# nv-tlabs/GEN3C

Measured on AMD Instinct MI355X. Metric: denoise-steps/sec (121x1280x704 latent, Cosmos-7B), higher is better.
Workload: dtype bf16

## Files before the change

### gen3c_amd/_lib.py

```python
from __future__ import annotations

import ctypes as C
from pathlib import Path

_LIB_PATH = Path(__file__).resolve().parent / "lib" / "libgen3c_hip.so"
_lib = None

vp, i64, i32, f32 = C.c_void_p, C.c_int64, C.c_int, C.c_float

G3_OK, G3_ERR_ARG, G3_ERR_LAUNCH, G3_ERR_RESOURCE = 0, 1, 2, 3

SIGNATURES = {
    "g3_last_error": [],
    "g3_abi_version": [],
    "g3_set_option": [C.c_char_p, i32],
    "g3_device_info": [i32, C.POINTER(i32), C.POINTER(i32), C.c_char_p, i32],
    "g3_event_create": [C.POINTER(vp)],
    "g3_event_record": [vp, vp],
    "g3_event_elapsed_ms": [vp, vp, C.POINTER(f32)],
    "g3_event_destroy": [vp],
    "g3_gemm_bf16_nt": [vp, i64, vp, i64, vp, i64, i32, i32, i32, i32, vp, i32, i64, vp, i64, vp],
    "g3_flash_attn_fwd_kvseg_bf16": [vp, i64, i64, i64, vp, i64, i64, i64, vp, i64, i64, i64, i32, i64, vp, i64, i64, i64, i32, i32, i32,
                                     i32, i32, f32, vp],
    "g3_gemm_kernel_name": [i32, i32, i32, i32],
    "g3_quant_mxfp8_bf16": [vp, i64, vp, i64, vp, i64, i32, i32, vp],
    "g3_gemm_mxfp8_nt": [vp, i64, vp, i64, vp, i64, vp, i64, vp, i64, i32, i32, i32, i32, vp, i32, i64, vp, i64, vp],
    "g3_gemm_mxfp8_kernel_name": [i32, i32, i32, i32],
    "g3_gemm_mxfp8_nt_mxout": [vp, i64, vp, i64, vp, i64, vp, i64, vp, i64, vp, i64, i32, i32, i32, i32, vp],
    "g3_gemm_mxfp8_mxout_kernel_name": [i32, i32, i32, i32],
    "g3_gemv_bf16": [vp, i64, vp, i64, vp, i64, vp, i64, i32, i32, i32, i32, vp],
    "g3_flash_attn_kernel_name": [i32, i32, i32, i32],
    "g3_flash_attn_fwd_bf16": [vp, i64, i64, i64, vp, i64, i64, i64, vp, i64, i64, i64, vp, i64, i64, i64, i32, i32, i32,
                               i32, i32, f32, vp],
    "g3_cross_attn_fwd_bf16": [vp, i64, i64, i64, vp, f32, vp, i64, i64, i64, vp, i64, i64, i64, vp, i64, i64, i64, i32, i32, i32, i32, i32,
                               i32, f32, vp],
    "g3_flash_attn_fwd_ex_bf16": [vp, i64, i64, i64, vp, i64, i64, i64, vp, i64, i64, i64, i32, i64, vp, vp, vp, i64, i64, i64, i32, i32, i32,
                                  i32, i32, f32, i32, vp],
    "g3_flash_attn_fwd_carry_bf16": [vp, i64, i64, i64, vp, i64, i64, i64, vp, i64, i64, i64, i32, i64, i32, i32, vp, vp, vp, vp, vp, i64, i64,
                                     i64, i32, i32, i32, i32, i32, f32, i32, vp],
    "g3_flash_attn_kernel_name_ex": [i32, i32, i32, i32, i32],
    "g3_attn_merge_partials_bf16": [vp, vp, i32, i64, i64, i64, vp, i64, i64, i64, i32, i32, i32, i32, vp],
    "g3_transpose_v_bf16": [vp, i64, vp, i64, i32, i32, i32, i32, vp],
    "g3_layernorm_modulate_bf16": [vp, i64, vp, vp, i64, i32, vp, i64, i32, i32, f32, vp],
    "g3_posemb_layernorm_modulate_bf16": [vp, i64, vp, vp, vp, vp, i32, i32, i32, i32, vp, vp, i64, i32, vp, i64, i32, f32, vp],
    "g3_layernorm_modulate_mxfp8": [vp, i64, vp, vp, i64, i32, vp, i64, vp, i64, i32, i32, f32, vp],
    "g3_posemb_layernorm_modulate_mxfp8": [vp, i64, vp, vp, vp, vp, i32, i32, i32, i32, vp, vp, i64, i32, vp, i64, vp, i64, i32, f32, vp],
    "g3_qk_rmsnorm_rope_bf16": [vp, i64, vp, vp, vp, vp, i64, i32, i32, i32, i32, f32, vp],
    "g3_qk_rmsnorm_rope_pair_bf16": [vp, i64, vp, i32, vp, i32, vp, vp, vp, i64, i32, i32, i32, f32, vp],
    "g3_gemm_qk_norm_rope_bf16": [vp, i64, vp, i64, vp, i64, i32, i32, i32, i32, i32, vp, vp, vp, vp, i32, f32, vp, i64, vp],
    "g3_add_inplace_bf16": [vp, vp, i64, vp],
    "g3_warp_project_f32": [vp, vp, vp, vp, vp, vp, vp, vp, vp, i32, i32, i32, i32, vp],
    "g3_warp_splat_f32": [vp, vp, vp, vp, vp, vp, i32, i32, i32, i32, vp],
    "g3_warp_resolve_f32": [vp, vp, vp, vp, i32, i32, i32, vp],
    "g3_warp_windows_workspace_bytes": [i32, i32, i32],
    "g3_warp_splat_resolve_f32": [vp, vp, vp, vp, vp, vp, vp, vp, vp, vp, i32, i32, i32, i32, vp],
    "g3_render_workspace_bytes": [i32, i32, i32, i32],
    "g3_render_workspace_init": [vp, i32, i32, i32, i32, vp],
    "g3_render_items_f32": [vp, vp, vp, vp, vp, vp, vp, vp, vp, vp, vp, vp, vp, i32, i32, i32, i32, i32, vp],
    "g3_mesh_occlusion_f32": [vp, vp, vp, vp, vp, vp, vp, vp, vp, vp, i32, i32, i32, i32, vp],
    "g3_unproject_points_f32": [vp, vp, vp, vp, i32, i32, i32, vp],
    "g3_dit_patchify_bf16": [vp, vp, vp, i32, vp, i32, i32, i32, i32, i32, i32, vp],
    "g3_dit_unpatchify_bf16": [vp, i64, vp, i32, i32, i32, i32, i32, i32, i32, vp],
    "g3_timestep_embedding_bf16": [vp, vp, vp, vp, i32, i32, vp],
    "g3_reliable_depth_mask_f32": [vp, vp, i32, i32, i32, i32, f32, f32, vp],
    "g3_align_depth_workspace_bytes": [i32, i32],
    "g3_align_depth_f32": [vp, vp, vp, vp, vp, i32, i32, f32, f32, vp, vp, C.c_size_t, i32, i32, vp],
    "g3_conv3d_cl_bf16": [vp, i64, vp, i64, vp, vp, i64, vp, i64] + [i32] * 17 + [vp],
    "g3_conv3d_cl_gnstats_bf16": [vp, i64, vp, i64, vp, vp, i64, vp, i64] + [i32] * 17 + [vp, i32, vp],
    "g3_groupnorm_stats_cl_bf16": [vp, i64, vp, i32, i32, i32, vp],
    "g3_groupnorm_apply_cl_bf16": [vp, i64, vp, vp, vp, vp, i64, i32, i32, i32, f32, i32, vp],
    "g3_groupnorm_swish_cl_bf16": [vp, i64, vp, vp, vp, vp, i64, i32, i32, i32, f32, i32, vp],
    "g3_haar3d_patch_bf16": [vp, vp, i32, i32, i32, vp],
    "g3_haar3d_unpatch_bf16": [vp, i64, vp, i32, i32, i32, vp],
    "g3_resample_cl_bf16": [vp, vp, i32, i32, i32, i32, i32, vp],
    "g3_softmax_rows_bf16": [vp, i64, i32, i32, f32, vp],
    "g3_transpose2d_bf16": [vp, i64, vp, i64, i32, i32, vp],
    "g3_temporal_attn_cl_bf16": [vp, vp, vp, vp, i32, i32, i32, f32, vp],
    "g3_spatial_attn_d512_bf16": [vp, vp, vp, i64, i64, vp, i32, i32, f32, vp],
    "g3_edm_prepare_input_bf16": [vp, vp, vp, vp, vp, vp, i64, i32, i32, f32, f32, f32, f32, vp],
    "g3_edm_cfg_euler_step_bf16": [vp, vp, vp, vp, vp, vp, i64, i32, i32, f32, f32, f32, f32, f32, f32, f32, vp],
}
_RESTYPES = {"g3_last_error": C.c_char_p, "g3_flash_attn_kernel_name": C.c_char_p, "g3_gemm_kernel_name": C.c_char_p, "g3_gemm_mxfp8_kernel_name": C.c_char_p, "g3_gemm_mxfp8_mxout_kernel_name": C.c_char_p, "g3_flash_attn_kernel_name_ex": C.c_char_p, "g3_align_depth_workspace_bytes": C.c_size_t,
             "g3_warp_windows_workspace_bytes": C.c_size_t, "g3_render_workspace_bytes": C.c_size_t}


class Gen3cHipError(RuntimeError):
    pass


def lib_path() -> Path:
    return _LIB_PATH


def load():
    global _lib
    if _lib is not None:
        return _lib
    import torch
    if not _LIB_PATH.exists():
        raise Gen3cHipError(
            f"{_LIB_PATH} is missing: build it with `python -m gen3c_amd.build` (or __graft_entry__.build()). "
            "gen3c_amd has no CPU/PyTorch fallback for its HIP kernels."
        )
    lib = C.CDLL(str(_LIB_PATH))
    for name, argtypes in SIGNATURES.items():
        fn = getattr(lib, name)
        fn.argtypes = argtypes
        fn.restype = _RESTYPES.get(name, C.c_int)
    _lib = lib
    return lib


def last_error() -> str:
    msg = load().g3_last_error()
    return msg.decode() if msg else "?"


def check(rc: int, what: str = ""):
    if rc != 0:
        msg = load().g3_last_error()
        raise Gen3cHipError(f"{what or 'gen3c_hip call'} failed (rc={rc}): {msg.decode() if msg else '?'}")
```

### gen3c_amd/csrc/attention.hip

```cpp
#include "common.hpp"
#include <stdlib.h>
#include <mutex>
#include <type_traits>

namespace {

constexpr int HD = 128;
constexpr int QB = 32;
constexpr int NWAVES = 8;
constexpr int BQ = QB * NWAVES;
constexpr int KVB = 64;
constexpr int NTHREADS = 64 * NWAVES;

struct AttnParams {
    const bf16_t* Q; int64_t q_row, q_batch, q_head;
    const bf16_t* K; int64_t k_row, k_batch, k_head;
    const bf16_t* Vt; int64_t vt_row, vt_batch, vt_head;
    bf16_t* O; int64_t o_row, o_batch, o_head;
    int Sq, Skv;
    float scale_log2;
    int vt_seg_len;
    int64_t vt_seg_stride;
    int grid_q, n_hb, n_heads, xcd_heads;
    float* O32;
    float* LSE;
    int kv_dense;
    const bf16_t* q_norm_w;
    float q_norm_eps;
    const float* carry_o;
    const float* carry_lse;
    int kv_skip_begin, kv_skip_len;
    uint32_t kv_skip_vt_bytes;
};

G3_DEVICE int k_off(int row, int chunk) { return row * HD + ((chunk ^ (row & 15)) << 3); }
G3_DEVICE int v_off(int row, int chunk) { return row * KVB + ((chunk ^ ((row >> 1) & 7)) << 3); }
G3_DEVICE int swap23(int i) { return (i & ~12) | ((i & 4) << 1) | ((i & 8) >> 1); }

template <int CTX>
__global__ __launch_bounds__(NTHREADS, 2) void flash_attn_fwd_kernel(AttnParams p) {
    extern __shared__ __attribute__((aligned(16))) char smem_raw[];
    bf16_t* sK = reinterpret_cast<bf16_t*>(smem_raw);
    bf16_t* sV = sK + 2 * KVB * HD;

    const int tid = threadIdx.x;
    const int lane = tid & 63;
    const int wave = tid >> 6;
    const int l31 = lane & 31;
    const int g = lane >> 5;
    const int head = blockIdx.y;
    const int batch = blockIdx.z;

    const bf16_t* Qb = p.Q + batch * p.q_batch + head * p.q_head;
    const bf16_t* Kb = p.K + batch * p.k_batch + head * p.k_head;
    const bf16_t* Vb = p.Vt + batch * p.vt_batch + head * p.vt_head;
    bf16_t* Ob = p.O + batch * p.o_batch + head * p.o_head;

    const int q_idx = blockIdx.x * BQ + wave * QB + l31;
    const bool q_ok = q_idx < p.Sq;
    bf16x8 qf[8];
    {
        const bf16_t* qrow = Qb + (int64_t)(q_ok ? q_idx : 0) * p.q_row + 8 * g;
#pragma unroll
        for (int ks = 0; ks < 8; ++ks) qf[ks] = q_ok ? load_bf16x8(qrow + 16 * ks) : zero_bf16x8();
    }

    bf16x8 rk[2], rv[2];
    auto stage_load = [&](int kv0) {
#pragma unroll
        for (int i = 0; i < 2; ++i) {
            const int idx = tid + NTHREADS * i;
            {
                const int row = idx >> 4, chunk = idx & 15;
                const bool ok = (kv0 + row) < p.Skv;
                rk[i] = ok ? load_bf16x8(Kb + (int64_t)(kv0 + row) * p.k_row + chunk * 8) : zero_bf16x8();
            }
            {
                const int row = idx >> 3, chunk = idx & 7;
                const bool ok = (kv0 + chunk * 8) < p.Skv;
                rv[i] = ok ? load_bf16x8(Vb + (int64_t)row * p.vt_row + kv0 + chunk * 8) : zero_bf16x8();
            }
        }
    };
    auto stage_write = [&](int buf) {
        bf16_t* dK = sK + buf * KVB * HD;
        bf16_t* dV = sV + buf * HD * KVB;
#pragma unroll
        for (int i = 0; i < 2; ++i) {
            const int idx = tid + NTHREADS * i;
            store_bf16x8(dK + k_off(idx >> 4, idx & 15), rk[i]);
            store_bf16x8(dV + v_off(idx >> 3, idx & 7), rv[i]);
        }
    };

    f32x16 accO[4];
#pragma unroll
    for (int d = 0; d < 4; ++d)
#pragma unroll
        for (int r = 0; r < 16; ++r) accO[d][r] = 0.f;
    float m_run = -1e30f;
    float l_run = 0.f;

    const int krow_perm = swap23(l31);
    const int nt = (p.Skv + KVB - 1) / KVB;
    stage_load(0);
    stage_write(0);
    __syncthreads();

    for (int t = 0; t < nt; ++t) {
        const int buf = t & 1;
        const int kv0 = t * KVB;
        if (t + 1 < nt) stage_load(kv0 + KVB);

        const bf16_t* cK = sK + buf * KVB * HD;
        const bf16_t* cV = sV + buf * HD * KVB;

        f32x16 accS[2];
#pragma unroll
        for (int mb = 0; mb < 2; ++mb) {
#pragma unroll
            for (int r = 0; r < 16; ++r) accS[mb][r] = 0.f;
#pragma unroll
            for (int ks = 0; ks < 8; ++ks) {
                const bf16x8 kf = load_bf16x8(cK + k_off(32 * mb + krow_perm, 2 * ks + g));
                accS[mb] = __builtin_amdgcn_mfma_f32_32x32x16_bf16(kf, qf[ks], accS[mb], 0, 0, 0);
            }
        }

        if (kv0 + KVB > p.Skv) {
#pragma unroll
            for (int mb = 0; mb < 2; ++mb)
#pragma unroll
                for (int r = 0; r < 16; ++r) {
                    const int kv = kv0 + 32 * mb + 16 * (r >> 3) + 8 * g + (r & 7);
                    if (kv >= p.Skv) accS[mb][r] = -INFINITY;
                }
        }

        float mx = accS[0][0];
#pragma unroll
        for (int r = 1; r < 16; ++r) mx = fmaxf(mx, accS[0][r]);
#pragma unroll
        for (int r = 0; r < 16; ++r) mx = fmaxf(mx, accS[1][r]);
        mx = fmaxf(mx, wave_xor_f32(mx, 32));
        const float m_new = fmaxf(m_run, mx * p.scale_log2);
        const float alpha = __builtin_amdgcn_exp2f(m_run - m_new);
        m_run = m_new;

        float psum = 0.f;
        bf16x8 pb[4];
#pragma unroll
        for (int mb = 0; mb < 2; ++mb)
#pragma unroll
            for (int r = 0; r < 16; ++r) {
                const float pv = __builtin_amdgcn_exp2f(__builtin_fmaf(accS[mb][r], p.scale_log2, -m_new));
                psum += pv;
                pb[2 * mb + (r >> 3)][r & 7] = f32_to_bf16(pv);
            }
        l_run = l_run * alpha + psum;
#pragma unroll
        for (int d = 0; d < 4; ++d)
#pragma unroll
            for (int r = 0; r < 16; ++r) accO[d][r] *= alpha;

#pragma unroll
        for (int s = 0; s < 4; ++s) {
#pragma unroll
            for (int d = 0; d < 4; ++d) {
                const bf16x8 vf = load_bf16x8(cV + v_off(32 * d + l31, 2 * s + g));
                accO[d] = __builtin_amdgcn_mfma_f32_32x32x16_bf16(vf, pb[s], accO[d], 0, 0, 0);
            }
        }

        if (t + 1 < nt) stage_write(buf ^ 1);
        __syncthreads();
    }

    const float l_tot = l_run + wave_xor_f32(l_run, 32);
    const float inv = 1.0f / l_tot;
    if (q_ok) {
        bf16_t* orow = Ob + (int64_t)q_idx * p.o_row;
#pragma unroll
        for (int d = 0; d < 4; ++d)
#pragma unroll
            for (int q4 = 0; q4 < 4; ++q4) {
                bf16x4 o;
#pragma unroll
                for (int e = 0; e < 4; ++e) o[e] = f32_to_bf16(accO[d][4 * q4 + e] * inv);
                *reinterpret_cast<bf16x4*>(orow + 32 * d + 8 * q4 + 4 * g) = o;
            }
    }
}


constexpr float RESCALE_THR = 8.0f;

G3_DEVICE float max3(float a, float b, float c) {
    float r;
    asm("v_max3_f32 %0, %1, %2, %3" : "=v"(r) : "v"(a), "v"(b), "v"(c));
    return r;
}
G3_DEVICE void swap_halves(float& a, float& b) {
    asm volatile("s_nop 1\n\tv_permlane32_swap_b32 %0, %1" : "+v"(a), "+v"(b));
}
G3_DEVICE float xor32_max(float x) {
    float a = x, b = x;
    swap_halves(a, b);
    return max3(a, b, b);
}
G3_DEVICE float xor32_sum(float x) {
    float a = x, b = x;
    swap_halves(a, b);
    return a + b;
}

template <int CTX>
__global__ __launch_bounds__(NTHREADS, 2) void flash_attn_fwd_v2_kernel(AttnParams p) {
    extern __shared__ __attribute__((aligned(16))) char smem_raw[];
    bf16_t* sK = reinterpret_cast<bf16_t*>(smem_raw);
    bf16_t* sV = sK + 2 * KVB * HD;

    const int tid = threadIdx.x;
    const int lane = tid & 63;
    const int wave = tid >> 6;
    const int l31 = lane & 31;
    const int g = lane >> 5;
    const int head = blockIdx.y;
    const int batch = blockIdx.z;

    const bf16_t* Qb = p.Q + batch * p.q_batch + head * p.q_head;
    const bf16_t* Kb = p.K + batch * p.k_batch + head * p.k_head;
    const bf16_t* Vb = p.Vt + batch * p.vt_batch + head * p.vt_head;
    bf16_t* Ob = p.O + batch * p.o_batch + head * p.o_head;

    const int q_idx = blockIdx.x * BQ + wave * QB + l31;
    const bool q_ok = q_idx < p.Sq;
    bf16x8 qf[8];
    {
        const bf16_t* qrow = Qb + (int64_t)(q_ok ? q_idx : 0) * p.q_row + 8 * g;
#pragma unroll
        for (int ks = 0; ks < 8; ++ks) qf[ks] = q_ok ? load_bf16x8(qrow + 16 * ks) : zero_bf16x8();
    }

    bf16x8 rk[2], rv[2];
    auto load_k = [&](int kv0) {
#pragma unroll
        for (int i = 0; i < 2; ++i) {
            const int idx = tid + NTHREADS * i;
            const int row = idx >> 4, chunk = idx & 15;
            rk[i] = (kv0 + row) < p.Skv ? load_bf16x8(Kb + (int64_t)(kv0 + row) * p.k_row + chunk * 8) : zero_bf16x8();
        }
    };
    auto load_v = [&](int kv0) {
#pragma unroll
        for (int i = 0; i < 2; ++i) {
            const int idx = tid + NTHREADS * i;
            const int row = idx >> 3, chunk = idx & 7;
            rv[i] = (kv0 + chunk * 8) < p.Skv ? load_bf16x8(Vb + (int64_t)row * p.vt_row + kv0 + chunk * 8) : zero_bf16x8();
        }
    };
    auto write_k = [&](int buf) {
        bf16_t* dK = sK + buf * KVB * HD;
#pragma unroll
        for (int i = 0; i < 2; ++i) {
            const int idx = tid + NTHREADS * i;
            store_bf16x8(dK + k_off(idx >> 4, idx & 15), rk[i]);
        }
    };
    auto write_v = [&](int buf) {
        bf16_t* dV = sV + buf * HD * KVB;
#pragma unroll
        for (int i = 0; i < 2; ++i) {
            const int idx = tid + NTHREADS * i;
            store_bf16x8(dV + v_off(idx >> 3, idx & 7), rv[i]);
        }
    };

    const int krow_perm = swap23(l31);
    int koff[8], voff[4];
#pragma unroll
    for (int ks = 0; ks < 8; ++ks) koff[ks] = k_off(krow_perm, 2 * ks + g);
#pragma unroll
    for (int s4 = 0; s4 < 4; ++s4) voff[s4] = v_off(l31, 2 * s4 + g);
    auto qk = [&](f32x16 (&S)[2], int kbuf) {
        const bf16_t* cK = sK + kbuf * KVB * HD;
#pragma unroll
        for (int mb = 0; mb < 2; ++mb) {
#pragma unroll
            for (int r = 0; r < 16; ++r) S[mb][r] = 0.f;
#pragma unroll
            for (int ks = 0; ks < 8; ++ks) {
                const bf16x8 kf = load_bf16x8(cK + 32 * mb * HD + koff[ks]);
                S[mb] = __builtin_amdgcn_mfma_f32_32x32x16_bf16(kf, qf[ks], S[mb], 0, 0, 0);
            }
        }
    };

    f32x16 accO[4];
#pragma unroll
    for (int d = 0; d < 4; ++d)
#pragma unroll
        for (int r = 0; r < 16; ++r) accO[d][r] = 0.f;
    float m_run = -1e30f;
    float l_run = 0.f;
    const float c = p.scale_log2;
    const int nt = (p.Skv + KVB - 1) / KVB;

    load_k(0);
    load_v(0);
    write_k(0);
    write_v(0);
    if (nt > 1) {
        load_k(KVB);
        write_k(1);
    }
    __syncthreads();
    f32x16 SA[2], SB[2];
    qk(SA, 0);

    auto tile = [&](f32x16 (&S_cur)[2], f32x16 (&S_next)[2], int t, auto has_next_c, auto par_c) {
        constexpr bool has_next = decltype(has_next_c)::value;
        constexpr int par = decltype(par_c)::value;
        const int kv0 = t * KVB;
        if (!has_next && kv0 + KVB > p.Skv) {
#pragma unroll
            for (int mb = 0; mb < 2; ++mb)
#pragma unroll
                for (int r = 0; r < 16; ++r) {
                    const int kv = kv0 + 32 * mb + 16 * (r >> 3) + 8 * g + (r & 7);
                    if (kv >= p.Skv) S_cur[mb][r] = -INFINITY;
                }
        }
        float mx = max3(S_cur[0][0], S_cur[0][1], S_cur[0][2]);
#pragma unroll
        for (int r = 3; r < 15; r += 2) mx = max3(mx, S_cur[0][r], S_cur[0][r + 1]);
// ... 253 lines not shown
            for (int r = 0; r < 16; ++r) SA[mb][r] = 0.f;
#pragma unroll
            for (int ks = 0; ks < 8; ++ks)
                SA[mb] = __builtin_amdgcn_mfma_f32_32x32x16_bf16(load_bf16x8(cK + 32 * mb * HD + koff[ks]), qf[ks], SA[mb], 0, 0, 0);
        }
    }
    G3_JITTER(wave + 1, blockIdx.x);
#ifndef G3_AB_OMIT_PROLOGUE_BARRIER
    __syncthreads();
#endif
    if (nt == 1 && KVB > Skv) mask_tail(SA, 0);
    float mx_cur = row_max(SA);
    f32x16 negm;
    if (FOLD) {
        m_run = mx_cur;
#pragma unroll
        for (int mb = 0; mb < 2; ++mb)
#pragma unroll
            for (int r = 0; r < 16; ++r) SA[mb][r] -= m_run;
#pragma unroll
        for (int r = 0; r < 16; ++r) negm[r] = -m_run;
        mx_cur = 0.f;
    }
#ifndef G3_AB_NO_ATTN_SETPRIO
    if (__builtin_amdgcn_readfirstlane(threadIdx.x) >= 256) __builtin_amdgcn_s_setprio(1);
#endif

    auto tile = [&](f32x16 (&S_cur)[2], f32x16 (&S_next)[2], int t, auto has_next_c, auto par_c) {
        constexpr bool has_next = decltype(has_next_c)::value;
        constexpr int par = decltype(par_c)::value;
        const int kv0 = t * KVB;
        G3_JITTER(wave + blockIdx.x, t);
        if (!has_next && kv0 + KVB > Skv) {
            mask_tail(S_cur, kv0);
            mx_cur = row_max(S_cur);
        }
        if (has_next) {
            if (t + 2 < nt) dma_k(kv0 + 2 * KVB, par);
            dma_v(kv0 + KVB, par ^ 1);
        }
        if (FOLD) {
            if (__any(mx_cur > RESCALE_THR)) {
                const float delta = fmaxf(mx_cur, 0.f);
                const float alpha = __builtin_amdgcn_exp2f(-delta);
                m_run += delta;
                l_run *= alpha;
#pragma unroll
                for (int d = 0; d < 4; ++d)
#pragma unroll
                    for (int r = 0; r < 16; ++r) accO[d][r] *= alpha;
#pragma unroll
                for (int mb = 0; mb < 2; ++mb)
#pragma unroll
                    for (int r = 0; r < 16; ++r) S_cur[mb][r] -= delta;
#pragma unroll
                for (int r = 0; r < 16; ++r) negm[r] = -m_run;
            }
        } else if (__any(mx_cur - m_run > RESCALE_THR)) {
            const float m_new = fmaxf(m_run, mx_cur);
            const float alpha = __builtin_amdgcn_exp2f(m_run - m_new);
            m_run = m_new;
            l_run *= alpha;
#pragma unroll
            for (int d = 0; d < 4; ++d)
#pragma unroll
                for (int r = 0; r < 16; ++r) accO[d][r] *= alpha;
        }
        const float neg_m = -m_run;
        float psum[4] = {0.f, 0.f, 0.f, 0.f};
        bf16x8 pb[4];
        auto softmax_slice = [&](int sl) {
            const int mb = sl >> 1, r0 = (sl & 1) * 8;
#pragma unroll
            for (int j = 0; j < 8; ++j) {
                const float sv = FOLD ? S_cur[mb][r0 + j] : __builtin_fmaf(S_cur[mb][r0 + j], c, neg_m);
                const float pv = (G3_AB_ATTN_ABLATE & 1) ? sv : __builtin_amdgcn_exp2f(sv);
                if (!(G3_AB_ATTN_ABLATE & 2)) psum[sl] += pv;
                pb[sl][j] = f32_to_bf16(pv);
            }
        };

        constexpr int RD = MW_RD;
        bf16x8 fr[RD];
        if (MW && has_next) {
            constexpr int KS = (par ^ 1) * KVB * HD * 2;
            constexpr int VS = par * HD * KVB * 2;
            auto k_addr = [&](auto ksc) -> uint32_t {
                constexpr int ks = decltype(ksc)::value;
                if constexpr (ks < MW_KREGS) return kaddr[ks];
                else return lds_addr_flip128(kaddr[ks - 4]);
            };
            if (!FOLD) {
#pragma unroll
                for (int mb = 0; mb < 2; ++mb)
#pragma unroll
                    for (int r = 0; r < 16; ++r) S_next[mb][r] = 0.f;
            }
            static_for<0, RD - 1>([&](auto ic) { constexpr int i = decltype(ic)::value; lds_read_frag<KS + 32 * (i >> 3) * HD * 2>(fr[i % RD], k_addr(std::integral_constant<int, (i & 7)>{})); });
            static_for<0, 16>([&](auto ic) {
                constexpr int i = decltype(ic)::value;
                constexpr int n = i + RD - 1;
                if constexpr (n < 16) lds_read_frag<KS + 32 * (n >> 3) * HD * 2>(fr[n % RD], k_addr(std::integral_constant<int, (n & 7)>{}));
                else lds_read_frag<VS + 32 * ((n - 16) & 3) * KVB * 2>(fr[n % RD], vaddr[(n - 16) >> 2]);
                lds_wait_frag<RD - 1>(fr[i % RD]);
                S_next[i >> 3] = __builtin_amdgcn_mfma_f32_32x32x16_bf16(fr[i % RD], qf[i & 7], (FOLD && (i & 7) == 0) ? negm : S_next[i >> 3], 0, 0, 0);
                if (i == 3) softmax_slice(0);
                if (i == 11) softmax_slice(1);
            });
#pragma unroll
            for (int i = 0; i < 16; ++i) {
                G3_SGB(SGB_MFMA, 1);
                G3_SGB(SGB_VALU, QA);
                G3_SGB(SGB_TRANS, 1);
            }
        } else if (has_next) {
            const bf16_t* cK = sK + (par ^ 1) * KVB * HD;
            bf16x8 kf[4];
#pragma unroll
            for (int i = 0; i < 3; ++i) kf[i] = load_bf16x8(cK + 32 * (i >> 3) * HD + koff[i & 7]);
            if (G3_AB_ATTN_ABLATE & 8) kf[3] = kf[0];
            if (!FOLD) {
#pragma unroll
                for (int mb = 0; mb < 2; ++mb)
#pragma unroll
                    for (int r = 0; r < 16; ++r) S_next[mb][r] = 0.f;
            }
#pragma unroll
            for (int i = 0; i < 16; ++i) {
                if (i + 3 < 16 && !(G3_AB_ATTN_ABLATE & 8)) kf[(i + 3) & 3] = load_bf16x8(cK + 32 * ((i + 3) >> 3) * HD + koff[(i + 3) & 7]);
                S_next[i >> 3] = __builtin_amdgcn_mfma_f32_32x32x16_bf16(kf[i & 3], qf[i & 7], (FOLD && (i & 7) == 0) ? negm : S_next[i >> 3], 0, 0, 0);
                if (i == 3) softmax_slice(0);
                if (i == 11) softmax_slice(1);
            }
            G3_SGB(SGB_DSR, 3);
#pragma unroll
            for (int i = 0; i < 16; ++i) {
                G3_SGB(SGB_MFMA, 1);
                if (i + 3 < 16) G3_SGB(SGB_DSR, 1);
                G3_SGB(SGB_VALU, QA);
                G3_SGB(SGB_TRANS, 1);
            }
        } else {
            softmax_slice(0);
            softmax_slice(1);
        }

        G3_JITTER(wave + blockIdx.x + 3, t);
        if (MW && has_next) {
            constexpr int VS = par * HD * KVB * 2;
            softmax_slice(2);
            float mx_next = 0.f;
            static_for<0, 16>([&](auto ic) {
                constexpr int i = decltype(ic)::value;
                constexpr int j = i + RD - 1;
                if constexpr (j < 16) lds_read_frag<VS + 32 * (j & 3) * KVB * 2>(fr[(16 + j) % RD], vaddr[j >> 2]);
                lds_wait_frag<(j < 16) ? RD - 1 : (15 - i)>(fr[(16 + i) % RD]);
                accO[i & 3] = __builtin_amdgcn_mfma_f32_32x32x16_bf16(fr[(16 + i) % RD], pb[i >> 2], accO[i & 3], 0, 0, 0);
                if (i == 3) softmax_slice(3);
                if (has_next && i == 7) mx_next = row_max(S_next);
            });
#pragma unroll
            for (int i = 0; i < 16; ++i) {
                G3_SGB(SGB_MFMA, 1);
                G3_SGB(SGB_VALU, QBV);
                G3_SGB(SGB_TRANS, 1);
            }
            l_run += (psum[0] + psum[1]) + (psum[2] + psum[3]);
            mx_cur = mx_next;
        } else {
            const bf16_t* cV = sV + par * HD * KVB;
            bf16x8 vf[4];
#pragma unroll
            for (int i = 0; i < 3; ++i) vf[i] = load_bf16x8(cV + 32 * (i & 3) * KVB + voff[i >> 2]);
            if (G3_AB_ATTN_ABLATE & 8) vf[3] = vf[0];
            softmax_slice(2);
            float mx_next = 0.f;
#pragma unroll
            for (int i = 0; i < 16; ++i) {
                if (i + 3 < 16 && !(G3_AB_ATTN_ABLATE & 8)) vf[(i + 3) & 3] = load_bf16x8(cV + 32 * ((i + 3) & 3) * KVB + voff[(i + 3) >> 2]);
                accO[i & 3] = __builtin_amdgcn_mfma_f32_32x32x16_bf16(vf[i & 3], pb[i >> 2], accO[i & 3], 0, 0, 0);
                if (i == 3) softmax_slice(3);
                if (has_next && i == 7) mx_next = row_max(S_next);
            }
            G3_SGB(SGB_DSR, 3);
#pragma unroll
            for (int i = 0; i < 16; ++i) {
                G3_SGB(SGB_MFMA, 1);
                if (i + 3 < 16) G3_SGB(SGB_DSR, 1);
                G3_SGB(SGB_VALU, QBV);
                G3_SGB(SGB_TRANS, 1);
            }
            l_run += (psum[0] + psum[1]) + (psum[2] + psum[3]);
            mx_cur = mx_next;
        }
        if (has_next) lds_dma_publish_barrier();
    };

    using True = std::integral_constant<bool, true>;
    using False = std::integral_constant<bool, false>;
    using P0 = std::integral_constant<int, 0>;
    using P1 = std::integral_constant<int, 1>;
    int t = 0;
    for (; t + 2 < nt; t += 2) {
        tile(SA, SB, t, True{}, P0{});
        tile(SB, SA, t + 1, True{}, P1{});
    }
    if (t + 1 < nt) {
        tile(SA, SB, t, True{}, P0{});
        tile(SB, SA, t + 1, False{}, P1{});
    } else {
        tile(SA, SB, t, False{}, P0{});
    }

    float l_tot = xor32_sum(l_run);
    float o_scale = 1.0f;
    if (p.kv_dense > 0 && p.kv_dense < p.Skv) {
        const float m_new = fmaxf(m_run, 0.f);
        o_scale = __builtin_amdgcn_exp2f(m_run - m_new);
        l_tot = l_tot * o_scale + (float)(p.Skv - p.kv_dense) * __builtin_amdgcn_exp2f(-m_new);
        m_run = m_new;
    }
    const float inv = o_scale / l_tot;
    if constexpr (CP) {
        const int q_ld = q_ok ? q_idx : p.Sq - 1;
        const int64_t li = ((int64_t)blockIdx.z * p.n_heads + blockIdx.y) * p.Sq + q_ld;
        const int64_t o_hb = (int64_t)blockIdx.z * p.o_batch + (int64_t)blockIdx.y * p.o_head;
        const float lse_k = m_run + __builtin_amdgcn_logf(l_tot);
        f32x4 oc[4][4];
        float lse_c = -INFINITY;
        if (p.carry_lse) {
            const float* crow = p.carry_o + o_hb + (int64_t)q_ld * p.o_row + 4 * g;
#pragma unroll
            for (int d = 0; d < 4; ++d)
#pragma unroll
                for (int q4 = 0; q4 < 4; ++q4) oc[d][q4] = *reinterpret_cast<const f32x4*>(crow + 32 * d + 8 * q4);
            lse_c = p.carry_lse[li];
        } else {
#pragma unroll
            for (int d = 0; d < 4; ++d)
#pragma unroll
                for (int q4 = 0; q4 < 4; ++q4) oc[d][q4] = f32x4{0.f, 0.f, 0.f, 0.f};
        }
        const float mm = fmaxf(lse_c, lse_k);
        const float wc = __builtin_amdgcn_exp2f(lse_c - mm), wk = __builtin_amdgcn_exp2f(lse_k - mm);
        const float rs = 1.0f / (wc + wk);
        const float fc = wc * rs, fk = (wk * rs) * inv;
        const bool use_c = fc > 0.f;
        if (q_ok) {
            const int64_t ro = o_hb + (int64_t)q_idx * p.o_row;
#pragma unroll
            for (int d = 0; d < 4; ++d)
#pragma unroll
                for (int q4 = 0; q4 < 4; ++q4) {
                    const int64_t off = ro + 32 * d + 8 * q4 + 4 * g;
                    f32x4 o;
#pragma unroll
                    for (int e = 0; e < 4; ++e) o[e] = (use_c ? fc * oc[d][q4][e] : 0.f) + fk * accO[d][4 * q4 + e];
                    if (p.O32) {
                        *reinterpret_cast<f32x4*>(p.O32 + off) = o;
                    } else {
                        bf16x4 ob;
#pragma unroll
                        for (int e = 0; e < 4; ++e) ob[e] = f32_to_bf16(o[e]);
                        *reinterpret_cast<bf16x4*>(p.O + off) = ob;
                    }
                }
            if (p.O32 && g == 0) p.LSE[li] = mm + __builtin_amdgcn_logf(wc + wk);
        }
        return;
    }
    if (p.O32) {
        if (q_ok) {
            float* orow = p.O32 + (int64_t)blockIdx.z * p.o_batch + (int64_t)blockIdx.y * p.o_head + (int64_t)q_idx * p.o_row;
#pragma unroll
            for (int d = 0; d < 4; ++d)
#pragma unroll
                for (int q4 = 0; q4 < 4; ++q4) {
                    f32x4 o;
#pragma unroll
                    for (int e = 0; e < 4; ++e) o[e] = accO[d][4 * q4 + e] * inv;
                    *reinterpret_cast<f32x4*>(orow + 32 * d + 8 * q4 + 4 * g) = o;
                }
            if (g == 0) p.LSE[((int64_t)blockIdx.z * p.n_heads + blockIdx.y) * p.Sq + q_idx] = m_run + __builtin_amdgcn_logf(l_tot);
        }
        return;
    }
    if (q_ok) {
        bf16_t* orow = Ob + (int64_t)q_idx * p.o_row;
#pragma unroll
        for (int d = 0; d < 4; ++d)
#pragma unroll
            for (int q4 = 0; q4 < 4; ++q4) {
                bf16x4 o;
#pragma unroll
                for (int e = 0; e < 4; ++e) o[e] = f32_to_bf16(accO[d][4 * q4 + e] * inv);
                *reinterpret_cast<bf16x4*>(orow + 32 * d + 8 * q4 + 4 * g) = o;
            }
    }
}



#include "attention_w4.hpp"
#define W4B_CP 0
#include "attention_w4b.hpp"
#undef W4B_CP
#define W4B_CP 1
#include "attention_w4b.hpp"
#undef W4B_CP

}

static int attn_resolve_variant(int Sq, int Skv, int B, int H, int requested = 0) {
    int variant = requested ? requested : g3_opt_attn_variant;
    if (variant == 0) {
        const long n_wg = (long)((Sq + 255) / 256) * H * B;
        const long rounds = (n_wg + 255) / 256;
        const bool even_fill = n_wg * 100 >= rounds * 256 * 93;
        variant = (Skv > 2048 && (Skv % KVB) == 0 && even_fill) ? 11 : 4;
    }
    if ((variant == 10 || variant == 11) && (Skv % KVB)) variant = 9;
    return variant;
}

extern "C" const char* g3_flash_attn_kernel_name_ex(int Sq, int Skv, int B, int H, int variant_req) {
    const bool long_ctx = Skv > 2048;
    switch (attn_resolve_variant(Sq, Skv, B, H, variant_req)) {
        case 1: return long_ctx ? "flash_attn_fwd_kernel<0>" : "flash_attn_fwd_kernel<1>";
        case 2: return long_ctx ? "flash_attn_fwd_v2_kernel<0>" : "flash_attn_fwd_v2_kernel<1>";
        case 3: return long_ctx ? "flash_attn_fwd_v3_kernel<0, 6, 8, false>" : "flash_attn_fwd_v3_kernel<1, 6, 8, false>";
        case 5: return long_ctx ? "flash_attn_fwd_v3_kernel<0, 6, 8, true>" : "flash_attn_fwd_v3_kernel<1, 6, 8, true>";
        case 6: return long_ctx ? "flash_attn_fwd_v3_kernel<0, 6, 8, true, true, 4, 4>" : "flash_attn_fwd_v3_kernel<1, 6, 8, false, true>";
        case 7: return long_ctx ? "flash_attn_fwd_v3_kernel<0, 6, 8, true, true, 4, 4>" : "flash_attn_fwd_v3_kernel<1, 6, 8, true, true, 4, 4>";
        case 8: return long_ctx ? "flash_attn_fwd_v3_kernel<0, 6, 8, false, true>" : "flash_attn_fwd_v3_kernel<1, 6, 8, false, true>";
        case 9: return long_ctx ? "flash_attn_fwd_w4_kernel<0>" : "flash_attn_fwd_w4_kernel<1>";
        case 10: return "flash_attn_fwd_w4b_kernel<false>";
        case 11: return "flash_attn_fwd_w4b_kernel<true>";
        default: return long_ctx ? "flash_attn_fwd_v3_kernel<0, 6, 8, true>" : "flash_attn_fwd_v3_kernel<1, 6, 8, false>";
    }
}

extern "C" const char* g3_flash_attn_kernel_name(int Sq, int Skv, int B, int H) { return g3_flash_attn_kernel_name_ex(Sq, Skv, B, H, 0); }

static int flash_attn_launch(const void* q, int64_t q_row, int64_t q_batch, int64_t q_head, const void* k, int64_t k_row, int64_t k_batch,
                             int64_t k_head, const void* vt, int64_t vt_row, int64_t vt_batch, int64_t vt_head, int vt_seg_len,
                             int64_t vt_seg_stride, void* o, int64_t o_row, int64_t o_batch, int64_t o_head, int Sq, int Skv, int B, int H,
                             int head_dim, float softmax_scale, void* stream, int variant_req = 0, float* o_partial = nullptr, float* lse = nullptr, int kv_dense = 0,
                             const void* q_norm_w = nullptr, float q_norm_eps = 0.f, bool cp_form = false, const float* carry_o = nullptr,
                             const float* carry_lse = nullptr, int kv_skip_begin = 0, int kv_skip_len = 0, uint32_t kv_skip_vt_bytes = 0) {
    if (!q || !k || !vt || (!o && !o_partial)) return g3_set_error(G3_ERR_ARG, "g3_flash_attn_fwd_bf16: null operand");
    if ((o_partial != nullptr) != (lse != nullptr)) return g3_set_error(G3_ERR_ARG, "g3_flash_attn_fwd_ex_bf16: o_partial and lse go together");
    if (o_partial && (((uintptr_t)o_partial & 15) || ((uintptr_t)lse & 3))) return g3_set_error(G3_ERR_ARG, "g3_flash_attn_fwd_ex_bf16: misaligned o_partial / lse");
    if (head_dim != HD) return g3_set_error(G3_ERR_ARG, "g3_flash_attn_fwd_bf16: head_dim %d unsupported (128 only)", head_dim);
    if (Sq <= 0 || Skv <= 0 || B <= 0 || H <= 0) return g3_set_error(G3_ERR_ARG, "g3_flash_attn_fwd_bf16: bad shape");
    if ((q_row & 7) || (k_row & 7) || (vt_row & 7) || (o_row & 3) || (q_batch & 7) || (k_batch & 7) || (vt_batch & 7) ||
        (q_head & 7) || (k_head & 7) || (vt_head & 7) || (o_batch & 3) || (o_head & 3))
        return g3_set_error(G3_ERR_ARG, "g3_flash_attn_fwd_bf16: strides must keep 16-byte (q,k,vt) / 8-byte (o) alignment");
    if ((((uintptr_t)q | (uintptr_t)k | (uintptr_t)vt) & 15) || ((uintptr_t)o & 7))
        return g3_set_error(G3_ERR_ARG, "g3_flash_attn_fwd_bf16: misaligned pointer");
    const int skv_phys = Skv + kv_skip_len;
    const int kv_span = vt_seg_len > 0 ? vt_seg_len : skv_phys;
    if (vt_seg_len < 0 || (vt_seg_len > 0 && ((vt_seg_len % KVB) || (skv_phys % vt_seg_len) || (vt_seg_stride & 7) || vt_seg_stride <= 0)))
        return g3_set_error(G3_ERR_ARG, "g3_flash_attn_fwd_kvseg_bf16: segments must be a multiple of 64 keys, tile S_kv exactly, 16-byte aligned stride");
    if (vt_row < ((kv_span + 7) & ~7)) return g3_set_error(G3_ERR_ARG, "g3_flash_attn_fwd_bf16: vt leading dim %lld < keys per row rounded to 8", (long long)vt_row);
    AttnParams p;
    p.Q = (const bf16_t*)q; p.q_row = q_row; p.q_batch = q_batch; p.q_head = q_head;
    p.K = (const bf16_t*)k; p.k_row = k_row; p.k_batch = k_batch; p.k_head = k_head;
    p.Vt = (const bf16_t*)vt; p.vt_row = vt_row; p.vt_batch = vt_batch; p.vt_head = vt_head;
    p.O = (bf16_t*)o; p.o_row = o_row; p.o_batch = o_batch; p.o_head = o_head;
    p.Sq = Sq; p.Skv = Skv;
    p.scale_log2 = softmax_scale * 1.4426950408889634f;
    p.vt_seg_len = vt_seg_len; p.vt_seg_stride = vt_seg_stride;
    p.grid_q = 0; p.n_hb = 0; p.n_heads = H; p.xcd_heads = 0;
    p.O32 = o_partial; p.LSE = lse;
    p.kv_dense = 0;
    if (kv_dense > 0) {
        const int kd = ((kv_dense + KVB - 1) / KVB) * KVB;
        if (kv_dense > Skv) return g3_set_error(G3_ERR_ARG, "g3_cross_attn_fwd_bf16: kv_dense %d > S_kv %d", kv_dense, Skv);
        if (kd < Skv) p.kv_dense = kd;
    }
    p.q_norm_w = (const bf16_t*)q_norm_w; p.q_norm_eps = q_norm_eps;
    p.carry_o = carry_o; p.carry_lse = carry_lse;
    p.kv_skip_begin = kv_skip_begin; p.kv_skip_len = kv_skip_len; p.kv_skip_vt_bytes = kv_skip_vt_bytes;
    if (q_norm_w && ((uintptr_t)q_norm_w & 15)) return g3_set_error(G3_ERR_ARG, "g3_cross_attn_fwd_bf16: misaligned q_norm_weight");
    const size_t smem = (size_t)2 * (KVB * HD + HD * KVB) * sizeof(bf16_t);
    static bool attr_set[64] = {};
    static std::mutex attr_mu;
    int variant = attn_resolve_variant(Sq, Skv, B, H, variant_req);
    if (cp_form && variant != 4 && variant != 11)
        return g3_set_error(G3_ERR_ARG, "g3_flash_attn_fwd_carry_bf16: the carry / key-skip form exists for the 8-wave (4) and one-wave-per-SIMD (11) kernels only "
                                        "(variant %d chosen; 11 needs S_kv %% 64 == 0)", variant);
    if (o_partial && variant == 9) variant = 4;
    if ((p.kv_dense || p.q_norm_w) && (variant < 3 || variant >= 9)) variant = 4;
    if (variant >= 3 && vt_row < ((kv_span + KVB - 1) / KVB) * KVB) variant = 2;
    if (variant >= 3) {
        const uint64_t k_max = (uint64_t)(skv_phys - 1 + 2 * KVB) * (uint64_t)k_row * 2u + 256u;
        const uint64_t n_seg = vt_seg_len > 0 ? (uint64_t)(skv_phys / vt_seg_len) : 1u;
        const uint64_t v_max = (uint64_t)(HD - 1) * (uint64_t)vt_row * 2u + (n_seg - 1) * (uint64_t)vt_seg_stride * 2u + ((uint64_t)kv_span + KVB) * 2u + 256u;
        if (k_max > 0xFFFFFFFFull || v_max > 0xFFFFFFFFull) {
            if (cp_form)
                return g3_set_error(G3_ERR_ARG, "g3_flash_attn_fwd_carry_bf16: K / V^T span (skipped keys included) exceeds the kernel's 32-bit byte offsets (k %llu, vt %llu bytes); "
                                                "the 64-bit-addressing kernel has no carry form", (unsigned long long)k_max, (unsigned long long)v_max);
            if (vt_seg_len > 0)
                return g3_set_error(G3_ERR_ARG, "g3_flash_attn_fwd_kvseg_bf16: K / V^T span exceeds the kernel's 32-bit byte offsets (k %llu, vt %llu bytes)",
                                    (unsigned long long)k_max, (unsigned long long)v_max);
            variant = 2;
        }
    }
    if (cp_form && variant < 3)
        return g3_set_error(G3_ERR_ARG, "g3_flash_attn_fwd_carry_bf16: V^T leading dimension %lld below ceil64 of the keys it spans forces the 64-bit-addressing kernel, which has "
                                        "no carry form", (long long)vt_row);
    if (vt_seg_len > 0 && variant < 3)
        return g3_set_error(G3_ERR_ARG, "g3_flash_attn_fwd_kvseg_bf16: segmented V^T is implemented by the default (v3) kernel only");
    if (o_partial && variant < 3)
        return g3_set_error(G3_ERR_ARG, "g3_flash_attn_fwd_ex_bf16: split-KV partial outputs are implemented by the v3 / w4b kernels only (variant %d chosen)", variant);
    if ((p.kv_dense || p.q_norm_w) && variant < 3)
        return g3_set_error(G3_ERR_ARG, "g3_cross_attn_fwd_bf16: the Q norm / zero-tail form is implemented by the v3 kernels only (variant %d chosen: V^T leading dimension below "
                                        "ceil64(S_kv), or operands beyond the kernel's 32-bit byte offsets)", variant);
    int dev_id = 0;
    if (hipGetDevice(&dev_id) != hipSuccess || dev_id < 0 || dev_id >= 64) return g3_set_error(G3_ERR_LAUNCH, "flash_attn: hipGetDevice failed");
    {
      std::lock_guard<std::mutex> attr_lock(attr_mu);
      if (!attr_set[dev_id]) {
        const void* fns[19] = {reinterpret_cast<const void*>(&flash_attn_fwd_w4b_carry_kernel<true>),
                               reinterpret_cast<const void*>(&flash_attn_fwd_v3_kernel<2, 6, 8, true>), reinterpret_cast<const void*>(&flash_attn_fwd_v3_kernel<3, 6, 8, false>),
                               reinterpret_cast<const void*>(&flash_attn_fwd_w4b_kernel<false>), reinterpret_cast<const void*>(&flash_attn_fwd_w4b_kernel<true>),
                               reinterpret_cast<const void*>(&flash_attn_fwd_kernel<0>), reinterpret_cast<const void*>(&flash_attn_fwd_kernel<1>),
                               reinterpret_cast<const void*>(&flash_attn_fwd_v2_kernel<0>), reinterpret_cast<const void*>(&flash_attn_fwd_v2_kernel<1>),
                               reinterpret_cast<const void*>(&flash_attn_fwd_v3_kernel<0, 6, 8, false>), reinterpret_cast<const void*>(&flash_attn_fwd_v3_kernel<1, 6, 8, false>),
                               reinterpret_cast<const void*>(&flash_attn_fwd_v3_kernel<0, 6, 8, true>), reinterpret_cast<const void*>(&flash_attn_fwd_v3_kernel<1, 6, 8, true>),
                               reinterpret_cast<const void*>(&flash_attn_fwd_v3_kernel<0, 6, 8, true, true, 4, 4>), reinterpret_cast<const void*>(&flash_attn_fwd_v3_kernel<1, 6, 8, true, true, 4, 4>),
                               reinterpret_cast<const void*>(&flash_attn_fwd_v3_kernel<0, 6, 8, false, true>), reinterpret_cast<const void*>(&flash_attn_fwd_v3_kernel<1, 6, 8, false, true>),
                               reinterpret_cast<const void*>(&flash_attn_fwd_w4_kernel<0>), reinterpret_cast<const void*>(&flash_attn_fwd_w4_kernel<1>)};
        for (int i = 0; i < 19; ++i) {
            hipError_t e = hipFuncSetAttribute(fns[i], hipFuncAttributeMaxDynamicSharedMemorySize, (int)smem);
            if (e != hipSuccess) return g3_set_error(G3_ERR_LAUNCH, "flash_attn: hipFuncSetAttribute: %s", hipGetErrorString(e));
        }
        attr_set[dev_id] = true;
      }
    }
    dim3 grid((Sq + BQ - 1) / BQ, H, B);
    const bool long_ctx = Skv > 2048;
    hipStream_t st = (hipStream_t)stream;
    if (variant == 10 || variant == 11) {
        dim3 grid4((Sq + W4_BQ - 1) / W4_BQ, H, B);
        p.grid_q = (int)grid4.x; p.n_hb = H * B; p.n_heads = H;
        p.xcd_heads = (g3_opt_attn_xcd_heads && (H * B) % 8 == 0) ? 1 : 0;
        if (p.xcd_heads) grid4 = dim3(grid4.x * H * B, 1, 1);
        if (cp_form) hipLaunchKernelGGL(flash_attn_fwd_w4b_carry_kernel<true>, grid4, dim3(W4_THREADS), smem, st, p);
        else if (variant == 11) hipLaunchKernelGGL(flash_attn_fwd_w4b_kernel<true>, grid4, dim3(W4_THREADS), smem, st, p);
        else hipLaunchKernelGGL(flash_attn_fwd_w4b_kernel<false>, grid4, dim3(W4_THREADS), smem, st, p);
        return g3_check_launch("g3_flash_attn_fwd_bf16");
    }
    if (variant == 9) {
        dim3 grid4((Sq + W4_BQ - 1) / W4_BQ, H, B);
        if (long_ctx) hipLaunchKernelGGL(flash_attn_fwd_w4_kernel<0>, grid4, dim3(W4_THREADS), smem, st, p);
        else hipLaunchKernelGGL(flash_attn_fwd_w4_kernel<1>, grid4, dim3(W4_THREADS), smem, st, p);
        return g3_check_launch("g3_flash_attn_fwd_bf16");
    }
#define G3_LAUNCH_ATTN(KERNEL0, KERNEL1) do { if (long_ctx) hipLaunchKernelGGL(KERNEL0, grid, dim3(NTHREADS), smem, st, p); else hipLaunchKernelGGL(KERNEL1, grid, dim3(NTHREADS), smem, st, p); } while (0)
    if (cp_form) G3_LAUNCH_ATTN((flash_attn_fwd_v3_kernel<2, 6, 8, true>), (flash_attn_fwd_v3_kernel<3, 6, 8, false>));
    else if (variant == 1) G3_LAUNCH_ATTN(flash_attn_fwd_kernel<0>, flash_attn_fwd_kernel<1>);
    else if (variant == 2) G3_LAUNCH_ATTN(flash_attn_fwd_v2_kernel<0>, flash_attn_fwd_v2_kernel<1>);
    else if (variant == 3) G3_LAUNCH_ATTN((flash_attn_fwd_v3_kernel<0, 6, 8, false>), (flash_attn_fwd_v3_kernel<1, 6, 8, false>));
    else if (variant == 5) G3_LAUNCH_ATTN((flash_attn_fwd_v3_kernel<0, 6, 8, true>), (flash_attn_fwd_v3_kernel<1, 6, 8, true>));
    else if (variant == 6) G3_LAUNCH_ATTN((flash_attn_fwd_v3_kernel<0, 6, 8, true, true, 4, 4>), (flash_attn_fwd_v3_kernel<1, 6, 8, false, true>));
    else if (variant == 7) G3_LAUNCH_ATTN((flash_attn_fwd_v3_kernel<0, 6, 8, true, true, 4, 4>), (flash_attn_fwd_v3_kernel<1, 6, 8, true, true, 4, 4>));
    else if (variant == 8) G3_LAUNCH_ATTN((flash_attn_fwd_v3_kernel<0, 6, 8, false, true>), (flash_attn_fwd_v3_kernel<1, 6, 8, false, true>));
    else G3_LAUNCH_ATTN((flash_attn_fwd_v3_kernel<0, 6, 8, true>), (flash_attn_fwd_v3_kernel<1, 6, 8, false>));
#undef G3_LAUNCH_ATTN
    return g3_check_launch("g3_flash_attn_fwd_bf16");
}

extern "C" int g3_flash_attn_fwd_bf16(const void* q, int64_t q_row, int64_t q_batch, int64_t q_head, const void* k,
                                      int64_t k_row, int64_t k_batch, int64_t k_head, const void* vt, int64_t vt_row,
                                      int64_t vt_batch, int64_t vt_head, void* o, int64_t o_row, int64_t o_batch,
                                      int64_t o_head, int Sq, int Skv, int B, int H, int head_dim, float softmax_scale,
                                      void* stream) {
    return flash_attn_launch(q, q_row, q_batch, q_head, k, k_row, k_batch, k_head, vt, vt_row, vt_batch, vt_head, 0, 0, o, o_row, o_batch, o_head,
                             Sq, Skv, B, H, head_dim, softmax_scale, stream);
}

extern "C" int g3_flash_attn_fwd_kvseg_bf16(const void* q, int64_t q_row, int64_t q_batch, int64_t q_head, const void* k, int64_t k_row,
                                            int64_t k_batch, int64_t k_head, const void* vt, int64_t vt_row, int64_t vt_batch,
                                            int64_t vt_head, int vt_seg_len, int64_t vt_seg_stride, void* o, int64_t o_row, int64_t o_batch,
                                            int64_t o_head, int Sq, int Skv, int B, int H, int head_dim, float softmax_scale, void* stream) {
    if (vt_seg_len <= 0) return g3_set_error(G3_ERR_ARG, "g3_flash_attn_fwd_kvseg_bf16: vt_seg_len must be positive");
    return flash_attn_launch(q, q_row, q_batch, q_head, k, k_row, k_batch, k_head, vt, vt_row, vt_batch, vt_head, vt_seg_len, vt_seg_stride, o, o_row,
                             o_batch, o_head, Sq, Skv, B, H, head_dim, softmax_scale, stream);
}

extern "C" int g3_cross_attn_fwd_bf16(const void* q, int64_t q_row, int64_t q_batch, int64_t q_head, const void* q_norm_weight, float q_norm_eps, const void* k,
                                      int64_t k_row, int64_t k_batch, int64_t k_head, const void* vt, int64_t vt_row, int64_t vt_batch, int64_t vt_head, void* o,
                                      int64_t o_row, int64_t o_batch, int64_t o_head, int Sq, int Skv, int kv_dense, int B, int H, int head_dim,
                                      float softmax_scale, void* stream) {
    if (kv_dense < 0) return g3_set_error(G3_ERR_ARG, "g3_cross_attn_fwd_bf16: kv_dense must be >= 0 (0 = every key through the loop)");
    return flash_attn_launch(q, q_row, q_batch, q_head, k, k_row, k_batch, k_head, vt, vt_row, vt_batch, vt_head, 0, 0, o, o_row, o_batch, o_head, Sq, Skv, B, H,
                             head_dim, softmax_scale, stream, 0, nullptr, nullptr, kv_dense, q_norm_weight, q_norm_eps);
}

extern "C" int g3_flash_attn_fwd_ex_bf16(const void* q, int64_t q_row, int64_t q_batch, int64_t q_head, const void* k, int64_t k_row,
                                         int64_t k_batch, int64_t k_head, const void* vt, int64_t vt_row, int64_t vt_batch, int64_t vt_head,
                                         int vt_seg_len, int64_t vt_seg_stride, void* o, float* o_partial, float* lse, int64_t o_row,
                                         int64_t o_batch, int64_t o_head, int Sq, int Skv, int B, int H, int head_dim, float softmax_scale,
                                         int variant, void* stream) {
    if (variant < 0 || variant > 11) return g3_set_error(G3_ERR_ARG, "g3_flash_attn_fwd_ex_bf16: variant %d out of range", variant);
    if (o && o_partial) return g3_set_error(G3_ERR_ARG, "g3_flash_attn_fwd_ex_bf16: pass either o (bf16 result) or o_partial + lse, not both");
    if (o_partial && ((o_row & 3) || (o_batch & 3) || (o_head & 3))) return g3_set_error(G3_ERR_ARG, "g3_flash_attn_fwd_ex_bf16: o_partial strides must be multiples of 4");
    return flash_attn_launch(q, q_row, q_batch, q_head, k, k_row, k_batch, k_head, vt, vt_row, vt_batch, vt_head, vt_seg_len, vt_seg_stride, o, o_row,
                             o_batch, o_head, Sq, Skv, B, H, head_dim, softmax_scale, stream, variant, o_partial, lse);
}

extern "C" int g3_flash_attn_fwd_carry_bf16(const void* q, int64_t q_row, int64_t q_batch, int64_t q_head, const void* k, int64_t k_row,
                                            int64_t k_batch, int64_t k_head, const void* vt, int64_t vt_row, int64_t vt_batch, int64_t vt_head,
                                            int vt_seg_len, int64_t vt_seg_stride, int kv_skip_begin, int kv_skip_len, const float* carry_o,
                                            const float* carry_lse, void* o, float* o_partial, float* lse, int64_t o_row, int64_t o_batch,
                                            int64_t o_head, int Sq, int Skv, int B, int H, int head_dim, float softmax_scale, int variant,
                                            void* stream) {
    const char* fn = "g3_flash_attn_fwd_carry_bf16";
    if (variant < 0 || variant > 11) return g3_set_error(G3_ERR_ARG, "%s: variant %d out of range", fn, variant);
    if (o && o_partial) return g3_set_error(G3_ERR_ARG, "%s: pass either o (bf16 result) or o_partial + lse, not both", fn);
    if (!q || !k || !vt || (!o && !o_partial)) return g3_set_error(G3_ERR_ARG, "%s: null operand", fn);
    if ((o_row & 3) || (o_batch & 3) || (o_head & 3)) return g3_set_error(G3_ERR_ARG, "%s: o / o_partial / carry_o strides must be multiples of 4", fn);
    if ((carry_o != nullptr) != (carry_lse != nullptr)) return g3_set_error(G3_ERR_ARG, "%s: carry_o and carry_lse go together", fn);
    if (carry_o && (((uintptr_t)carry_o & 15) || ((uintptr_t)carry_lse & 3))) return g3_set_error(G3_ERR_ARG, "%s: misaligned carry_o (16 B) / carry_lse (4 B)", fn);
    if (Skv <= 0) return g3_set_error(G3_ERR_ARG, "%s: bad shape", fn);
    if (kv_skip_begin < 0 || kv_skip_len < 0 || (kv_skip_begin % KVB) || (kv_skip_len % KVB) || kv_skip_begin > Skv)
        return g3_set_error(G3_ERR_ARG, "%s: kv_skip (begin %d, len %d) must be multiples of 64 with 0 <= begin <= S_kv %d", fn, kv_skip_begin, kv_skip_len, Skv);
    if (vt_seg_len > 0 && kv_skip_len > 0 && ((kv_skip_begin % vt_seg_len) || (kv_skip_len % vt_seg_len)))
        return g3_set_error(G3_ERR_ARG, "%s: kv_skip (begin %d, len %d) must cover whole V^T segments of %d keys", fn, kv_skip_begin, kv_skip_len, vt_seg_len);
    if ((int64_t)Skv + kv_skip_len > 0x7fffffff) return g3_set_error(G3_ERR_ARG, "%s: S_kv + kv_skip_len overflows", fn);
    const int64_t vt_jump = vt_seg_len > 0 ? (int64_t)(kv_skip_len / vt_seg_len) * vt_seg_stride : (int64_t)kv_skip_len;
    if (vt_seg_len > 0 && vt_seg_stride <= 0) return g3_set_error(G3_ERR_ARG, "%s: vt_seg_stride must be positive", fn);
    if (vt_seg_len == 0 && vt_row < ((int64_t)Skv + kv_skip_len + KVB - 1) / KVB * KVB)
        return g3_set_error(G3_ERR_ARG, "%s: V^T leading dim %lld below ceil64(S_kv + kv_skip_len) forces the 64-bit-addressing kernel, which has no carry form", fn,
                            (long long)vt_row);
    if (kv_skip_len > 0 && kv_skip_begin == 0) {
        k = (const bf16_t*)k + (int64_t)kv_skip_len * k_row;
        vt = (const bf16_t*)vt + vt_jump;
        kv_skip_len = 0;
    }
    if (kv_skip_begin == Skv) kv_skip_len = 0;
    if (kv_skip_len == 0) kv_skip_begin = 0;
    const int64_t vt_jump_bytes = (vt_seg_len > 0 ? (int64_t)(kv_skip_len / vt_seg_len) * vt_seg_stride : (int64_t)kv_skip_len) * 2;
    if (vt_jump_bytes > 0xFFFFFFFFll) return g3_set_error(G3_ERR_ARG, "%s: the skipped V^T range exceeds the kernel's 32-bit byte offsets", fn);
    return flash_attn_launch(q, q_row, q_batch, q_head, k, k_row, k_batch, k_head, vt, vt_row, vt_batch, vt_head, vt_seg_len, vt_seg_stride, o, o_row,
                             o_batch, o_head, Sq, Skv, B, H, head_dim, softmax_scale, stream, variant, o_partial, lse, 0, nullptr, 0.f, true, carry_o,
                             carry_lse, kv_skip_begin, kv_skip_len, (uint32_t)vt_jump_bytes);
}

namespace {
constexpr int MERGE_MAX_PARTS = 8;
struct MergeParams {
    const float* o[MERGE_MAX_PARTS];
    const float* lse[MERGE_MAX_PARTS];
    int n_parts;
    int64_t p_row, p_batch, p_head;
    bf16_t* out; int64_t o_row, o_batch, o_head;
    int Sq, B, H;
};
__global__ __launch_bounds__(256) void attn_merge_partials_kernel(MergeParams p) {
    const int64_t idx = (int64_t)blockIdx.x * 256 + threadIdx.x;
    const int c = (int)(idx & 15);
    int64_t r = idx >> 4;
    const int h = (int)(r % p.H); r /= p.H;
    const int b = (int)(r % p.B);
    const int64_t qi = r / p.B;
    if (qi >= p.Sq) return;
    const int64_t li = ((int64_t)b * p.H + h) * p.Sq + qi;
    float l[MERGE_MAX_PARTS], mx = -INFINITY;
#pragma unroll
    for (int i = 0; i < MERGE_MAX_PARTS; ++i)
        if (i < p.n_parts) { l[i] = p.lse[i][li]; mx = fmaxf(mx, l[i]); }
    float wsum = 0.f;
#pragma unroll
    for (int i = 0; i < MERGE_MAX_PARTS; ++i)
        if (i < p.n_parts) { l[i] = __builtin_amdgcn_exp2f(l[i] - mx); wsum += l[i]; }
    const float inv = 1.0f / wsum;
    float acc[8] = {0.f, 0.f, 0.f, 0.f, 0.f, 0.f, 0.f, 0.f};
    const int64_t poff = qi * p.p_row + (int64_t)b * p.p_batch + (int64_t)h * p.p_head + 8 * c;
#pragma unroll
    for (int i = 0; i < MERGE_MAX_PARTS; ++i)
        if (i < p.n_parts) {
            const f32x4 a = *reinterpret_cast<const f32x4*>(p.o[i] + poff);
            const f32x4 bb = *reinterpret_cast<const f32x4*>(p.o[i] + poff + 4);
            const float w = l[i] * inv;
#pragma unroll
            for (int e = 0; e < 4; ++e) { acc[e] += w * a[e]; acc[4 + e] += w * bb[e]; }
        }
    bf16x8 o;
#pragma unroll
    for (int e = 0; e < 8; ++e) o[e] = f32_to_bf16(acc[e]);
    store_bf16x8(p.out + qi * p.o_row + (int64_t)b * p.o_batch + (int64_t)h * p.o_head + 8 * c, o);
}
}

extern "C" int g3_attn_merge_partials_bf16(const float* const* o_parts, const float* const* lse_parts, int n_parts, int64_t p_row, int64_t p_batch,
                                           int64_t p_head, void* out, int64_t o_row, int64_t o_batch, int64_t o_head, int Sq, int B, int H,
                                           int head_dim, void* stream) {
    if (!o_parts || !lse_parts || !out) return g3_set_error(G3_ERR_ARG, "g3_attn_merge_partials_bf16: null operand");
    if (n_parts < 1 || n_parts > MERGE_MAX_PARTS) return g3_set_error(G3_ERR_ARG, "g3_attn_merge_partials_bf16: 1..%d parts", MERGE_MAX_PARTS);
    if (head_dim != HD || Sq <= 0 || B <= 0 || H <= 0) return g3_set_error(G3_ERR_ARG, "g3_attn_merge_partials_bf16: bad shape");
    if ((p_row & 3) || (p_batch & 3) || (p_head & 3) || (o_row & 7) || (o_batch & 7) || (o_head & 7) || ((uintptr_t)out & 15))
        return g3_set_error(G3_ERR_ARG, "g3_attn_merge_partials_bf16: strides / pointers must keep 16-byte alignment");
    MergeParams p;
    for (int i = 0; i < MERGE_MAX_PARTS; ++i) {
        p.o[i] = i < n_parts ? o_parts[i] : nullptr;
        p.lse[i] = i < n_parts ? lse_parts[i] : nullptr;
        if (i < n_parts && (!p.o[i] || !p.lse[i] || ((uintptr_t)p.o[i] & 15))) return g3_set_error(G3_ERR_ARG, "g3_attn_merge_partials_bf16: part %d null / misaligned", i);
    }
    p.n_parts = n_parts; p.p_row = p_row; p.p_batch = p_batch; p.p_head = p_head;
    p.out = (bf16_t*)out; p.o_row = o_row; p.o_batch = o_batch; p.o_head = o_head; p.Sq = Sq; p.B = B; p.H = H;
    const int64_t total = (int64_t)Sq * B * H * 16;
    hipLaunchKernelGGL(attn_merge_partials_kernel, dim3((unsigned)((total + 255) / 256)), dim3(256), 0, (hipStream_t)stream, p);
    return g3_check_launch("g3_attn_merge_partials_bf16");
}
```

### gen3c_amd/csrc/attention_w4b.hpp

```cpp

#ifndef G3_ATTENTION_W4B_HELPERS
#define G3_ATTENTION_W4B_HELPERS
#define W4B_RING_AGPRS "a192","a193","a194","a195","a196","a197","a198","a199","a200","a201","a202","a203","a204","a205","a206","a207","a208","a209","a210","a211","a212","a213","a214","a215","a216","a217","a218","a219","a220","a221","a222","a223","a224","a225","a226","a227","a228","a229","a230","a231","a232","a233","a234","a235","a236","a237","a238","a239","a240","a241","a242","a243","a244","a245","a246","a247","a248","a249","a250","a251","a252","a253","a254","a255"
#define W4B_OWNED W4_OWNED_AGPRS, W4B_RING_AGPRS
constexpr int W4B_RING0 = 192;
constexpr int W4B_D = 6;

#if G3_AB_ATTN_ABLATE & 32
#define W4B_READ ""
#else
#define W4B_READ "ds_read_b128 a[%c[ra]:%c[rb]], %[addr] offset:%c[off]\n\t"
#endif
#define W4B_QK(h) "v_mfma_f32_32x32x16_bf16 %[s" #h "], a[%c[fa]:%c[fb]], a[%c[q" #h "]:%c[e" #h "]], %[s" #h "]\n\t"
#define W4B_QK0(h) "v_mfma_f32_32x32x16_bf16 %[s" #h "], a[%c[fa]:%c[fb]], a[%c[q" #h "]:%c[e" #h "]], %[c" #h "]\n\t"
#define W4B_PV(h) "v_mfma_f32_32x32x16_bf16 a[%c[o" #h "]:%c[g" #h "]], a[%c[fa]:%c[fb]], %[pf" #h "], a[%c[o" #h "]:%c[g" #h "]]\n\t"
#if G3_AB_ATTN_ABLATE & 128
#define W4B_M0 ""
#define W4B_DMA ""
#else
#define W4B_M0 "s_mov_b32 m0, %[m0v]\n\t"
#define W4B_DMA "global_load_lds_dwordx4 %[voff], %[sbase]\n\t"
#endif
#if G3_AB_ATTN_ABLATE & 256
#define W4B_MAXP(k) ""
#define W4B_MAXP0(k) "v_mov_b32 %[mx], 0\n\tv_mov_b32 %[my], 0\n\t"
#else
#define W4B_MAXP(k) "v_max3_f32 %[mx], %[mx], %[ma" #k "], %[mb" #k "]\n\tv_max3_f32 %[my], %[my], %[mc" #k "], %[md" #k "]\n\t"
#define W4B_MAXP0(k) "v_max3_f32 %[mx], 0, %[ma" #k "], %[mb" #k "]\n\tv_max3_f32 %[my], 0, %[mc" #k "], %[md" #k "]\n\t"
#endif

template <int O0, int O1, int O2, int O3, int O4, int O5> G3_DEVICE void w4b_read_head(uint32_t ad0, uint32_t ad1, uint32_t ad2) {
    static_assert(W4B_D == 6, "w4b_read_head is laid out for a read-ahead of 6");
    if (!(G3_AB_ATTN_ABLATE & 32))
        asm volatile("ds_read_b128 a[192:195], %0 offset:%c3\n\tds_read_b128 a[196:199], %0 offset:%c4\n\tds_read_b128 a[200:203], %1 offset:%c5\n\t"
                     "ds_read_b128 a[204:207], %1 offset:%c6\n\tds_read_b128 a[208:211], %2 offset:%c7\n\tds_read_b128 a[212:215], %2 offset:%c8"
                     ::"v"(ad0), "v"(ad1), "v"(ad2), "n"(O0), "n"(O1), "n"(O2), "n"(O3), "n"(O4), "n"(O5) : W4B_OWNED);
}

#define W4B_XA "v_exp_f32 %[a2], %[x2]\n\tv_exp_f32 %[b2], %[y2]\n\tv_add_f32 %[pe], %[pe], %[a2]\n\t"
#define W4B_XB "v_add_f32 %[pe], %[pe], %[b2]\n\tv_cvt_pk_bf16_f32 %[k2], %[a2], %[b2]\n\t"
template <int I, int ROFF, bool READ, int WN, bool INIT, bool DMA, int EXTRA = 0>
G3_DEVICE void w4b_step_qk(uint32_t addr, f32x16& s0, f32x16& s1, const f32x16& c0, const f32x16& c1, float x1, float y1, uint32_t& k1, float& p1, float& r1,
                           uint32_t m0v, uint32_t voff, const char* sbase, float& a1, float& b1, float x2 = 0.f, float y2 = 0.f, uint32_t* k2 = nullptr,
                           float* pe = nullptr, float* a2 = nullptr, float* b2 = nullptr) {
    constexpr int ks = I >> 1;
    constexpr int q0 = W4_QBASE + 4 * ks, q1 = W4_QBASE + 4 * (8 + ks);
    constexpr int fa = W4B_RING0 + 4 * (I & 15), ra = W4B_RING0 + 4 * ((I + W4B_D) & 15);
#define W4B_A_OUT [a1] "+v"(a1), [b1] "+v"(b1), [k1] "=&v"(k1), [p1] "+v"(p1), [r1] "+v"(r1)
#define W4B_A_IN [addr] "v"(addr), [x1] "v"(x1), [y1] "v"(y1), [off] "n"(ROFF), [wn] "n"(WN), [q0] "n"(q0), [e0] "n"(q0 + 3), [q1] "n"(q1), [e1] "n"(q1 + 3), \
                 [fa] "n"(fa), [fb] "n"(fa + 3), [ra] "n"(ra), [rb] "n"(ra + 3)
    static_assert(READ, "region A always reads ahead");
    if constexpr (INIT && DMA)
        asm volatile(W4B_M0 W4B_READ W4_WAIT W4B_QK0(0) W4_UNIT(1) W4B_DMA W4B_QK0(1)
                     : W4B_A_OUT, [s0] "=&v"(s0), [s1] "=&v"(s1) : W4B_A_IN, [c0] "v"(c0), [c1] "v"(c1), [m0v] "s"(m0v), [voff] "v"(voff), [sbase] "s"(sbase)
                     : "memory");
    else if constexpr (!INIT && DMA)
        asm volatile(W4B_M0 W4B_READ W4_WAIT W4B_QK(0) W4_UNIT(1) W4B_DMA W4B_QK(1)
                     : W4B_A_OUT, [s0] "+v"(s0), [s1] "+v"(s1) : W4B_A_IN, [m0v] "s"(m0v), [voff] "v"(voff), [sbase] "s"(sbase) : "memory");
    else if constexpr (INIT && !DMA && EXTRA == 1)
        asm volatile(W4B_READ W4_WAIT W4B_QK0(0) W4_UNIT(1) W4B_QK0(1) W4B_XA
                     : W4B_A_OUT, [s0] "=&v"(s0), [s1] "=&v"(s1), [a2] "=&v"(*a2), [b2] "=&v"(*b2), [pe] "+v"(*pe)
                     : W4B_A_IN, [c0] "v"(c0), [c1] "v"(c1), [x2] "v"(x2), [y2] "v"(y2));
    else if constexpr (INIT && !DMA)
        asm volatile(W4B_READ W4_WAIT W4B_QK0(0) W4_UNIT(1) W4B_QK0(1)
                     : W4B_A_OUT, [s0] "=&v"(s0), [s1] "=&v"(s1) : W4B_A_IN, [c0] "v"(c0), [c1] "v"(c1));
    else if constexpr (EXTRA == 1)
        asm volatile(W4B_READ W4_WAIT W4B_QK(0) W4_UNIT(1) W4B_QK(1) W4B_XA
                     : W4B_A_OUT, [s0] "+v"(s0), [s1] "+v"(s1), [a2] "=&v"(*a2), [b2] "=&v"(*b2), [pe] "+v"(*pe) : W4B_A_IN, [x2] "v"(x2), [y2] "v"(y2));
    else if constexpr (EXTRA == 2)
        asm volatile(W4B_READ W4_WAIT W4B_QK(0) W4_UNIT(1) W4B_QK(1) W4B_XB
                     : W4B_A_OUT, [s0] "+v"(s0), [s1] "+v"(s1), [k2] "=&v"(*k2), [pe] "+v"(*pe) : W4B_A_IN, [a2] "v"(*a2), [b2] "v"(*b2));
    else
        asm volatile(W4B_READ W4_WAIT W4B_QK(0) W4_UNIT(1) W4B_QK(1) : W4B_A_OUT, [s0] "+v"(s0), [s1] "+v"(s1) : W4B_A_IN);
    static_assert(EXTRA == 0 || (!DMA && !(INIT && EXTRA == 2)), "w4b_step_qk: extra half units only on steps without an LDS-DMA piece");
#undef W4B_A_OUT
#undef W4B_A_IN
}

template <int I, int ROFF, bool READ, int WN, bool UNIT, int MX>
G3_DEVICE void w4b_step_pv(uint32_t addr, const u32x4& pf0, const u32x4& pf1, float x1, float y1, uint32_t& k1, float& p1, float& r1, float& mx, float& my,
                           float ma0, float mb0, float mc0, float md0, float ma1, float mb1, float mc1, float md1, float ma2, float mb2, float mc2, float md2,
                           float& a1, float& b1) {
    constexpr int D = I & 3;
    constexpr int o0 = 16 * D, o1 = 16 * (4 + D);
    constexpr int fa = W4B_RING0 + 4 * ((16 + I) & 15), ra = W4B_RING0 + 4 * ((16 + I + W4B_D) & 15);
#define W4B_B_IN [pf0] "v"(pf0), [pf1] "v"(pf1), [wn] "n"(WN), [o0] "n"(o0), [g0] "n"(o0 + 15), [o1] "n"(o1), [g1] "n"(o1 + 15), [fa] "n"(fa), [fb] "n"(fa + 3)
#define W4B_B_RD [addr] "v"(addr), [off] "n"(ROFF), [ra] "n"(ra), [rb] "n"(ra + 3)
#define W4B_B_UO [a1] "+v"(a1), [b1] "+v"(b1), [k1] "=&v"(k1), [p1] "+v"(p1), [r1] "+v"(r1)
#define W4B_B_UI [x1] "v"(x1), [y1] "v"(y1)
#define W4B_B_M0 [ma0] "v"(ma0), [mb0] "v"(mb0), [mc0] "v"(mc0), [md0] "v"(md0)
    if constexpr (READ && UNIT && MX == 0)
        asm volatile(W4B_READ W4_WAIT W4B_PV(0) W4_UNIT(1) W4B_PV(1) : W4B_B_UO : W4B_B_IN, W4B_B_RD, W4B_B_UI);
    else if constexpr (READ && UNIT && MX == 1)
        asm volatile(W4B_READ W4_WAIT W4B_PV(0) W4_UNIT(1) W4B_PV(1) W4B_MAXP0(0) : W4B_B_UO, [mx] "=&v"(mx), [my] "=&v"(my) : W4B_B_IN, W4B_B_RD, W4B_B_UI, W4B_B_M0);
    else if constexpr (READ && UNIT && MX == 2)
        asm volatile(W4B_READ W4_WAIT W4B_PV(0) W4_UNIT(1) W4B_PV(1) W4B_MAXP(0) : W4B_B_UO, [mx] "+v"(mx), [my] "+v"(my) : W4B_B_IN, W4B_B_RD, W4B_B_UI, W4B_B_M0);
    else if constexpr (!READ && UNIT && MX == 1)
        asm volatile(W4_WAIT W4B_PV(0) W4_UNIT(1) W4B_PV(1) W4B_MAXP0(0) : W4B_B_UO, [mx] "=&v"(mx), [my] "=&v"(my) : W4B_B_IN, W4B_B_UI, W4B_B_M0);
    else if constexpr (!READ && UNIT && MX == 2)
        asm volatile(W4_WAIT W4B_PV(0) W4_UNIT(1) W4B_PV(1) W4B_MAXP(0) : W4B_B_UO, [mx] "+v"(mx), [my] "+v"(my) : W4B_B_IN, W4B_B_UI, W4B_B_M0);
    else if constexpr (!READ && UNIT && MX == 0)
        asm volatile(W4_WAIT W4B_PV(0) W4_UNIT(1) W4B_PV(1) : W4B_B_UO : W4B_B_IN, W4B_B_UI);
    else if constexpr (!READ && !UNIT && MX == 3)
        asm volatile(W4_WAIT W4B_PV(0) W4B_MAXP(0) W4B_PV(1) W4B_MAXP(1) W4B_MAXP(2)
                     : [mx] "+v"(mx), [my] "+v"(my)
                     : W4B_B_IN, W4B_B_M0, [ma1] "v"(ma1), [mb1] "v"(mb1), [mc1] "v"(mc1), [md1] "v"(md1), [ma2] "v"(ma2), [mb2] "v"(mb2), [mc2] "v"(mc2), [md2] "v"(md2));
    else if constexpr (READ && !UNIT && MX == 3)
        asm volatile(W4B_READ W4_WAIT W4B_PV(0) W4B_MAXP(0) W4B_PV(1) W4B_MAXP(1) W4B_MAXP(2)
                     : [mx] "+v"(mx), [my] "+v"(my)
                     : W4B_B_IN, W4B_B_RD, W4B_B_M0, [ma1] "v"(ma1), [mb1] "v"(mb1), [mc1] "v"(mc1), [md1] "v"(md1), [ma2] "v"(ma2), [mb2] "v"(mb2), [mc2] "v"(mc2), [md2] "v"(md2));
    else if constexpr (READ && !UNIT && MX == 0)
        asm volatile(W4B_READ W4_WAIT W4B_PV(0) W4B_PV(1) : : W4B_B_IN, W4B_B_RD);
    else {
        static_assert(!READ && !UNIT && MX == 0, "w4b_step_pv: combination not laid out");
        asm volatile(W4_WAIT W4B_PV(0) W4B_PV(1) : : W4B_B_IN);
    }
#undef W4B_B_RD
#undef W4B_B_UO
#undef W4B_B_UI
#undef W4B_B_M0
}
template <int I, int WN, bool READ = false, int ROFF = 0>
G3_DEVICE void w4b_step_pv_fold(const u32x4& pf0, const u32x4& pf1, float& a0, float& b0, float& c0, float& d0, float& a1, float& b1, float& c1, float& d1, float& t0,
                                 float& t1, uint32_t addr = 0u) {
    constexpr int D = I & 3;
    constexpr int o0 = 16 * D, o1 = 16 * (4 + D);
    constexpr int fa = W4B_RING0 + 4 * ((16 + I) & 15), ra = W4B_RING0 + 4 * ((16 + I + W4B_D) & 15);
    if constexpr (READ && I == 14)
        asm volatile(W4B_READ W4_WAIT W4B_PV(0) "v_max3_f32 %[a0], %[a0], %[b0], %[c0]\n\tv_max3_f32 %[a1], %[a1], %[b1], %[c1]\n\tv_max_f32 %[a0], %[a0], %[d0]\n\tv_max_f32 %[a1], %[a1], %[d1]\n\t"
                     W4B_PV(1) "v_mov_b32 %[t0], %[a0]\n\tv_mov_b32 %[t1], %[a1]\n\t"
                     : [a0] "+v"(a0), [a1] "+v"(a1), [t0] "=&v"(t0), [t1] "=&v"(t1)
                     : W4B_B_IN, [b0] "v"(b0), [c0] "v"(c0), [d0] "v"(d0), [b1] "v"(b1), [c1] "v"(c1), [d1] "v"(d1), [addr] "v"(addr), [off] "n"(ROFF), [ra] "n"(ra), [rb] "n"(ra + 3));
    else if constexpr (READ)
        asm volatile(W4B_READ W4_WAIT W4B_PV(0) "v_permlane32_swap_b32 %[t0], %[a0]\n\tv_permlane32_swap_b32 %[t1], %[a1]\n\t" W4B_PV(1)
                     "v_max_f32 %[a0], %[a0], %[t0]\n\tv_max_f32 %[a1], %[a1], %[t1]\n\t"
                     : [a0] "+v"(a0), [a1] "+v"(a1), [t0] "+v"(t0), [t1] "+v"(t1) : W4B_B_IN, [addr] "v"(addr), [off] "n"(ROFF), [ra] "n"(ra), [rb] "n"(ra + 3));
    else if constexpr (I == 14)
        asm volatile(W4_WAIT W4B_PV(0) "v_max3_f32 %[a0], %[a0], %[b0], %[c0]\n\tv_max3_f32 %[a1], %[a1], %[b1], %[c1]\n\tv_max_f32 %[a0], %[a0], %[d0]\n\tv_max_f32 %[a1], %[a1], %[d1]\n\t"
                     W4B_PV(1) "v_mov_b32 %[t0], %[a0]\n\tv_mov_b32 %[t1], %[a1]\n\t"
                     : [a0] "+v"(a0), [a1] "+v"(a1), [t0] "=&v"(t0), [t1] "=&v"(t1)
                     : W4B_B_IN, [b0] "v"(b0), [c0] "v"(c0), [d0] "v"(d0), [b1] "v"(b1), [c1] "v"(c1), [d1] "v"(d1));
    else
        asm volatile(W4_WAIT W4B_PV(0) "v_permlane32_swap_b32 %[t0], %[a0]\n\tv_permlane32_swap_b32 %[t1], %[a1]\n\t" W4B_PV(1)
                     "v_max_f32 %[a0], %[a0], %[t0]\n\tv_max_f32 %[a1], %[a1], %[t1]\n\t"
                     : [a0] "+v"(a0), [a1] "+v"(a1), [t0] "+v"(t0), [t1] "+v"(t1) : W4B_B_IN);
}
#undef W4B_B_IN

G3_DEVICE void w4b_fence_acc() { asm volatile("s_nop 7\n\ts_nop 3" ::: W4B_OWNED); }
template <int R> G3_DEVICE void w4b_sub_inplace(f32x16& x, float d) {
    float t = x[R];
    asm volatile("v_sub_f32 %0, %0, %1" : "+v"(t) : "v"(d));
    x[R] = t;
}
template <int R> G3_DEVICE void w4b_set_inplace(f32x16& x, float v) {
    float t = x[R];
    asm volatile("v_mov_b32 %0, %1" : "+v"(t) : "v"(v));
    x[R] = t;
}
G3_DEVICE void w4b_mul_inplace(float& x, float a) { asm volatile("v_mul_f32 %0, %0, %1" : "+v"(x) : "v"(a)); }

#endif

#if W4B_CP
#define W4B_KERNEL flash_attn_fwd_w4b_carry_kernel
#else
#define W4B_KERNEL flash_attn_fwd_w4b_kernel
#endif
template <bool XB>
__global__ __launch_bounds__(W4_THREADS, 1) void W4B_KERNEL(AttnParams p) {
    constexpr bool CP = W4B_CP;
    extern __shared__ __attribute__((aligned(16))) char smem_raw[];
    bf16_t* sK = reinterpret_cast<bf16_t*>(smem_raw);
    bf16_t* sV = sK + 2 * KVB * HD;

    const int tid = threadIdx.x;
    const int lane = tid & 63;
    const int wave = __builtin_amdgcn_readfirstlane(tid >> 6);
    const int l31 = lane & 31;
    const int g = lane >> 5;
    int qblk = blockIdx.x, head = blockIdx.y, batch = blockIdx.z;
    if (p.xcd_heads) {
        const int xcd = blockIdx.x & 7, slot = blockIdx.x >> 3;
        const int hb = xcd + 8 * (slot / p.grid_q);
        qblk = slot - (slot / p.grid_q) * p.grid_q;
        head = hb % p.n_heads;
        batch = hb / p.n_heads;
    }

    const bf16_t* Qb = p.Q + batch * p.q_batch + head * p.q_head;
    const bf16_t* Kb = p.K + batch * p.k_batch + head * p.k_head;
    const bf16_t* Vb = p.Vt + batch * p.vt_batch + head * p.vt_head;
    bf16_t* Ob = p.O + batch * p.o_batch + head * p.o_head;
    float* o32_base = p.O32;
    float* lse_base = p.LSE;
    asm volatile("" : "+s"(o32_base), "+s"(lse_base));
    const float* carry_o = nullptr;
    const float* carry_lse = nullptr;
    uint32_t skip_t0 = 0u, skip_nt = 0u, v_skip = 0u;
    if constexpr (CP) {
        carry_o = p.carry_o;
        carry_lse = p.carry_lse;
        skip_t0 = (uint32_t)p.kv_skip_begin / KVB;
        skip_nt = (uint32_t)p.kv_skip_len / KVB;
        v_skip = p.kv_skip_vt_bytes;
        asm volatile("" : "+s"(carry_o), "+s"(carry_lse), "+s"(skip_t0), "+s"(skip_nt), "+s"(v_skip));
    }
    auto k_tile = [&](uint32_t t) -> uint32_t {
        if constexpr (CP) return t + (t >= skip_t0 ? skip_nt : 0u);
        else return t;
    };

    static_for<0, 16>([&](auto fc) {
        constexpr int f = decltype(fc)::value, h = f >> 3, ks = f & 7;
        const int q_idx = qblk * W4_BQ + wave * 64 + 32 * h + l31;
        const bool q_ok = q_idx < p.Sq;
        bf16x8 qv = q_ok ? load_bf16x8(Qb + (int64_t)q_idx * p.q_row + 8 * g + 16 * ks) : zero_bf16x8();
#pragma unroll
        for (int e = 0; e < 8; ++e) qv[e] = f32_to_bf16((float)qv[e] * p.scale_log2);
        const u32x4 qw = __builtin_bit_cast(u32x4, qv);
        w4_acc_write<W4_QBASE + 4 * f + 0>(qw[0]);
        w4_acc_write<W4_QBASE + 4 * f + 1>(qw[1]);
        w4_acc_write<W4_QBASE + 4 * f + 2>(qw[2]);
        w4_acc_write<W4_QBASE + 4 * f + 3>(qw[3]);
    });
    static_for<0, 128>([&](auto rc) { w4_acc_zero<decltype(rc)::value>(); });

    const int k_row0 = tid >> 4, k_src_chunk = (tid & 15) ^ (k_row0 & 15);
    const int v_row0 = tid >> 3, v_src_chunk = (tid & 7) ^ ((v_row0 >> 1) & 7);
    const char* Kbytes = reinterpret_cast<const char*>(Kb);
    const char* Vbytes = reinterpret_cast<const char*>(Vb);
    const uint32_t k_row_bytes = (uint32_t)p.k_row * 2u;
    const uint32_t v_row_bytes = (uint32_t)p.vt_row * 2u;
    uint32_t dma_off[8];
#pragma unroll
    for (int j = 0; j < 4; ++j) {
        dma_off[j] = ((uint32_t)k_row0 + 16u * j) * k_row_bytes + (uint32_t)k_src_chunk * 16u;
        dma_off[4 + j] = ((uint32_t)v_row0 + 32u * j) * v_row_bytes + (uint32_t)v_src_chunk * 16u;
    }
#pragma unroll
    for (int j = 0; j < 8; ++j) asm volatile("" : "+v"(dma_off[j]));
    const uint32_t k_tile_bytes = (uint32_t)KVB * k_row_bytes;
    const uint32_t seg_len = (uint32_t)p.vt_seg_len, seg_bytes = (uint32_t)p.vt_seg_stride * 2u;
    auto v_tile_off = [&](uint32_t kv0) -> uint32_t {
        if (!seg_len) return kv0 * 2u;
        const uint32_t sg = kv0 / seg_len;
        return sg * seg_bytes + (kv0 - sg * seg_len) * 2u;
    };
    auto dma_tile_builtin = [&](const char* base, const uint32_t* off, bf16_t* dst) {
#pragma unroll
        for (int i = 0; i < 4; ++i)
            __builtin_amdgcn_global_load_lds((const __attribute__((address_space(1))) void*)(base + off[i]),
                                             (__attribute__((address_space(3))) void*)(dst + wave * 64 * 8 + 256 * 8 * i), 16, 0, 0);
    };

    const int krow_perm = swap23(l31);
    const uint32_t lds_k0 = (uint32_t)(uintptr_t)(__attribute__((address_space(3))) bf16_t*)sK;
    const uint32_t lds_v0 = (uint32_t)(uintptr_t)(__attribute__((address_space(3))) bf16_t*)sV;
    uint32_t kaddr[8], vaddr[4];
#pragma unroll
    for (int ks = 0; ks < 8; ++ks) kaddr[ks] = lds_k0 + 2u * (uint32_t)k_off(krow_perm, 2 * ks + g);
#pragma unroll
    for (int s4 = 0; s4 < 4; ++s4) vaddr[s4] = lds_v0 + 2u * (uint32_t)v_off(l31, 2 * s4 + g);

    float m_run[2], mx_cur[2];
    float psum[2][4];
#pragma unroll
    for (int h = 0; h < 2; ++h)
#pragma unroll
        for (int k = 0; k < 4; ++k) psum[h][k] = 0.f;
    float ta[2] = {0.f, 0.f}, tb[2] = {0.f, 0.f};
    float pe[2][2] = {{0.f, 0.f}, {0.f, 0.f}};
    float xa[2], xb[2];
    const int nt = p.Skv / KVB;

    dma_tile_builtin(Kbytes, dma_off, sK);
    dma_tile_builtin(Vbytes, dma_off + 4, sV);
    if (nt > 1) dma_tile_builtin(Kbytes + k_tile(1u) * k_tile_bytes, dma_off, sK + KVB * HD);
    G3_JITTER(wave, blockIdx.x + 5);
    lds_dma_publish_barrier();
    G3_JITTER(wave + 2, blockIdx.x);
    f32x16 SA[2][2], SB[2][2];
    f32x16 negm[2];
    {
        f32x16 zero;
#pragma unroll
        for (int r = 0; r < 16; ++r) zero[r] = 0.f;
        static_for<0, 16>([&](auto ic) {
            constexpr int i = decltype(ic)::value, mb = i >> 3, ks = i & 7;
            const bf16x8 kf = load_bf16x8(sK + 32 * mb * HD + k_off(krow_perm, 2 * ks + g));
            if constexpr (ks == 0) {
                w4_qk0<0, -1>(SA[0][mb], kf, zero);
                w4_qk0<8, -1>(SA[1][mb], kf, zero);
            } else {
                w4_qk<ks, -1>(SA[0][mb], kf);
                w4_qk<8 + ks, -1>(SA[1][mb], kf);
            }
        });
    }
    w4_fence_v(SA[0][0], SA[0][1], SA[1][0], SA[1][1]);
    __syncthreads();
#pragma unroll
    for (int h = 0; h < 2; ++h) {
        float ma = max3(SA[h][0][0], SA[h][0][1], SA[h][0][2]);
        float mb2 = max3(SA[h][1][0], SA[h][1][1], SA[h][1][2]);
#pragma unroll
        for (int r = 3; r < 15; r += 2) {
            ma = max3(ma, SA[h][0][r], SA[h][0][r + 1]);
            mb2 = max3(mb2, SA[h][1][r], SA[h][1][r + 1]);
        }
        m_run[h] = xor32_max(max3(ma, mb2, max3(SA[h][0][15], SA[h][1][15], SA[h][1][15])));
#pragma unroll
        for (int mb = 0; mb < 2; ++mb)
#pragma unroll
            for (int r = 0; r < 16; ++r) SA[h][mb][r] -= m_run[h];
#pragma unroll
        for (int r = 0; r < 16; ++r) negm[h][r] = -m_run[h];
        mx_cur[h] = 0.f;
    }
    if (XB && nt > 1) {
        constexpr int KS1 = KVB * HD * 2;
        w4b_read_head<KS1, KS1 + 32 * HD * 2, KS1, KS1 + 32 * HD * 2, KS1, KS1 + 32 * HD * 2>(kaddr[0], kaddr[1], kaddr[2]);
    }
    uint32_t v_off_next = v_tile_off(KVB);
    if constexpr (CP) v_off_next += skip_t0 == 1u ? v_skip : 0u;
    const uint32_t seg_tiles = seg_len ? seg_len / KVB : 0x7fffffffu;
    uint32_t v_seg_pos = seg_len ? (1u % seg_tiles) : 1u;
    const uint32_t v_seg_jump = seg_len ? seg_bytes - seg_len * 2u : 0u;

    auto tile = [&](f32x16 (&S_cur)[2][2], f32x16 (&S_next)[2][2], int t, auto has_next_c, auto par_c) {
        constexpr bool has_next = decltype(has_next_c)::value;
        constexpr int par = decltype(par_c)::value;
        constexpr int D = W4B_D;
        constexpr int KS = (par ^ 1) * KVB * HD * 2;
        constexpr int VS = par * HD * KVB * 2;
        auto frag_off = [](auto nc) constexpr { constexpr int n = decltype(nc)::value; return n < 16 ? KS + 32 * (n & 1) * HD * 2 : VS + 32 * ((n - 16) & 3) * KVB * 2; };
        auto frag_addr = [&](auto nc) -> uint32_t { constexpr int n = decltype(nc)::value; if constexpr (n < 16) return kaddr[(n >> 1) & 7]; else return vaddr[((n - 16) >> 2) & 3]; };
        G3_JITTER(wave + blockIdx.x, t);
        if constexpr (!(XB && has_next)) {
            constexpr int n0 = has_next ? 0 : 16;
            using N0 = std::integral_constant<int, n0>;
            using N1 = std::integral_constant<int, n0 + 1>;
            using N2 = std::integral_constant<int, n0 + 2>;
            using N3 = std::integral_constant<int, n0 + 3>;
            using N4 = std::integral_constant<int, n0 + 4>;
            using N5 = std::integral_constant<int, n0 + 5>;
            w4b_read_head<frag_off(N0{}), frag_off(N1{}), frag_off(N2{}), frag_off(N3{}), frag_off(N4{}), frag_off(N5{})>(frag_addr(N0{}), frag_addr(N2{}), frag_addr(N4{}));
        }
        if (__any(fmaxf(mx_cur[0], mx_cur[1]) > RESCALE_THR)) {
            float alpha[2], delta[2];
#pragma unroll
            for (int h = 0; h < 2; ++h) {
                delta[h] = mx_cur[h];
                alpha[h] = __builtin_amdgcn_exp2f(-delta[h]);
                m_run[h] += delta[h];
            }
            asm volatile("s_nop 7\n\ts_nop 3" : "+v"(alpha[0]), "+v"(alpha[1]) : : W4B_OWNED);
#pragma unroll
            for (int h = 0; h < 2; ++h) {
#pragma unroll
                for (int k = 0; k < 4; ++k) w4b_mul_inplace(psum[h][k], alpha[h]);
                if (XB && h == 0) {
                    w4b_mul_inplace(pe[0][0], alpha[0]);
                    w4b_mul_inplace(pe[0][1], alpha[0]);
                    w4b_mul_inplace(pe[1][0], alpha[0]);
                    w4b_mul_inplace(pe[1][1], alpha[0]);
                }
                const float nm = -m_run[h], dl = delta[h];
                static_for<0, 16>([&](auto rc) {
                    constexpr int r = decltype(rc)::value;
                    w4b_sub_inplace<r>(S_cur[h][0], dl);
                    w4b_sub_inplace<r>(S_cur[h][1], dl);
                    w4b_set_inplace<r>(negm[h], nm);
                });
            }
            static_for<0, 64>([&](auto rc) { w4_acc_scale<decltype(rc)::value>(alpha[0]); });
            static_for<64, 128>([&](auto rc) { w4_acc_scale<decltype(rc)::value>(alpha[1]); });
        }
        u32x4 pb[2][4];
        auto ux = [&](auto uc) -> float { constexpr int u = decltype(uc)::value, sl = u >> 3, h = (u >> 2) & 1, q = u & 3; return S_cur[h][sl >> 1][(sl & 1) * 8 + 2 * q]; };
        auto uy = [&](auto uc) -> float { constexpr int u = decltype(uc)::value, sl = u >> 3, h = (u >> 2) & 1, q = u & 3; return S_cur[h][sl >> 1][(sl & 1) * 8 + 2 * q + 1]; };
        auto uput = [&](auto uc, uint32_t pk) { constexpr int u = decltype(uc)::value, sl = u >> 3, h = (u >> 2) & 1, q = u & 3; pb[h][sl][q] = pk; };
        auto sm_unit = [&](auto uc) {
            constexpr int u = decltype(uc)::value, h = (u >> 2) & 1, pa = 2 * (u & 1);
            float a, b;
            uint32_t pk;
            if (G3_AB_ATTN_ABLATE & 16) {
                pk = 0;
            } else {
                asm volatile("v_exp_f32 %0, %5\n\tv_exp_f32 %1, %6\n\tv_add_f32 %3, %3, %0\n\tv_add_f32 %4, %4, %1\n\tv_cvt_pk_bf16_f32 %2, %0, %1"
                             : "=&v"(a), "=&v"(b), "=v"(pk), "+v"(psum[h][pa]), "+v"(psum[h][pa + 1]) : "v"(ux(uc)), "v"(uy(uc)));
            }
            uput(uc, pk);
        };
        constexpr int NHEAD = has_next ? (XB ? 0 : 4) : 20;
        static_for<0, NHEAD>([&](auto uc) { sm_unit(uc); });

        if constexpr (has_next) {
            const int t2 = min(t + 2, nt - 1);
            const char* kbase = Kbytes + k_tile((uint32_t)t2) * k_tile_bytes;
            const char* vbase = Vbytes + v_off_next;
            static_for<0, 16>([&](auto ic) {
                constexpr int I = decltype(ic)::value;
                using NR = std::integral_constant<int, I + D>;
                using U = std::integral_constant<int, (XB ? 0 : 4) + I>;
                constexpr int hu = (U::value >> 2) & 1, pa = 2 * (I & 1);
                constexpr bool dma = XB ? (I & 1) == 0 : I < 8;
                constexpr int j = XB ? (I >> 1) : (I & 7);
                const uint32_t m0v = dma ? (j < 4 ? lds_k0 + (uint32_t)(par * KVB * HD * 2 + 256 * j * 16) : lds_v0 + (uint32_t)((par ^ 1) * HD * KVB * 2 + 256 * (j - 4) * 16)) + (uint32_t)wave * 1024u : 0u;
                uint32_t k1 = 0;
                if constexpr (XB && (I & 1)) {
                    constexpr int ex = (I & 2) ? 2 : 1;
                    constexpr int xu = 16 + (I >> 2);
                    using XU = std::integral_constant<int, xu>;
                    uint32_t k2 = 0;
                    w4b_step_qk<I, frag_off(NR{}), true, D, (I >> 1) == 0, false, ex>(frag_addr(NR{}), S_next[0][I & 1], S_next[1][I & 1], negm[0], negm[1], ux(U{}), uy(U{}), k1,
                                                                                      psum[hu][pa], psum[hu][pa + 1], 0u, 0u, nullptr, ta[I & 1], tb[I & 1], ux(XU{}), uy(XU{}), &k2,
                                                                                      &pe[0][ex - 1], &xa[0], &xb[0]);
                    if constexpr (ex == 2) uput(XU{}, k2);
                } else {
                    w4b_step_qk<I, frag_off(NR{}), true, D, (I >> 1) == 0, dma>(frag_addr(NR{}), S_next[0][I & 1], S_next[1][I & 1], negm[0], negm[1], ux(U{}), uy(U{}), k1,
                                                                               psum[hu][pa], psum[hu][pa + 1], m0v, dma_off[j], j < 4 ? kbase : vbase, ta[I & 1], tb[I & 1]);
                }
                uput(U{}, k1);
            });
            const bool wrap = (v_seg_pos + 1u == seg_tiles);
            v_off_next += wrap ? (uint32_t)(KVB * 2) + v_seg_jump : (uint32_t)(KVB * 2);
            v_seg_pos = wrap ? 0u : v_seg_pos + 1u;
            if constexpr (CP) v_off_next += (uint32_t)(t + 2) == skip_t0 ? v_skip : 0u;
        }
        G3_JITTER(wave + blockIdx.x + 3, t);
        {
            float cx[2][2], cy[2][2], tx[2];
            auto sn = [&](auto hc, auto mbc, auto rc) -> float { return S_next[decltype(hc)::value][decltype(mbc)::value][decltype(rc)::value]; };
            constexpr int KSN = par * KVB * HD * 2;
            auto rd_off = [](auto nc) constexpr { constexpr int n = decltype(nc)::value; return n < 32 ? VS + 32 * ((n - 16) & 3) * KVB * 2 : KSN + 32 * (n & 1) * HD * 2; };
            auto rd_addr = [&](auto nc) -> uint32_t { constexpr int n = decltype(nc)::value; if constexpr (n < 32) return vaddr[((n - 16) >> 2) & 3]; else return kaddr[((n - 32) >> 1) & 7]; };
            static_for<0, 14>([&](auto ic) {
                constexpr int I = decltype(ic)::value;
                constexpr bool rd = (I + D < 16) || (XB && has_next);
                using NR = std::integral_constant<int, rd ? 16 + I + D : 16>;
                constexpr bool unit = I < 12;
                using U = std::integral_constant<int, unit ? 20 + I : 20>;
                constexpr int hu = (U::value >> 2) & 1, pa = 2 * (I & 1);
                constexpr int mxk = !has_next ? 0 : (I < 2 ? 0 : (I == 2 || I == 3 || I == 10 || I == 11) ? 1 : I < 12 ? 2 : 3);
                constexpr int mh = I < 10 ? 0 : 1;
                constexpr int k0 = I < 2 ? 0 : I < 10 ? I - 2 : I < 12 ? I - 10 : I == 12 ? 2 : 5;
                constexpr int k1i = mxk == 3 ? k0 + 1 : k0, k2i = mxk == 3 ? k0 + 2 : k0;
                using H = std::integral_constant<int, mh>;
#define W4B_SN(mb, r) (has_next ? sn(H{}, std::integral_constant<int, mb>{}, std::integral_constant<int, (r)>{}) : 0.f)
                if constexpr (XB && has_next && I == 10) {
                    if (!(G3_AB_ATTN_ABLATE & 64)) asm volatile("s_waitcnt vmcnt(0)\n\ts_barrier" ::: "memory");
                }
                uint32_t k1 = 0;
                w4b_step_pv<I, rd_off(NR{}), rd, rd ? D : 15 - I, unit, mxk>(rd_addr(NR{}), pb[0][I >> 2], pb[1][I >> 2], ux(U{}), uy(U{}), k1, psum[hu][pa], psum[hu][pa + 1],
                                                                          cx[mh][I & 1], cy[mh][I & 1], W4B_SN(0, 2 * k0), W4B_SN(0, 2 * k0 + 1), W4B_SN(1, 2 * k0),
                                                                          W4B_SN(1, 2 * k0 + 1), W4B_SN(0, 2 * k1i), W4B_SN(0, 2 * k1i + 1), W4B_SN(1, 2 * k1i),
                                                                          W4B_SN(1, 2 * k1i + 1), W4B_SN(0, 2 * k2i), W4B_SN(0, 2 * k2i + 1), W4B_SN(1, 2 * k2i),
                                                                          W4B_SN(1, 2 * k2i + 1), ta[I & 1], tb[I & 1]);
#undef W4B_SN
                if constexpr (unit) uput(U{}, k1);
            });
            if constexpr (has_next) {
                if constexpr (XB) {
                    using N14 = std::integral_constant<int, 16 + 14 + D>;
                    using N15 = std::integral_constant<int, 16 + 15 + D>;
                    w4b_step_pv_fold<14, D, true, rd_off(N14{})>(pb[0][3], pb[1][3], cx[0][0], cy[0][0], cx[0][1], cy[0][1], cx[1][0], cy[1][0], cx[1][1], cy[1][1], tx[0], tx[1],
                                                                 rd_addr(N14{}));
                    w4b_step_pv_fold<15, D, true, rd_off(N15{})>(pb[0][3], pb[1][3], cx[0][0], cy[0][0], cx[0][1], cy[0][1], cx[1][0], cy[1][0], cx[1][1], cy[1][1], tx[0], tx[1],
                                                                 rd_addr(N15{}));
                } else {
                    w4b_step_pv_fold<14, 1>(pb[0][3], pb[1][3], cx[0][0], cy[0][0], cx[0][1], cy[0][1], cx[1][0], cy[1][0], cx[1][1], cy[1][1], tx[0], tx[1]);
                    w4b_step_pv_fold<15, 0>(pb[0][3], pb[1][3], cx[0][0], cy[0][0], cx[0][1], cy[0][1], cx[1][0], cy[1][0], cx[1][1], cy[1][1], tx[0], tx[1]);
                }
                mx_cur[0] = cx[0][0];
                mx_cur[1] = cx[1][0];
            } else {
                float d0 = 0.f, d1 = 0.f;
                uint32_t kd = 0;
                w4b_step_pv<14, 0, false, 1, false, 0>(0u, pb[0][3], pb[1][3], 0.f, 0.f, kd, d0, d1, d0, d1, 0, 0, 0, 0, 0, 0, 0, 0, 0, 0, 0, 0, d0, d1);
                w4b_step_pv<15, 0, false, 0, false, 0>(0u, pb[0][3], pb[1][3], 0.f, 0.f, kd, d0, d1, d0, d1, 0, 0, 0, 0, 0, 0, 0, 0, 0, 0, 0, 0, d0, d1);
            }
        }
        if (!XB && has_next && !(G3_AB_ATTN_ABLATE & 64)) lds_dma_publish_barrier();
    };

    using True = std::integral_constant<bool, true>;
    using False = std::integral_constant<bool, false>;
    using P0 = std::integral_constant<int, 0>;
    using P1 = std::integral_constant<int, 1>;
    int t = 0;
    for (; t + 2 < nt; t += 2) {
        tile(SA, SB, t, True{}, P0{});
        tile(SB, SA, t + 1, True{}, P1{});
    }
    if (t + 1 < nt) {
        tile(SA, SB, t, True{}, P0{});
        tile(SB, SA, t + 1, False{}, P1{});
    } else {
        tile(SA, SB, t, False{}, P0{});
    }

    w4b_fence_acc();
    static_for<0, 2>([&](auto hc) {
        constexpr int h = decltype(hc)::value;
        const float extra = (XB && h == 0) ? (pe[0][0] + pe[0][1]) + (pe[1][0] + pe[1][1]) : 0.f;
        const float inv = 1.0f / xor32_sum(((psum[h][0] + psum[h][1]) + (psum[h][2] + psum[h][3])) + extra);
        const int q_idx = qblk * W4_BQ + wave * 64 + 32 * h + l31;
        if constexpr (CP) {
            const bool q_ok = q_idx < p.Sq;
            const int q_ld = q_ok ? q_idx : p.Sq - 1;
            const int64_t li = ((int64_t)batch * p.n_heads + head) * p.Sq + q_ld;
            const int64_t ro = (int64_t)batch * p.o_batch + (int64_t)head * p.o_head + (int64_t)q_idx * p.o_row;
            const int64_t ro_ld = (int64_t)batch * p.o_batch + (int64_t)head * p.o_head + (int64_t)q_ld * p.o_row;
            const float lse_k = m_run[h] - __builtin_amdgcn_logf(inv);
            f32x4 oc[16];
            float lse_c = -INFINITY;
            if (carry_lse) {
                using gf32x4 = const __attribute__((address_space(1))) f32x4;
                gf32x4* crow = (gf32x4*)(carry_o + ro_ld + 4 * g);
#pragma unroll
                for (int c = 0; c < 16; ++c) oc[c] = crow[(32 * (c >> 2) + 8 * (c & 3)) / 4];
                lse_c = ((const __attribute__((address_space(1))) float*)carry_lse)[li];
            } else {
#pragma unroll
                for (int c = 0; c < 16; ++c) oc[c] = f32x4{0.f, 0.f, 0.f, 0.f};
            }
            const float mm = fmaxf(lse_c, lse_k);
            const float wc = __builtin_amdgcn_exp2f(lse_c - mm), wk = __builtin_amdgcn_exp2f(lse_k - mm);
            const float rs = 1.0f / (wc + wk);
            const float fc = wc * rs, fk = (wk * rs) * inv;
            const bool use_c = fc > 0.f;
            static_for<0, 16>([&](auto cc) {
                constexpr int c = decltype(cc)::value, d = c >> 2, q4 = c & 3;
                constexpr int R = 16 * (4 * h + d) + 4 * q4;
                const int64_t off = ro + 32 * d + 8 * q4 + 4 * g;
                float o[4];
                o[0] = (use_c ? fc * oc[c][0] : 0.f) + fk * w4_acc_read<R + 0>();
                o[1] = (use_c ? fc * oc[c][1] : 0.f) + fk * w4_acc_read<R + 1>();
                o[2] = (use_c ? fc * oc[c][2] : 0.f) + fk * w4_acc_read<R + 2>();
                o[3] = (use_c ? fc * oc[c][3] : 0.f) + fk * w4_acc_read<R + 3>();
                if (!q_ok) return;
                if (o32_base) {
                    *reinterpret_cast<f32x4*>(o32_base + off) = f32x4{o[0], o[1], o[2], o[3]};
                } else {
                    bf16x4 ob;
#pragma unroll
                    for (int e = 0; e < 4; ++e) ob[e] = f32_to_bf16(o[e]);
                    *reinterpret_cast<bf16x4*>(p.O + off) = ob;
                }
            });
            if (o32_base && g == 0 && q_ok) lse_base[li] = mm + __builtin_amdgcn_logf(wc + wk);
            return;
        }
        if (o32_base) {
            float* prow = o32_base + (int64_t)batch * p.o_batch + (int64_t)head * p.o_head + (int64_t)q_idx * p.o_row;
            static_for<0, 16>([&](auto cc) {
                constexpr int d = decltype(cc)::value >> 2, q4 = decltype(cc)::value & 3;
                constexpr int R = 16 * (4 * h + d) + 4 * q4;
                f32x4 o;
                o[0] = w4_acc_read<R + 0>() * inv;
                o[1] = w4_acc_read<R + 1>() * inv;
                o[2] = w4_acc_read<R + 2>() * inv;
                o[3] = w4_acc_read<R + 3>() * inv;
                if (q_idx < p.Sq) *reinterpret_cast<f32x4*>(prow + 32 * d + 8 * q4 + 4 * g) = o;
            });
            if (g == 0 && q_idx < p.Sq) lse_base[((int64_t)batch * p.n_heads + head) * p.Sq + q_idx] = m_run[h] - __builtin_amdgcn_logf(inv);
            return;
        }
        bf16_t* orow = Ob + (int64_t)q_idx * p.o_row;
        static_for<0, 16>([&](auto cc) {
            constexpr int d = decltype(cc)::value >> 2, q4 = decltype(cc)::value & 3;
            constexpr int R = 16 * (4 * h + d) + 4 * q4;
            bf16x4 o;
            o[0] = f32_to_bf16(w4_acc_read<R + 0>() * inv);
            o[1] = f32_to_bf16(w4_acc_read<R + 1>() * inv);
            o[2] = f32_to_bf16(w4_acc_read<R + 2>() * inv);
            o[3] = f32_to_bf16(w4_acc_read<R + 3>() * inv);
            if (q_idx < p.Sq) *reinterpret_cast<bf16x4*>(orow + 32 * d + 8 * q4 + 4 * g) = o;
        });
    });
}
#undef W4B_KERNEL
```

### gen3c_amd/dit.py

```python
from __future__ import annotations

import math
from enum import Enum
from typing import Dict, List, Optional, Tuple

import torch
from torch import nn

from . import ops
from .parallel import ContextParallelAttention, split_inputs_cp

_FUSE_QKV_EPILOGUE = __import__("os").environ.get("G3_FUSE_QKV_EPILOGUE", "0") != "0"


_V_OPERAND_SWAP = __import__("os").environ.get("G3_V_OPERAND_SWAP", "1") != "0"


def _v_by_operand_swap(S: int) -> bool:
    return _V_OPERAND_SWAP and S % 4 == 0


_CROSS_Q_NORM_IN_ATTENTION = __import__("os").environ.get("G3_CROSS_Q_NORM_IN_ATTENTION", "1") != "0"


def _project_norm_rope(h, w, n_q, n_k, norm_q, norm_k, cos, sin, S, B, nH_total, hq=None, wq=None):
    if wq is not None:
        y = ops.gemm_mxfp8_nt(hq[0], hq[1], wq[0], wq[1])
    elif _FUSE_QKV_EPILOGUE:
        return ops.gemm_qk_norm_rope(h, w, n_q, n_k, norm_q, norm_k, cos, sin, S, B)
    else:
        y = ops.gemm_nt(h, w)
    if n_q and n_k:
        ops.qk_rmsnorm_rope_pair(y[:, :n_q + n_k], norm_q, n_q // 128, norm_k, n_k // 128, cos, sin, S, B)
    elif n_q:
        ops.qk_rmsnorm_rope(y[:, :n_q], norm_q, cos, sin, S, B, n_q // 128, out=y[:, :n_q])
    elif n_k:
        ops.qk_rmsnorm_rope(y[:, n_q:n_q + n_k], norm_k, cos, sin, S, B, n_k // 128, out=y[:, n_q:n_q + n_k])
    return y


LINEAR_PRECISIONS = ("bf16", "mxfp8")
MXFP8_PRODUCERS = ("separate", "fused")
MXFP8_LINEARS = ("fa_qkv", "fa_out", "ca_q", "ca_out", "w1", "w2")


def _mx_rows(blk: dict, name: str, rows: slice):
    mx = blk.get("mx")
    return None if mx is None else (mx[name][0][rows], mx[name][1][rows])


class DataType(Enum):
    IMAGE = "image"
    VIDEO = "video"


def tensor_version(t: torch.Tensor) -> Optional[int]:
    return None if t.is_inference() else t._version


def cacheable(*tensors) -> bool:
    return all(not (isinstance(t, torch.Tensor) and t.is_inference()) for t in tensors)


def _is_video(data_type) -> bool:
    v = getattr(data_type, "value", data_type)
    return str(v).lower().endswith("video")


class _Node(nn.Module):
    """Anonymous container used to reproduce the reference's parameter names (e.g. `to_q.0.weight`)."""


def _register(root: nn.Module, dotted: str, tensor: torch.Tensor, buffer: bool = False):
    *path, leaf = dotted.split(".")
    mod = root
    for p in path:
        if p not in mod._modules:
            mod.add_module(p, _Node())
        mod = mod._modules[p]
    if buffer:
        mod.register_buffer(leaf, tensor, persistent=True)
    else:
        mod.register_parameter(leaf, nn.Parameter(tensor, requires_grad=False))


def _xavier_uniform_(t: torch.Tensor):
    fan_out, fan_in = t.shape
    a = math.sqrt(6.0 / (fan_in + fan_out))
    return t.uniform_(-a, a)


class VideoExtendGeneralDIT(nn.Module):
    def __init__(
        self,
        max_img_h: int = 240,
        max_img_w: int = 240,
        max_frames: int = 128,
        in_channels: int = 16 + 1,
        out_channels: int = 16,
        patch_spatial: int = 2,
        patch_temporal: int = 1,
        concat_padding_mask: bool = True,
        block_config: str = "FA-CA-MLP",
        model_channels: int = 4096,
        num_blocks: int = 28,
        num_heads: int = 32,
        mlp_ratio: float = 4.0,
        block_x_format: str = "THWBD",
        crossattn_emb_channels: int = 1024,
        use_cross_attn_mask: bool = False,
        pos_emb_cls: str = "rope3d",
        pos_emb_learnable: bool = False,
        pos_emb_interpolation: str = "crop",
        affline_emb_norm: bool = True,
        use_adaln_lora: bool = True,
        adaln_lora_dim: int = 256,
        rope_h_extrapolation_ratio: float = 1.0,
        rope_w_extrapolation_ratio: float = 1.0,
        rope_t_extrapolation_ratio: float = 1.0,
        extra_per_block_abs_pos_emb: bool = True,
        extra_per_block_abs_pos_emb_type: str = "learnable",
        extra_h_extrapolation_ratio: float = 1.0,
        extra_w_extrapolation_ratio: float = 1.0,
        extra_t_extrapolation_ratio: float = 1.0,
        add_augment_sigma_embedding: bool = False,
        device: Optional[torch.device | str] = None,
        dtype: torch.dtype = torch.bfloat16,
        init_weights: bool = True,
        linear_precision: str = "bf16",
        mxfp8_producers: str = "separate",
    ) -> None:
        super().__init__()
        if block_config.upper() != "FA-CA-MLP":
            raise NotImplementedError(f"block_config {block_config!r}: only 'FA-CA-MLP' (GEN3C-Cosmos-7B) is built")
        if block_x_format != "THWBD" or pos_emb_cls != "rope3d" or not use_adaln_lora or not affline_emb_norm:
            raise NotImplementedError("only the faditv2 configuration (THWBD, rope3d, AdaLN-LoRA, affine emb norm) is built")
        if not extra_per_block_abs_pos_emb or extra_per_block_abs_pos_emb_type.lower() != "learnable":
            raise NotImplementedError("extra_per_block_abs_pos_emb must be the learnable per-axis embedding")
        if use_cross_attn_mask or add_augment_sigma_embedding or pos_emb_learnable:
            raise NotImplementedError("use_cross_attn_mask / add_augment_sigma_embedding / learnable rope are not used by GEN3C")
        if model_channels // num_heads != 128:
            raise NotImplementedError("head_dim must be 128 (HIP attention kernel)")
        if dtype != torch.bfloat16:
            raise NotImplementedError("the HIP path computes in bf16 (reference precision='bfloat16', config/base/model.py:29)")

        self.max_img_h, self.max_img_w, self.max_frames = max_img_h, max_img_w, max_frames
        self.in_channels, self.out_channels = in_channels, out_channels
        self.patch_spatial, self.patch_temporal = patch_spatial, patch_temporal
        self.concat_padding_mask = concat_padding_mask
        self.model_channels, self.num_blocks, self.num_heads = model_channels, num_blocks, num_heads
        self.mlp_hidden = int(model_channels * mlp_ratio)
        self.crossattn_emb_channels = crossattn_emb_channels
        self.adaln_lora_dim = adaln_lora_dim
        self.block_x_format = block_x_format
        self.head_dim = 128
        self.base_fps = 24
        self.cp_group = None
        self.cp_size = None
        self._cp_attn: Optional[ContextParallelAttention] = None
        self.cross_attention_skip_zero_context = True
        self._tables: Dict[tuple, tuple] = {}
        self._packed = None
        self.linear_precision = "bf16"
        self.set_linear_precision(linear_precision)
        self.mxfp8_producers = "separate"
        self.set_mxfp8_producers(mxfp8_producers)
        self._tune_blocks: Optional[int] = None

        D, Hd = model_channels, self.head_dim
        kw = dict(device=device, dtype=dtype)
        E = lambda *shape: torch.empty(*shape, **kw)
        emb_in = (in_channels + (1 if concat_padding_mask else 0)) * patch_spatial * patch_spatial * patch_temporal
        self.patch_dim = emb_in

        _register(self, "x_embedder.proj.1.weight", E(D, emb_in))
        len_h, len_w, len_t = max_img_h // patch_spatial, max_img_w // patch_spatial, max_frames // patch_temporal
        _register(self, "pos_embedder.seq", torch.arange(max(len_h, len_w, len_t), dtype=torch.float, device=device), buffer=True)
        _register(self, "extra_pos_embedder.pos_emb_h", E(len_h, D))
        _register(self, "extra_pos_embedder.pos_emb_w", E(len_w, D))
        _register(self, "extra_pos_embedder.pos_emb_t", E(len_t, D))
        _register(self, "t_embedder.1.linear_1.weight", E(D, D))
        _register(self, "t_embedder.1.linear_2.weight", E(3 * D, D))
        for i in range(num_blocks):
            pre = f"blocks.block{i}.blocks"
            for j, ctx in ((0, D), (1, crossattn_emb_channels)):
                a = f"{pre}.{j}.block.attn"
                _register(self, f"{a}.to_q.0.weight", E(D, D))
                _register(self, f"{a}.to_q.1.weight", E(Hd))
                _register(self, f"{a}.to_k.0.weight", E(D, ctx))
                _register(self, f"{a}.to_k.1.weight", E(Hd))
                _register(self, f"{a}.to_v.0.weight", E(D, ctx))
                _register(self, f"{a}.to_out.0.weight", E(D, D))
            _register(self, f"{pre}.2.block.layer1.weight", E(self.mlp_hidden, D))
            _register(self, f"{pre}.2.block.layer2.weight", E(D, self.mlp_hidden))
            for j in range(3):
                _register(self, f"{pre}.{j}.adaLN_modulation.1.weight", E(adaln_lora_dim, D))
                _register(self, f"{pre}.{j}.adaLN_modulation.2.weight", E(3 * D, adaln_lora_dim))
        _register(self, "final_layer.linear.weight", E(patch_spatial * patch_spatial * patch_temporal * out_channels, D))
        _register(self, "final_layer.adaLN_modulation.1.weight", E(adaln_lora_dim, D))
        _register(self, "final_layer.adaLN_modulation.2.weight", E(2 * D, adaln_lora_dim))
        _register(self, "affline_norm.weight", E(D))

        dim_h = Hd // 6 * 2
        dim_t = Hd - 2 * dim_h
        self._rope_dims = (dim_t, dim_h, dim_h)
        self.h_ntk_factor = rope_h_extrapolation_ratio ** (dim_h / (dim_h - 2))
        self.w_ntk_factor = rope_w_extrapolation_ratio ** (dim_h / (dim_h - 2))
        self.t_ntk_factor = rope_t_extrapolation_ratio ** (dim_t / (dim_t - 2))

        if init_weights:
            self.initialize_weights()

    @torch.no_grad()
    def initialize_weights(self, randomize_adaln: bool = False, seed: Optional[int] = None):
        gen = None
        if seed is not None:
            gen = torch.Generator(device=self.affline_norm.weight.device)
            gen.manual_seed(seed)
        for name, p in self.named_parameters():
            if name.endswith(".to_q.1.weight") or name.endswith(".to_k.1.weight") or name == "affline_norm.weight":
                p.fill_(1.0)
            elif name.startswith("extra_pos_embedder."):
                tmp = torch.empty(p.shape, dtype=torch.float32, device=p.device)
                nn.init.trunc_normal_(tmp, std=0.02, a=-2.0, b=2.0, generator=gen)
                p.copy_(tmp)
            elif name.startswith("t_embedder."):
                p.normal_(0.0, 0.02, generator=gen)
            elif name.endswith("adaLN_modulation.2.weight") and not name.startswith("final_layer."):
                if randomize_adaln:
                    p.normal_(0.0, 0.02, generator=gen)
                else:
                    p.zero_()
            else:
                fan_out, fan_in = p.shape
                a = math.sqrt(6.0 / (fan_in + fan_out))
                p.uniform_(-a, a, generator=gen)
        self._packed = None
        self._tables.clear()

    def load_state_dict(self, state_dict, strict: bool = True, assign: bool = False):
        sd = {k: v for k, v in state_dict.items() if not k.endswith("_extra_state")}
        out = super().load_state_dict(sd, strict=strict, assign=assign)
        self._packed = None
        self._tables.clear()
        return out

    def _apply(self, fn, *args, **kwargs):
        out = super()._apply(fn, *args, **kwargs)
        self._packed = None
        self._tables.clear()
        return out

    def set_linear_precision(self, precision: str) -> None:
        if precision not in LINEAR_PRECISIONS:
            raise ValueError(f"linear_precision must be one of {LINEAR_PRECISIONS}, got {precision!r}")
        if precision != self.linear_precision:
            self._packed = None
        self.linear_precision = precision

    def set_mxfp8_producers(self, producers: str) -> None:
        if producers not in MXFP8_PRODUCERS:
            raise ValueError(f"mxfp8_producers must be one of {MXFP8_PRODUCERS}, got {producers!r}")
        self.mxfp8_producers = producers

    def _linear(self, a, blk: dict, name: str, out_mx: bool = False, **kw):
        mx = blk.get("mx")
        if mx is None:
            return ops.gemm_nt(a, blk[name], **kw)
        aq, as_ = a if isinstance(a, tuple) else ops.quant_mxfp8(a)
        if out_mx:
            kw["out_mx"] = True
        return ops.gemm_mxfp8_nt(aq, as_, mx[name][0], mx[name][1], **kw)

    def _ln(self, xs: torch.Tensor, shift: torch.Tensor, scale: torch.Tensor, fused: bool):
        return ops.layernorm_modulate_mxfp8(xs, shift, scale) if fused else ops.layernorm_modulate(xs, shift, scale)

    def _weights_key(self) -> tuple:
        return tuple((p.data_ptr(), tensor_version(p)) for p in self.parameters())

    def _pack(self):
        key = self._weights_key()
        if (self._packed is not None and self._packed["key"] == key and self._packed["versioned"]
                and self._packed["precision"] == self.linear_precision):
            return self._packed
        if self._packed is not None and self._packed["key"] != key:
            self._tables.clear()
        P = dict(self.named_parameters())
        blocks = []
        for i in range(self.num_blocks):
            pre = f"blocks.block{i}.blocks"
            fa, ca, mlp = f"{pre}.0", f"{pre}.1", f"{pre}.2"
            blocks.append(dict(
                fa_qkv=torch.cat([P[f"{fa}.block.attn.to_q.0.weight"], P[f"{fa}.block.attn.to_k.0.weight"],
                                  P[f"{fa}.block.attn.to_v.0.weight"]], dim=0).contiguous(),
                fa_qn=P[f"{fa}.block.attn.to_q.1.weight"], fa_kn=P[f"{fa}.block.attn.to_k.1.weight"],
                fa_out=P[f"{fa}.block.attn.to_out.0.weight"],
                ca_q=P[f"{ca}.block.attn.to_q.0.weight"],
                ca_kv=torch.cat([P[f"{ca}.block.attn.to_k.0.weight"], P[f"{ca}.block.attn.to_v.0.weight"]], dim=0).contiguous(),
                ca_qn=P[f"{ca}.block.attn.to_q.1.weight"], ca_kn=P[f"{ca}.block.attn.to_k.1.weight"],
                ca_out=P[f"{ca}.block.attn.to_out.0.weight"],
                w1=P[f"{mlp}.block.layer1.weight"], w2=P[f"{mlp}.block.layer2.weight"],
                ada=[(P[f"{pre}.{j}.adaLN_modulation.1.weight"], P[f"{pre}.{j}.adaLN_modulation.2.weight"]) for j in range(3)],
            ))
        if self.linear_precision == "mxfp8":
            for blk in blocks:
                blk["mx"] = {n: ops.quant_mxfp8(blk[n]) for n in MXFP8_LINEARS}
        self._packed = dict(blocks=blocks, P=P, key=key, versioned=cacheable(*P.values()), precision=self.linear_precision)
        return self._packed

    def enable_context_parallel(self, cp_group):
        import torch.distributed as dist
        self.cp_group = cp_group
        self.cp_size = dist.get_world_size(cp_group)
        self._cp_attn = ContextParallelAttention(cp_group, head_groups=4, schedule="local_first")
        cfg = __import__("os").environ.get("G3_CP_CONFIG")
        if cfg:
            g_, kern_, sched_ = (c.strip() for c in cfg.split(","))
            self._cp_attn.configure(head_groups=int(g_), kernel=kern_, schedule=sched_)
        self._tables.clear()

    def _cp_fused_qkv(self) -> bool:
        return self._cp_attn is not None and self._cp_attn.schedule in ("local_first", "local_carry")

    def disable_context_parallel(self):
        self.cp_group = None
        self.cp_size = None
        self._cp_attn = None
        self._tables.clear()

    @property
    def is_context_parallel_enabled(self) -> bool:
        return self.cp_group is not None

    @torch.no_grad()
    def _position_tables(self, B: int, T: int, Hp: int, Wp: int, fps: Optional[torch.Tensor], device) -> tuple:
        fps_val = None if fps is None else float(fps.flatten()[0])
        cp = self.cp_size or 1
        rank = 0
        if self.cp_group is not None:
            import torch.distributed as dist
            rank = dist.get_rank(self.cp_group)
        key = (B, T, Hp, Wp, fps_val, cp, rank, str(device))
        if key in self._tables:
            return self._tables[key]
        Tg = T * cp
        dim_t, dim_h, dim_w = self._rope_dims
        seq = self.pos_embedder.seq.to(device=device, dtype=torch.float32)
        rng_s = torch.arange(0, dim_h, 2, device=device)[: dim_h // 2].float() / dim_h
        rng_t = torch.arange(0, dim_t, 2, device=device)[: dim_t // 2].float() / dim_t
        h_freqs = 1.0 / ((10000.0 * self.h_ntk_factor) ** rng_s)
        w_freqs = 1.0 / ((10000.0 * self.w_ntk_factor) ** rng_s)
        t_freqs = 1.0 / ((10000.0 * self.t_ntk_factor) ** rng_t)
        assert Hp <= self.max_img_h // self.patch_spatial and Wp <= self.max_img_w // self.patch_spatial
        half_h = torch.outer(seq[:Hp], h_freqs)
        half_w = torch.outer(seq[:Wp], w_freqs)
        if fps_val is None:
            assert Tg == 1, "T should be 1 for image batch."
            half_t = torch.outer(seq[:Tg], t_freqs)
        else:
            half_t = torch.outer(seq[:Tg] / fps_val * self.base_fps, t_freqs)
        half = torch.cat([
            half_t[:, None, None, :].expand(Tg, Hp, Wp, -1),
            half_h[None, :, None, :].expand(Tg, Hp, Wp, -1),
            half_w[None, None, :, :].expand(Tg, Hp, Wp, -1),
        ], dim=-1)
        freqs = torch.cat([half, half], dim=-1)
        freqs = freqs[rank * T:(rank + 1) * T].reshape(T * Hp * Wp, 128).float()
        cos, sin = torch.cos(freqs).contiguous(), torch.sin(freqs).contiguous()

        pe_t = self.extra_pos_embedder.pos_emb_t[:Tg][rank * T:(rank + 1) * T].contiguous()
        pe_h = self.extra_pos_embedder.pos_emb_h[:Hp].contiguous()
        pe_w = self.extra_pos_embedder.pos_emb_w[:Wp].contiguous()
        emb = (pe_t[:, None, None, :] + pe_h[None, :, None, :]) + pe_w[None, None, :, :]
        norm = torch.linalg.vector_norm(emb, dim=-1, keepdim=True, dtype=torch.float32)
        norm = torch.add(1e-6, norm, alpha=math.sqrt(1.0 / emb.shape[-1]))
        pos = dict(pe_t=pe_t, pe_h=pe_h, pe_w=pe_w, norm=norm.to(emb.dtype).reshape(T * Hp * Wp).contiguous())
        del emb
        self._tables[key] = (cos, sin, pos)
        return self._tables[key]

    def position_embedding_rows(self, B: int, T: int, Hp: int, Wp: int, fps, device) -> torch.Tensor:
        pos = self._position_tables(B, T, Hp, Wp, fps, device)[2]
        emb = (pos["pe_t"][:, None, None, :] + pos["pe_h"][None, :, None, :]) + pos["pe_w"][None, None, :, :]
        emb = emb / pos["norm"].reshape(T, Hp, Wp, 1)
        D = emb.shape[-1]
        return emb.reshape(T * Hp * Wp, 1, D).expand(-1, B, -1).reshape(T * Hp * Wp * B, D).contiguous()

    @torch.no_grad()
    def forward(
        self,
        x: torch.Tensor,
        timesteps: torch.Tensor,
        crossattn_emb: torch.Tensor,
        crossattn_mask: Optional[torch.Tensor] = None,
        fps: Optional[torch.Tensor] = None,
        image_size: Optional[torch.Tensor] = None,
        padding_mask: Optional[torch.Tensor] = None,
        scalar_feature: Optional[torch.Tensor] = None,
        data_type=DataType.VIDEO,
        video_cond_bool: Optional[torch.Tensor] = None,
        condition_video_indicator: Optional[torch.Tensor] = None,
        condition_video_input_mask: Optional[torch.Tensor] = None,
        condition_video_augment_sigma: Optional[torch.Tensor] = None,
        condition_video_pose: Optional[torch.Tensor] = None,
        **kwargs,
    ) -> torch.Tensor:
        if scalar_feature is not None:
            raise NotImplementedError("Scalar feature is not implemented yet.")
        B, C, T, H, W = x.shape
        dev = x.device
        sources = [(x.to(torch.bfloat16).contiguous(), True)]
        if _is_video(data_type):
            assert condition_video_input_mask is not None, "condition_video_input_mask is required for video data type"
            if self.cp_group is not None:
                condition_video_input_mask = split_inputs_cp(condition_video_input_mask, 2, self.cp_group)
                if condition_video_indicator is not None:
                    condition_video_indicator = split_inputs_cp(condition_video_indicator, 2, self.cp_group)
                if condition_video_pose is not None:
                    condition_video_pose = split_inputs_cp(condition_video_pose, 2, self.cp_group)
            sources.append((condition_video_input_mask.to(torch.bfloat16).contiguous(), True))
            if condition_video_pose is not None:
                sources.append((condition_video_pose.to(torch.bfloat16).contiguous(), True))
        if self.concat_padding_mask:
            pm = _nearest_resize(padding_mask, (H, W)).to(torch.bfloat16)
            sources.append((pm.reshape(B, 1, H, W).contiguous(), False))
        c_in = sum(t.shape[1] for t, _ in sources)
        assert c_in * self.patch_spatial ** 2 * self.patch_temporal == self.patch_dim, f"channel mismatch: got {c_in} input channels"

        ps, pt = self.patch_spatial, self.patch_temporal
        Tp, Hp, Wp = T // pt, H // ps, W // ps
        S = Tp * Hp * Wp
        D = self.model_channels
        patches = ops.dit_patchify(sources, B, T, H, W, pt, ps)

        pk = self._pack()
        P = pk["P"]
        cos, sin, pos = self._position_tables(B, Tp, Hp, Wp, fps, dev)

        xs = ops.gemm_nt(patches, P["x_embedder.proj.1.weight"])

        ts = timesteps.flatten().to(torch.float32)
        if ts.shape[0] != B:
            ts = ts.expand(B)
        t_sin, emb = ops.timestep_embedding(ts.contiguous(), P["affline_norm.weight"], D)
        h1 = ops.gemv(t_sin, P["t_embedder.1.linear_1.weight"])
        adaln_lora = ops.gemv(h1, P["t_embedder.1.linear_2.weight"], act_in=1)

        M = crossattn_emb.shape[1]
        nH = self.num_heads
        ca_kv, ca_dense = self._cross_attention_kv(pk, crossattn_emb)
        if not self.cross_attention_skip_zero_context:
            ca_dense = 0
        for bi, blk in enumerate(pk["blocks"][: self._tune_blocks] if self._tune_blocks else pk["blocks"]):
            shift, scale, gate = self._modulation(emb, blk["ada"][0], adaln_lora, 3)
            if "full" not in pos:
                pe_sum = (pos["pe_t"][:, None, None, :] + pos["pe_h"][None, :, None, :]) + pos["pe_w"][None, None, :, :]
                pos["full"] = (pe_sum / pos["norm"].reshape(Tp, Hp, Wp, 1)).reshape(S, D).contiguous()
                del pe_sum
            fused = "mx" in blk and self.mxfp8_producers == "fused"
            if fused:
                h, hq = None, ops.posemb_layernorm_modulate_mxfp8(xs, pos["full"], None, None, None, Tp, Hp, Wp, B, shift, scale)
            else:
                h = ops.posemb_layernorm_modulate(xs, pos["full"], None, None, None, Tp, Hp, Wp, B, shift, scale)
                hq = ops.quant_mxfp8(h) if "mx" in blk else None
            if self._cp_fused_qkv():
                qkv = _project_norm_rope(h, blk["fa_qkv"], D, D, blk["fa_qn"], blk["fa_kn"], cos, sin, S, B, nH, hq=hq,
                                         wq=_mx_rows(blk, "fa_qkv", slice(None)))
                pending = self._cp_attn.start(qkv[:, D:2 * D], qkv[:, 2 * D:], S, B, nH)
                o = self._cp_attn.finish(qkv[:, :D], pending)
            elif self._cp_attn is not None:
                kv = _project_norm_rope(h, blk["fa_qkv"][D:], 0, D, None, blk["fa_kn"], cos, sin, S, B, nH, hq=hq,
                                        wq=_mx_rows(blk, "fa_qkv", slice(D, None)))
                pending = self._cp_attn.start(kv[:, :D], kv[:, D:], S, B, nH)
                q = _project_norm_rope(h, blk["fa_qkv"][:D], D, 0, blk["fa_qn"], None, cos, sin, S, B, nH, hq=hq,
                                       wq=_mx_rows(blk, "fa_qkv", slice(0, D)))
                o = self._cp_attn.finish(q, pending)
            else:
                if hq is not None:
                    qkv = ops.gemm_mxfp8_nt(hq[0], hq[1], *blk["mx"]["fa_qkv"])
                    ops.qk_rmsnorm_rope_pair(qkv[:, :2 * D], blk["fa_qn"], nH, blk["fa_kn"], nH, cos, sin, S, B)
                    q, k = qkv[:, :D], qkv[:, D:2 * D]
                    vt = ops.transpose_v(qkv[:, 2 * D:], S, B, nH, out=self._vt_buffer(S, B, nH, dev))
                elif _FUSE_QKV_EPILOGUE:
                    vt = self._vt_buffer(S, B, nH, dev)
                    qkv = ops.gemm_qk_norm_rope(h, blk["fa_qkv"], D, D, blk["fa_qn"], blk["fa_kn"], cos, sin, S, B, vt=vt)
                    q, k = qkv[:, :D], qkv[:, D:2 * D]
                elif _v_by_operand_swap(S):
                    qk = ops.gemm_nt(h, blk["fa_qkv"][:2 * D])
                    ops.qk_rmsnorm_rope_pair(qk, blk["fa_qn"], nH, blk["fa_kn"], nH, cos, sin, S, B)
                    q, k = qk[:, :D], qk[:, D:]
                    vt = self._vt_buffer(S, B, nH, dev)
                    hv = h.view(S, B, D)
                    for b_ in range(B):
                        ops.gemm_nt(blk["fa_qkv"][2 * D:], hv[:, b_], out=vt[b_].view(D, -1)[:, :S])
                else:
                    qkv = ops.gemm_nt(h, blk["fa_qkv"])
                    ops.qk_rmsnorm_rope_pair(qkv[:, :2 * D], blk["fa_qn"], nH, blk["fa_kn"], nH, cos, sin, S, B)
                    q, k = qkv[:, :D], qkv[:, D:2 * D]
                    vt = ops.transpose_v(qkv[:, 2 * D:], S, B, nH, out=self._vt_buffer(S, B, nH, dev))
                o = ops.flash_attn(q, k, vt, S, S, B, nH)
            self._linear(o, blk, "fa_out", out=xs, epilogue=ops.EPI_GATED_RESIDUAL, gate=gate, residual=xs)
            shift, scale, gate = self._modulation(emb, blk["ada"][1], adaln_lora, 3)
            h = self._ln(xs, shift, scale, fused)
            k, vt = ca_kv[bi]
            if _CROSS_Q_NORM_IN_ATTENTION:
                o = ops.flash_attn(self._linear(h, blk, "ca_q"), k, vt, S, M, B, nH, kv_dense=ca_dense, q_norm_weight=blk["ca_qn"])
            else:
                hq = h if fused else (ops.quant_mxfp8(h) if "mx" in blk else None)
                q = _project_norm_rope(h, blk["ca_q"], D, 0, blk["ca_qn"], None, None, None, S, B, nH, hq=hq, wq=_mx_rows(blk, "ca_q", slice(None)))
                o = ops.flash_attn(q, k, vt, S, M, B, nH, kv_dense=ca_dense)
            self._linear(o, blk, "ca_out", out=xs, epilogue=ops.EPI_GATED_RESIDUAL, gate=gate, residual=xs)
            shift, scale, gate = self._modulation(emb, blk["ada"][2], adaln_lora, 3)
            h = self._ln(xs, shift, scale, fused)
            u = self._linear(h, blk, "w1", epilogue=ops.EPI_GELU, out_mx=fused)
            self._linear(u, blk, "w2", out=xs, epilogue=ops.EPI_GATED_RESIDUAL, gate=gate, residual=xs)

        fl = (P["final_layer.adaLN_modulation.1.weight"], P["final_layer.adaLN_modulation.2.weight"])
        shift, scale = self._modulation(emb, fl, adaln_lora[:, : 2 * D], 2)
        h = ops.layernorm_modulate(xs, shift, scale)
        y = ops.gemm_nt(h, P["final_layer.linear.weight"])
        return ops.dit_unpatchify(y, B, self.out_channels, T, H, W, pt, ps)

    def _vt_buffer(self, S: int, B: int, H: int, dev) -> torch.Tensor:
        key = (S, B, H, str(dev))
        buf = getattr(self, "_vt_cache", None)
        if buf is None or buf[0] != key:
            buf = self._vt_cache = (key, torch.zeros((B, H, 128, ops.ceil_to(S, 64)), dtype=torch.bfloat16, device=dev))
        return buf[1]

    def _cross_attention_kv(self, pk, crossattn_emb: torch.Tensor):
        use_cache = cacheable(crossattn_emb) and pk["versioned"]
        key = (crossattn_emb.data_ptr(), tensor_version(crossattn_emb), tuple(crossattn_emb.shape), crossattn_emb.dtype, pk["key"])
        cache = self.__dict__.setdefault("_ca_kv_cache", {})
        hit = cache.get(key) if use_cache else None
        if hit is not None and hit[0] is crossattn_emb:
            return hit[1], hit[2]
        B, M = crossattn_emb.shape[:2]
        D, nH = self.model_channels, self.num_heads
        ctx = crossattn_emb.to(torch.bfloat16).permute(1, 0, 2).reshape(M * B, -1).contiguous()
        per_block = []
        for blk in pk["blocks"]:
            kv = ops.gemm_nt(ctx, blk["ca_kv"])
            per_block.append((ops.qk_rmsnorm_rope(kv[:, :D], blk["ca_kn"], None, None, M, B, nH), ops.transpose_v(kv[:, D:], M, B, nH)))
        if not use_cache:
            return per_block, 0
        dense = 0
        live = (crossattn_emb != 0).any(dim=-1).any(dim=0)
        n_live = int(live.nonzero().max()) + 1 if bool(live.any()) else 1
        cand = min(M, ops.ceil_to(n_live, 64))
        if cand < M:
            dirty = torch.zeros((), dtype=torch.bool, device=crossattn_emb.device)
            for k_, vt_ in per_block:
                dirty |= (k_[cand * B:] != 0).any() | (vt_[..., cand:M] != 0).any()
            if not bool(dirty):
                dense = cand
        while len(cache) >= 4:
            cache.pop(next(iter(cache)))
        cache[key] = (crossattn_emb, per_block, dense)
        return per_block, dense

    def _modulation(self, emb, ada, lora, n):
        w1, w2 = ada
        mid = ops.gemv(emb, w1, act_in=1)
        mod = ops.gemv(mid, w2, add=lora)
        D = self.model_channels
        return tuple(mod[:, i * D:(i + 1) * D] for i in range(n))


def _nearest_resize(mask: torch.Tensor, size: Tuple[int, int]) -> torch.Tensor:
    m = mask
    squeeze = False
    if m.dim() == 3:
        m = m.unsqueeze(1)
        squeeze = True
    if tuple(m.shape[-2:]) != tuple(size):
        m = torch.nn.functional.interpolate(m.float(), size=size, mode="nearest").to(mask.dtype)
    return m[:, 0] if (m.dim() == 4) else m
```

### gen3c_amd/ops.py

```python
from __future__ import annotations

import math
from typing import Optional

import torch

from . import _lib

EPI_NONE, EPI_GELU, EPI_GATED_RESIDUAL, EPI_BIAS = 0, 1, 2, 3

_KERNEL_TIMERS = None


def set_option(name: str, value: int):
    _lib.check(_lib.load().g3_set_option(name.encode(), int(value)), "g3_set_option")


def enable_kernel_timers(on: bool = True):
    global _KERNEL_TIMERS
    _KERNEL_TIMERS = [] if on else None


def collected_kernel_timers():
    return list(_KERNEL_TIMERS or [])
# ... 62 lines not shown
    _lib.check(lib.g3_quant_mxfp8_bf16(_dev(x, "x"), ldx, _dev(q, "q", torch.float8_e4m3fn), ldq, _dev(s, "scales", torch.uint8), lds, M, K,
                                       _stream()), "g3_quant_mxfp8_bf16")
    return q, s


def _mx_operands(aq, as_, wq, ws):
    M, K, lda = _rowmajor2d(aq, "aq")
    N, Kw, ldw = _rowmajor2d(wq, "wq")
    if K != Kw:
        raise _lib.Gen3cHipError(f"gemm_mxfp8_nt: K mismatch {K} vs {Kw}")
    Ma, Ka, ldas = _rowmajor2d(as_, "as_")
    Nw, Kws, ldws = _rowmajor2d(ws, "ws")
    if (Ma, Nw) != (M, N) or Ka * 32 != K or Kws * 32 != K:
        raise _lib.Gen3cHipError(f"gemm_mxfp8_nt: scale shapes {tuple(as_.shape)} / {tuple(ws.shape)} do not match operands [{M}, {K}] / [{N}, {K}]")
    return M, N, K, lda, ldas, ldw, ldws


def gemm_mxfp8_nt(aq: torch.Tensor, as_: torch.Tensor, wq: torch.Tensor, ws: torch.Tensor, out: Optional[torch.Tensor] = None,
                  epilogue: int = EPI_NONE, gate: Optional[torch.Tensor] = None, residual: Optional[torch.Tensor] = None, out_mx=None):
    if out_mx is not None and out_mx is not False:
        return _gemm_mxfp8_nt_mxout(aq, as_, wq, ws, out_mx, epilogue, out, gate, residual)
    M, N, K, lda, ldas, ldw, ldws = _mx_operands(aq, as_, wq, ws)
    if out is None:
        out = torch.empty((M, N), dtype=torch.bfloat16, device=aq.device)
    Mo, No, ldc = _rowmajor2d(out, "out")
    assert (Mo, No) == (M, N)
    gp, grows, ldg, rp, ldr = 0, 1, 0, 0, 0
    if gate is not None:
        grows, gn, ldg = _rowmajor2d(gate, "gate")
        assert gn == N
        gp = _dev(gate, "gate")
    if residual is not None:
        rm, rn, ldr = _rowmajor2d(residual, "residual")
        assert (rm, rn) == (M, N)
        rp = _dev(residual, "residual")
    lib = _lib.load()
    timer = None
    if _KERNEL_TIMERS is not None and M >= 4096:
        timer = HipTimer()
        timer.start()
    f8 = torch.float8_e4m3fn
    _lib.check(lib.g3_gemm_mxfp8_nt(_dev(aq, "aq", f8), lda, _dev(as_, "as_", torch.uint8), ldas, _dev(wq, "wq", f8), ldw,
                                    _dev(ws, "ws", torch.uint8), ldws, _dev(out, "out"), ldc, M, N, K, epilogue, gp, grows, ldg, rp, ldr,
                                    _stream()), "g3_gemm_mxfp8_nt")
    if timer is not None:
        timer.stop()
        _KERNEL_TIMERS.append(("gemm_mxfp8_nt", dict(M=M, N=N, K=K, epilogue=epilogue), timer))
    return out


def _mx_out_pair(out, M: int, K: int, device, what: str):
    if out is None or out is True:
        out = (torch.empty((M, K), dtype=torch.float8_e4m3fn, device=device), torch.empty((M, K // 32), dtype=torch.uint8, device=device))
    q, s = out
    Mq, Kq, ldq = _rowmajor2d(q, "q")
    Ms, Ks, lds = _rowmajor2d(s, "scales")
    if (Mq, Kq) != (M, K) or (Ms, Ks) != (M, K // 32):
        raise _lib.Gen3cHipError(f"{what}: output shapes {tuple(q.shape)} / {tuple(s.shape)} do not match [{M}, {K}]")
    return q, s, ldq, lds


def _gemm_mxfp8_nt_mxout(aq, as_, wq, ws, out_mx, epilogue, out, gate, residual):
    if out is not None or gate is not None or residual is not None:
        raise _lib.Gen3cHipError("gemm_mxfp8_nt: out_mx takes no bf16 out, gate or residual (epilogues NONE and GELU only)")
    M, N, K, lda, ldas, ldw, ldws = _mx_operands(aq, as_, wq, ws)
    q, s, ldq, lds = _mx_out_pair(out_mx, M, N, aq.device, "gemm_mxfp8_nt")
    lib = _lib.load()
    timer = None
    if _KERNEL_TIMERS is not None and M >= 4096:
        timer = HipTimer()
        timer.start()
    f8 = torch.float8_e4m3fn
    _lib.check(lib.g3_gemm_mxfp8_nt_mxout(_dev(aq, "aq", f8), lda, _dev(as_, "as_", torch.uint8), ldas, _dev(wq, "wq", f8), ldw,
                                          _dev(ws, "ws", torch.uint8), ldws, _dev(q, "q", f8), ldq, _dev(s, "scales", torch.uint8), lds, M, N, K,
                                          epilogue, _stream()), "g3_gemm_mxfp8_nt_mxout")
    if timer is not None:
        timer.stop()
        _KERNEL_TIMERS.append(("gemm_mxfp8_nt_mxout", dict(M=M, N=N, K=K, epilogue=epilogue), timer))
    return q, s


def gemv(a: torch.Tensor, w: torch.Tensor, add: Optional[torch.Tensor] = None, act_in: int = 0,
         out: Optional[torch.Tensor] = None) -> torch.Tensor:
    M, K, lda = _rowmajor2d(a, "a")
    N, Kw, ldw = _rowmajor2d(w, "w")
    assert K == Kw
    if out is None:
        out = torch.empty((M, N), dtype=torch.bfloat16, device=a.device)
    ap, ldadd = 0, 0
    if add is not None:
        am, an, ldadd = _rowmajor2d(add, "add")
        assert (am, an) == (M, N)
        ap = _dev(add, "add")
    lib = _lib.load()
    _lib.check(lib.g3_gemv_bf16(_dev(a, "a"), lda, _dev(w, "w"), ldw, ap, ldadd, _dev(out, "out"), out.stride(0), M, N, K,
                                act_in, _stream()), "g3_gemv_bf16")
    return out


def layernorm_modulate(x: torch.Tensor, shift: torch.Tensor, scale: torch.Tensor, out: Optional[torch.Tensor] = None,
                       eps: float = 1e-6) -> torch.Tensor:
    rows, D, ldx = _rowmajor2d(x, "x")
    B, Ds, ldmod = _rowmajor2d(shift, "shift")
    assert Ds == D and scale.shape == shift.shape and scale.stride(0) == ldmod
    if out is None:
        out = torch.empty((rows, D), dtype=torch.bfloat16, device=x.device)
    lib = _lib.load()
    _lib.check(lib.g3_layernorm_modulate_bf16(_dev(x, "x"), ldx, _dev(shift, "shift"), _dev(scale, "scale"), ldmod, B,
                                              _dev(out, "out"), out.stride(0), rows, D, eps, _stream()),
               "g3_layernorm_modulate_bf16")
    return out


def layernorm_modulate_mxfp8(x: torch.Tensor, shift: torch.Tensor, scale: torch.Tensor, out=None, eps: float = 1e-6):
    rows, D, ldx = _rowmajor2d(x, "x")
    B, Ds, ldmod = _rowmajor2d(shift, "shift")
    assert Ds == D and scale.shape == shift.shape and scale.stride(0) == ldmod
    q, s, ldq, lds = _mx_out_pair(out, rows, D, x.device, "layernorm_modulate_mxfp8")
    lib = _lib.load()
    _lib.check(lib.g3_layernorm_modulate_mxfp8(_dev(x, "x"), ldx, _dev(shift, "shift"), _dev(scale, "scale"), ldmod, B,
                                               _dev(q, "q", torch.float8_e4m3fn), ldq, _dev(s, "scales", torch.uint8), lds, rows, D, eps, _stream()),
               "g3_layernorm_modulate_mxfp8")
    return q, s


def posemb_layernorm_modulate(x: torch.Tensor, pe_t: torch.Tensor, pe_h: Optional[torch.Tensor], pe_w: Optional[torch.Tensor],
                              pos_norm: Optional[torch.Tensor], T: int, Hp: int, Wp: int, B: int, shift: torch.Tensor, scale: torch.Tensor,
                              out: Optional[torch.Tensor] = None, eps: float = 1e-6) -> torch.Tensor:
    rows, D, ldx = _rowmajor2d(x, "x")
    assert rows == T * Hp * Wp * B
    if pe_h is None:
        assert pe_w is None and pos_norm is None and pe_t.shape == (T * Hp * Wp, D) and pe_t.is_contiguous()
    else:
        for t, n in ((pe_t, T), (pe_h, Hp), (pe_w, Wp)):
            assert t.dim() == 2 and t.shape[0] >= n and t.shape[1] == D and t.is_contiguous()
        assert pos_norm.numel() == T * Hp * Wp and pos_norm.is_contiguous()
    Bm, Ds, ldmod = _rowmajor2d(shift, "shift")
    assert Ds == D and scale.shape == shift.shape and scale.stride(0) == ldmod
    if out is None:
        out = torch.empty((rows, D), dtype=torch.bfloat16, device=x.device)
    lib = _lib.load()
    _lib.check(lib.g3_posemb_layernorm_modulate_bf16(_dev(x, "x"), ldx, _dev(pe_t, "pe_t"), _dev(pe_h, "pe_h") if pe_h is not None else 0,
                                                     _dev(pe_w, "pe_w") if pe_w is not None else 0, _dev(pos_norm, "pos_norm") if pos_norm is not None else 0,
                                                     T, Hp, Wp, B, _dev(shift, "shift"), _dev(scale, "scale"), ldmod, Bm,
                                                     _dev(out, "out"), out.stride(0), D, eps, _stream()), "g3_posemb_layernorm_modulate_bf16")
    return out


def posemb_layernorm_modulate_mxfp8(x: torch.Tensor, pe_t: torch.Tensor, pe_h: Optional[torch.Tensor], pe_w: Optional[torch.Tensor],
                                    pos_norm: Optional[torch.Tensor], T: int, Hp: int, Wp: int, B: int, shift: torch.Tensor, scale: torch.Tensor,
                                    out=None, eps: float = 1e-6):
    rows, D, ldx = _rowmajor2d(x, "x")
    assert rows == T * Hp * Wp * B
    if pe_h is None:
        assert pe_w is None and pos_norm is None and pe_t.shape == (T * Hp * Wp, D) and pe_t.is_contiguous()
    else:
        for t, n in ((pe_t, T), (pe_h, Hp), (pe_w, Wp)):
            assert t.dim() == 2 and t.shape[0] >= n and t.shape[1] == D and t.is_contiguous()
        assert pos_norm.numel() == T * Hp * Wp and pos_norm.is_contiguous()
    Bm, Ds, ldmod = _rowmajor2d(shift, "shift")
    assert Ds == D and scale.shape == shift.shape and scale.stride(0) == ldmod
    q, s, ldq, lds = _mx_out_pair(out, rows, D, x.device, "posemb_layernorm_modulate_mxfp8")
    lib = _lib.load()
    _lib.check(lib.g3_posemb_layernorm_modulate_mxfp8(_dev(x, "x"), ldx, _dev(pe_t, "pe_t"), _dev(pe_h, "pe_h") if pe_h is not None else 0,
                                                      _dev(pe_w, "pe_w") if pe_w is not None else 0, _dev(pos_norm, "pos_norm") if pos_norm is not None else 0,
                                                      T, Hp, Wp, B, _dev(shift, "shift"), _dev(scale, "scale"), ldmod, Bm,
                                                      _dev(q, "q", torch.float8_e4m3fn), ldq, _dev(s, "scales", torch.uint8), lds, D, eps, _stream()),
               "g3_posemb_layernorm_modulate_mxfp8")
    return q, s


def qk_rmsnorm_rope(x: torch.Tensor, weight: torch.Tensor, cos: Optional[torch.Tensor], sin: Optional[torch.Tensor],
                    S: int, B: int, H: int, out: Optional[torch.Tensor] = None, eps: float = 1e-6) -> torch.Tensor:
    rows, width, ld_in = _rowmajor2d(x, "x")
    assert rows == S * B and width == H * 128
    if out is None:
        out = torch.empty((rows, H * 128), dtype=torch.bfloat16, device=x.device)
    cp = sp = 0
    if cos is not None:
        assert cos.shape == (S, 128) and sin.shape == (S, 128) and cos.is_contiguous() and sin.is_contiguous()
        cp, sp = _dev(cos, "cos", torch.float32), _dev(sin, "sin", torch.float32)
    lib = _lib.load()
    _lib.check(lib.g3_qk_rmsnorm_rope_bf16(_dev(x, "x"), ld_in, _dev(weight, "weight"), cp, sp, _dev(out, "out"),
                                           out.stride(0), S, B, H, 128, eps, _stream()), "g3_qk_rmsnorm_rope_bf16")
    return out


def qk_rmsnorm_rope_pair(x: torch.Tensor, weight_q: torch.Tensor, H_q: int, weight_k: torch.Tensor, H_k: int, cos: Optional[torch.Tensor],
                         sin: Optional[torch.Tensor], S: int, B: int, out: Optional[torch.Tensor] = None, eps: float = 1e-6) -> torch.Tensor:
    rows, width, ld_in = _rowmajor2d(x, "x")
    assert rows == S * B and width == (H_q + H_k) * 128
    if out is None:
        out = x
    cp = sp = 0
    if cos is not None:
        assert cos.shape == (S, 128) and sin.shape == (S, 128) and cos.is_contiguous() and sin.is_contiguous()
        cp, sp = _dev(cos, "cos", torch.float32), _dev(sin, "sin", torch.float32)
    lib = _lib.load()
    _lib.check(lib.g3_qk_rmsnorm_rope_pair_bf16(_dev(x, "x"), ld_in, _dev(weight_q, "weight_q"), H_q, _dev(weight_k, "weight_k"), H_k, cp, sp, _dev(out, "out"),
                                                out.stride(0), S, B, 128, eps, _stream()), "g3_qk_rmsnorm_rope_pair_bf16")
    return out


def gemm_qk_norm_rope(a: torch.Tensor, w: torch.Tensor, n_q: int, n_k: int, norm_q: Optional[torch.Tensor], norm_k: Optional[torch.Tensor],
                      cos: Optional[torch.Tensor], sin: Optional[torch.Tensor], S: int, B: int, out: Optional[torch.Tensor] = None,
                      eps: float = 1e-6, vt: Optional[torch.Tensor] = None) -> torch.Tensor:
    M, K, lda = _rowmajor2d(a, "a")
    N, Kw, ldw = _rowmajor2d(w, "w")
    assert K == Kw and M == S * B
    if out is None:
        out = torch.empty((M, N), dtype=torch.bfloat16, device=a.device)
    Mo, No, ldc = _rowmajor2d(out, "out")
    assert (Mo, No) == (M, N)
    cp = sp = 0
    if cos is not None:
        assert cos.shape == (S, 128) and sin.shape == (S, 128) and cos.is_contiguous() and sin.is_contiguous()
        cp, sp = _dev(cos, "cos", torch.float32), _dev(sin, "sin", torch.float32)
    lib = _lib.load()
    timer = None
    if _KERNEL_TIMERS is not None and M >= 4096:
        timer = HipTimer()
        timer.start()
    vtp, vt_ld = 0, 0
    if vt is not None:
        n_v = N - n_q - n_k
        assert n_v > 0 and vt.dim() == 4 and vt.shape[:3] == (B, n_v // 128, 128) and vt.shape[3] >= S and vt.is_contiguous()
        vtp, vt_ld = _dev(vt, "vt"), vt.shape[3]
    _lib.check(lib.g3_gemm_qk_norm_rope_bf16(_dev(a, "a"), lda, _dev(w, "w"), ldw, _dev(out, "out"), ldc, M, N, K, n_q, n_k,
                                             _dev(norm_q, "norm_q") if n_q else 0, _dev(norm_k, "norm_k") if n_k else 0, cp, sp, B, eps, vtp, vt_ld,
                                             _stream()),
               "g3_gemm_qk_norm_rope_bf16")
    if timer is not None:
        timer.stop()
        _KERNEL_TIMERS.append(("gemm_nt", dict(M=M, N=N, K=K, epilogue=5), timer))
    return out


def ceil_to(x: int, m: int) -> int:
    return (x + m - 1) // m * m


def transpose_v(v: torch.Tensor, S: int, B: int, H: int, out: Optional[torch.Tensor] = None) -> torch.Tensor:
    rows, width, ld_in = _rowmajor2d(v, "v")
    assert rows == S * B and width == H * 128
    ldvt = ceil_to(S, 64)
    if out is None:
        out = torch.empty((B, H, 128, ldvt), dtype=torch.bfloat16, device=v.device)
    assert out.shape == (B, H, 128, ldvt) and out.is_contiguous()
    lib = _lib.load()
    _lib.check(lib.g3_transpose_v_bf16(_dev(v, "v"), ld_in, _dev(out, "out"), ldvt, S, B, H, 128, _stream()),
               "g3_transpose_v_bf16")
    return out


def flash_attn(q: torch.Tensor, k: torch.Tensor, vt: torch.Tensor, Sq: int, Skv: int, B: int, H: int,
               out: Optional[torch.Tensor] = None, softmax_scale: Optional[float] = None, variant: int = 0, partial: bool = False, kv_dense: int = 0,
               q_norm_weight: Optional[torch.Tensor] = None, q_norm_eps: float = 1e-6, carry=None, kv_skip=None):
    if carry is not None or kv_skip is not None or (partial and out is not None):
        return _flash_attn_carry(q, k, vt, Sq, Skv, B, H, out, softmax_scale, variant, partial, carry, kv_skip)
    qr, qw, ldq = _rowmajor2d(q, "q")
    kr, kw, ldk = _rowmajor2d(k, "k")
    assert qr == Sq * B and kr == Skv * B and qw == H * 128 and kw == H * 128
    assert vt.is_contiguous() and vt.dim() in (4, 5) and tuple(vt.shape[-4:-1]) == (B, H, 128)
    ldvt = vt.shape[-1]
    o_part = lse = None
    if partial:
        assert out is None
        o_part = torch.empty((Sq * B, H * 128), dtype=torch.float32, device=q.device)
        lse = torch.empty((B, H, Sq), dtype=torch.float32, device=q.device)
        ldo = o_part.stride(0)
    else:
        if out is None:
            out = torch.empty((Sq * B, H * 128), dtype=torch.bfloat16, device=q.device)
        ldo = out.stride(0)
    if softmax_scale is None:
        softmax_scale = 1.0 / math.sqrt(128)
    lib = _lib.load()
    timer = None
    if _KERNEL_TIMERS is not None:
        timer = HipTimer()
        timer.start()
    n_seg = vt.shape[0] if vt.dim() == 5 else 0
    if n_seg:
        assert Skv % n_seg == 0
    if 0 < kv_dense < Skv or q_norm_weight is not None:
        assert not partial and not n_seg and not variant, "the cross-attention form takes plain V^T, a bf16 output and the automatic kernel choice"
        kd = int(kv_dense) if 0 < kv_dense < Skv else 0
        _lib.check(lib.g3_cross_attn_fwd_bf16(_dev(q, "q"), ldq * B, ldq, 128, _dev(q_norm_weight, "q_norm_weight") if q_norm_weight is not None else 0, float(q_norm_eps),
                                              _dev(k, "k"), ldk * B, ldk, 128, _dev(vt, "vt"), ldvt, H * 128 * ldvt, 128 * ldvt,
                                              _dev(out, "out"), ldo * B, ldo, 128, Sq, Skv, kd, B, H, 128, float(softmax_scale), _stream()),
                   "g3_cross_attn_fwd_bf16")
        if timer is not None:
            timer.stop()
            _KERNEL_TIMERS.append(("flash_attn_fwd", dict(Sq=Sq, Skv=Skv, B=B, H=H, partial=False, kv_dense=kd, q_norm=q_norm_weight is not None,
                                                          kernel=lib.g3_flash_attn_kernel_name_ex(Sq, Skv, B, H, 4).decode()), timer))
        return out
    _lib.check(lib.g3_flash_attn_fwd_ex_bf16(_dev(q, "q"), ldq * B, ldq, 128, _dev(k, "k"), ldk * B, ldk, 128, _dev(vt, "vt"), ldvt, H * 128 * ldvt, 128 * ldvt,
                                             Skv // n_seg if n_seg else 0, B * H * 128 * ldvt if n_seg else 0,
                                             0 if partial else _dev(out, "out"), _dev(o_part, "o_part", torch.float32) if partial else 0,
                                             _dev(lse, "lse", torch.float32) if partial else 0, ldo * B, ldo, 128, Sq, Skv, B, H, 128,
                                             float(softmax_scale), int(variant), _stream()), "g3_flash_attn_fwd_ex_bf16")
    if timer is not None:
        timer.stop()
        _KERNEL_TIMERS.append(("flash_attn_fwd", dict(Sq=Sq, Skv=Skv, B=B, H=H, partial=partial,
                                                      kernel=lib.g3_flash_attn_kernel_name_ex(Sq, Skv, B, H, int(variant)).decode()), timer))
    return (o_part, lse) if partial else out


def _carry_kernel_name(plain: str) -> str:
    return {"flash_attn_fwd_w4b_kernel<true>": "flash_attn_fwd_w4b_carry_kernel<true>",
            "flash_attn_fwd_v3_kernel<0, 6, 8, true>": "flash_attn_fwd_v3_kernel<2, 6, 8, true>",
            "flash_attn_fwd_v3_kernel<1, 6, 8, false>": "flash_attn_fwd_v3_kernel<3, 6, 8, false>"}.get(plain, plain)


def _flash_attn_carry(q, k, vt, Sq, Skv, B, H, out, softmax_scale, variant, partial, carry, kv_skip):
    skip_begin, skip_len = (int(kv_skip[0]), int(kv_skip[1])) if kv_skip is not None else (0, 0)
    skv_all = Skv + skip_len
    qr, qw, ldq = _rowmajor2d(q, "q")
    kr, kw, ldk = _rowmajor2d(k, "k")
    assert qr == Sq * B and kr == skv_all * B and qw == H * 128 and kw == H * 128
    assert vt.is_contiguous() and vt.dim() in (4, 5) and tuple(vt.shape[-4:-1]) == (B, H, 128)
    ldvt = vt.shape[-1]
    n_seg = vt.shape[0] if vt.dim() == 5 else 0
    if n_seg:
        assert skv_all % n_seg == 0
    lse = None
    if partial:
        if out is None:
            out = torch.empty((Sq * B, H * 128), dtype=torch.float32, device=q.device)
        assert out.dtype == torch.float32, "partial=True writes fp32"
        lse = torch.empty((B, H, Sq), dtype=torch.float32, device=q.device)
    elif out is None:
        out = torch.empty((Sq * B, H * 128), dtype=torch.bfloat16, device=q.device)
    orows, ow, ldo = _rowmajor2d(out, "out")
    assert (orows, ow) == (Sq * B, H * 128)
    co = cl = 0
    if carry is not None:
        o_c, l_c = carry
        if o_c.dtype != torch.float32 or o_c.shape != (Sq * B, H * 128) or o_c.stride() != out.stride():
            raise ValueError(f"flash_attn: carry o_part must be fp32 {(Sq * B, H * 128)} with the output's strides {out.stride()} "
                             f"(got {o_c.dtype} {tuple(o_c.shape)} {o_c.stride()})")
        if l_c.dtype != torch.float32 or l_c.shape != (B, H, Sq) or not l_c.is_contiguous():
            raise ValueError(f"flash_attn: carry lse must be contiguous fp32 {(B, H, Sq)}")
        co, cl = _dev(o_c, "carry_o", torch.float32), _dev(l_c, "carry_lse", torch.float32)
    if softmax_scale is None:
        softmax_scale = 1.0 / math.sqrt(128)
    lib = _lib.load()
    timer = None
    if _KERNEL_TIMERS is not None:
        timer = HipTimer()
        timer.start()
    _lib.check(lib.g3_flash_attn_fwd_carry_bf16(_dev(q, "q"), ldq * B, ldq, 128, _dev(k, "k"), ldk * B, ldk, 128, _dev(vt, "vt"), ldvt, H * 128 * ldvt,
                                                128 * ldvt, skv_all // n_seg if n_seg else 0, B * H * 128 * ldvt if n_seg else 0, skip_begin, skip_len, co, cl,
                                                0 if partial else _dev(out, "out"), _dev(out, "o_part", torch.float32) if partial else 0,
                                                _dev(lse, "lse", torch.float32) if partial else 0, ldo * B, ldo, 128, Sq, Skv, B, H, 128,
                                                float(softmax_scale), int(variant), _stream()), "g3_flash_attn_fwd_carry_bf16")
    if timer is not None:
        timer.stop()
        _KERNEL_TIMERS.append(("flash_attn_fwd", dict(Sq=Sq, Skv=Skv, B=B, H=H, partial=partial, carry=carry is not None, kv_skip=skip_len,
                                                      kernel=_carry_kernel_name(lib.g3_flash_attn_kernel_name_ex(Sq, Skv, B, H, int(variant)).decode())), timer))
    return (out, lse) if partial else out


def attn_merge(parts, Sq: int, B: int, H: int, out: Optional[torch.Tensor] = None) -> torch.Tensor:
    import ctypes as C
    n = len(parts)
    assert 1 <= n <= 8
    ld = parts[0][0].stride(0)
    for o, l in parts:
        assert o.shape == (Sq * B, H * 128) and o.stride(1) == 1 and o.stride(0) == ld and l.shape == (B, H, Sq) and l.is_contiguous()
    if out is None:
        out = torch.empty((Sq * B, H * 128), dtype=torch.bfloat16, device=parts[0][0].device)
    orows, ow, ldo = _rowmajor2d(out, "out")
    assert (orows, ow) == (Sq * B, H * 128)
    op = (C.c_void_p * n)(*[_dev(o, "o_part", torch.float32) for o, _ in parts])
    lp = (C.c_void_p * n)(*[_dev(l, "lse", torch.float32) for _, l in parts])
    _lib.check(_lib.load().g3_attn_merge_partials_bf16(op, lp, n, ld * B, ld, 128, _dev(out, "out"), ldo * B, ldo, 128, Sq, B, H, 128, _stream()),
               "g3_attn_merge_partials_bf16")
    return out


def add_inplace(x: torch.Tensor, y: torch.Tensor) -> torch.Tensor:
    assert x.is_contiguous() and y.is_contiguous() and x.numel() == y.numel()
    lib = _lib.load()
    _lib.check(lib.g3_add_inplace_bf16(_dev(x, "x"), _dev(y, "y"), x.numel(), _stream()), "g3_add_inplace_bf16")
    return x


def dit_patchify(sources, B: int, T: int, H: int, W: int, patch_t: int, patch_s: int) -> torch.Tensor:
    import ctypes as C
    assert 1 <= len(sources) <= 4
    ptrs, chans, has_t = [], [], []
    for i, (t, ht) in enumerate(sources):
        assert t.is_contiguous() and t.shape[0] == B and tuple(t.shape[-2:]) == (H, W) and (t.dim() == 5 and t.shape[2] == T if ht else t.dim() == 4)
        ptrs.append(_dev(t, f"source{i}"))
        chans.append(int(t.shape[1]))
        has_t.append(1 if ht else 0)
    n = len(sources)
    ctot = sum(chans)
    out = torch.empty(((T // patch_t) * (H // patch_s) * (W // patch_s) * B, ctot * patch_t * patch_s * patch_s), dtype=torch.bfloat16,
                      device=sources[0][0].device)
    lib = _lib.load()
    _lib.check(lib.g3_dit_patchify_bf16((C.c_void_p * n)(*ptrs), (C.c_int * n)(*chans), (C.c_int * n)(*has_t), n, out.data_ptr(), B, T, H, W,
                                        patch_t, patch_s, _stream()), "g3_dit_patchify_bf16")
    return out


def dit_unpatchify(y: torch.Tensor, B: int, C_out: int, T: int, H: int, W: int, patch_t: int, patch_s: int) -> torch.Tensor:
    rows, cols, ldy = _rowmajor2d(y, "y")
    assert rows == (T // patch_t) * (H // patch_s) * (W // patch_s) * B and cols == patch_s * patch_s * patch_t * C_out
    out = torch.empty((B, C_out, T, H, W), dtype=torch.bfloat16, device=y.device)
    lib = _lib.load()
    _lib.check(lib.g3_dit_unpatchify_bf16(_dev(y, "y"), ldy, out.data_ptr(), B, C_out, T, H, W, patch_t, patch_s, _stream()), "g3_dit_unpatchify_bf16")
    return out


def timestep_embedding(timesteps: torch.Tensor, norm_weight: torch.Tensor, D: int):
    assert timesteps.dim() == 1 and timesteps.is_contiguous() and norm_weight.numel() == D
    Bn = timesteps.shape[0]
    t_sin = torch.empty((Bn, D), dtype=torch.bfloat16, device=timesteps.device)
    emb = torch.empty_like(t_sin)
    lib = _lib.load()
    _lib.check(lib.g3_timestep_embedding_bf16(_dev(timesteps, "timesteps", torch.float32), _dev(norm_weight, "norm_weight"), t_sin.data_ptr(),
                                              emb.data_ptr(), Bn, D, _stream()), "g3_timestep_embedding_bf16")
    return t_sin, emb


def edm_prepare_input(xt, gt_latent, noise, indicator, T: int, hw: int, augment_sigma: float, c_in_aug: float,
                      c_in_bf16: float, c_in_step: float):
    assert xt.is_contiguous() and gt_latent.is_contiguous() and noise.is_contiguous() and indicator.is_contiguous()
    assert xt.shape == gt_latent.shape == noise.shape and indicator.numel() == T
    new_xt, new_xt_scaled = torch.empty_like(xt), torch.empty_like(xt)
    lib = _lib.load()
    _lib.check(lib.g3_edm_prepare_input_bf16(_dev(xt, "xt"), _dev(gt_latent, "gt_latent"), _dev(noise, "noise", torch.float32),
                                             _dev(indicator, "indicator", torch.float32), _dev(new_xt, "new_xt"),
                                             _dev(new_xt_scaled, "new_xt_scaled"), xt.numel(), T, hw, augment_sigma, c_in_aug,
                                             c_in_bf16, c_in_step, _stream()), "g3_edm_prepare_input_bf16")
    return new_xt, new_xt_scaled


def edm_cfg_euler_step(out_cond, out_uncond, new_xt, gt_latent, indicator, T: int, hw: int, guidance: float,
                       c_skip_bf16: float, c_out_bf16: float, c_skip: float, c_out: float, sigma: float, sigma_next: float):
    for t in (out_cond, out_uncond, new_xt, gt_latent, indicator):
        assert t.is_contiguous()
    assert out_cond.shape == out_uncond.shape == new_xt.shape == gt_latent.shape
    xt_next = torch.empty_like(new_xt)
    lib = _lib.load()
    _lib.check(lib.g3_edm_cfg_euler_step_bf16(_dev(out_cond, "out_cond"), _dev(out_uncond, "out_uncond"), _dev(new_xt, "new_xt"),
                                              _dev(gt_latent, "gt_latent"), _dev(indicator, "indicator", torch.float32),
                                              _dev(xt_next, "xt_next"), new_xt.numel(), T, hw, guidance, c_skip_bf16, c_out_bf16,
                                              c_skip, c_out, sigma, sigma_next, _stream()), "g3_edm_cfg_euler_step_bf16")
    return xt_next


class HipTimer:

    def __init__(self):
        import ctypes as C
        self._lib = _lib.load()
        self._a, self._b = C.c_void_p(), C.c_void_p()
        _lib.check(self._lib.g3_event_create(C.byref(self._a)))
        _lib.check(self._lib.g3_event_create(C.byref(self._b)))

    def start(self):
        _lib.check(self._lib.g3_event_record(self._a, _stream()))

    def stop(self):
        _lib.check(self._lib.g3_event_record(self._b, _stream()))

    def elapsed_ms(self) -> float:
        import ctypes as C
        ms = C.c_float(0)
        _lib.check(self._lib.g3_event_elapsed_ms(self._a, self._b, C.byref(ms)))
        return float(ms.value)

    def __del__(self):
        try:
            self._lib.g3_event_destroy(self._a)
            self._lib.g3_event_destroy(self._b)
        except Exception:
            pass
```

### include/gen3c_hip.h

```cpp
#ifndef GEN3C_HIP_H
#define GEN3C_HIP_H

#include <stddef.h>
#include <stdint.h>

#ifdef __cplusplus
extern "C" {
#endif

#define G3_OK 0
#define G3_ERR_ARG 1
#define G3_ERR_LAUNCH 2
#define G3_ERR_RESOURCE 3

#define G3_EPI_NONE 0
#define G3_EPI_GELU 1
#define G3_EPI_GATED_RESIDUAL 2
#define G3_EPI_BIAS 3
#define G3_EPI_BIAS_RESIDUAL 4

const char* g3_last_error(void);
int g3_abi_version(void);
int g3_set_option(const char* name , int value);
int g3_device_info(int device, int* cu_count, int* is_gfx950, char* arch_name , int arch_name_len);

int g3_event_create(void** ev);
int g3_event_record(void* ev, void* stream);
int g3_event_elapsed_ms(void* start, void* stop, float* ms );
int g3_event_destroy(void* ev);

int g3_gemm_bf16_nt(const void* A, int64_t lda, const void* W, int64_t ldw, void* C, int64_t ldc, int M, int N, int K,
                    int epilogue, const void* gate, int gate_rows, int64_t ldg, const void* residual, int64_t ldr,
                    void* stream);

const char* g3_gemm_kernel_name(int M, int N, int K, int epilogue);

int g3_quant_mxfp8_bf16(const void* x, int64_t ldx, void* q, int64_t ldq, void* scales, int64_t lds, int M, int K, void* stream);

int g3_gemm_mxfp8_nt(const void* aq, int64_t lda, const void* as, int64_t ldas, const void* wq, int64_t ldw, const void* ws, int64_t ldws,
                     void* c, int64_t ldc, int M, int N, int K, int epilogue, const void* gate, int gate_rows, int64_t ldg,
                     const void* residual, int64_t ldr, void* stream);

const char* g3_gemm_mxfp8_kernel_name(int M, int N, int K, int epilogue);

int g3_gemm_mxfp8_nt_mxout(const void* aq, int64_t lda, const void* as, int64_t ldas, const void* wq, int64_t ldw, const void* ws, int64_t ldws,
                           void* q_out, int64_t ldq, void* s_out, int64_t lds, int M, int N, int K, int epilogue, void* stream);

const char* g3_gemm_mxfp8_mxout_kernel_name(int M, int N, int K, int epilogue);

int g3_gemv_bf16(const void* a, int64_t lda, const void* w, int64_t ldw, const void* add, int64_t ldadd, void* out,
                 int64_t ldo, int M, int N, int K, int act_in, void* stream);

int g3_flash_attn_fwd_bf16(const void* q, int64_t q_row, int64_t q_batch, int64_t q_head, const void* k, int64_t k_row,
                           int64_t k_batch, int64_t k_head, const void* vt, int64_t vt_row, int64_t vt_batch,
                           int64_t vt_head, void* o, int64_t o_row, int64_t o_batch, int64_t o_head, int Sq, int Skv,
                           int B, int H, int head_dim, float softmax_scale, void* stream);

const char* g3_flash_attn_kernel_name(int Sq, int Skv, int B, int H);

int g3_cross_attn_fwd_bf16(const void* q, int64_t q_row, int64_t q_batch, int64_t q_head, const void* q_norm_weight, float q_norm_eps,
                           const void* k, int64_t k_row, int64_t k_batch, int64_t k_head, const void* vt, int64_t vt_row, int64_t vt_batch,
                           int64_t vt_head, void* o, int64_t o_row, int64_t o_batch, int64_t o_head, int Sq, int Skv, int kv_dense, int B, int H,
                           int head_dim, float softmax_scale, void* stream);

int g3_flash_attn_fwd_kvseg_bf16(const void* q, int64_t q_row, int64_t q_batch, int64_t q_head, const void* k, int64_t k_row,
                                 int64_t k_batch, int64_t k_head, const void* vt, int64_t vt_row, int64_t vt_batch, int64_t vt_head,
                                 int vt_seg_len, int64_t vt_seg_stride, void* o, int64_t o_row, int64_t o_batch, int64_t o_head, int Sq,
                                 int Skv, int B, int H, int head_dim, float softmax_scale, void* stream);

int g3_flash_attn_fwd_ex_bf16(const void* q, int64_t q_row, int64_t q_batch, int64_t q_head, const void* k, int64_t k_row, int64_t k_batch,
                              int64_t k_head, const void* vt, int64_t vt_row, int64_t vt_batch, int64_t vt_head, int vt_seg_len,
                              int64_t vt_seg_stride, void* o, float* o_partial, float* lse, int64_t o_row, int64_t o_batch, int64_t o_head,
                              int Sq, int Skv, int B, int H, int head_dim, float softmax_scale, int variant, void* stream);
const char* g3_flash_attn_kernel_name_ex(int Sq, int Skv, int B, int H, int variant);

int g3_flash_attn_fwd_carry_bf16(const void* q, int64_t q_row, int64_t q_batch, int64_t q_head, const void* k, int64_t k_row, int64_t k_batch,
                                 int64_t k_head, const void* vt, int64_t vt_row, int64_t vt_batch, int64_t vt_head, int vt_seg_len,
                                 int64_t vt_seg_stride, int kv_skip_begin, int kv_skip_len, const float* carry_o, const float* carry_lse,
                                 void* o, float* o_partial, float* lse, int64_t o_row, int64_t o_batch, int64_t o_head, int Sq, int Skv, int B,
                                 int H, int head_dim, float softmax_scale, int variant, void* stream);
int g3_attn_merge_partials_bf16(const float* const* o_parts , const float* const* lse_parts , int n_parts, int64_t p_row,
                                int64_t p_batch, int64_t p_head, void* out, int64_t o_row, int64_t o_batch, int64_t o_head, int Sq, int B,
                                int H, int head_dim, void* stream);

int g3_transpose_v_bf16(const void* v, int64_t ld_in, void* vt, int64_t ldvt, int S, int B, int H, int head_dim,
                        void* stream);

int g3_layernorm_modulate_bf16(const void* x, int64_t ldx, const void* shift, const void* scale, int64_t ldmod,
                               int mod_rows, void* out, int64_t ldo, int rows, int D, float eps, void* stream);

int g3_layernorm_modulate_mxfp8(const void* x, int64_t ldx, const void* shift, const void* scale, int64_t ldmod, int mod_rows, void* q,
                                int64_t ldq, void* scales, int64_t lds, int rows, int D, float eps, void* stream);

int g3_qk_rmsnorm_rope_bf16(const void* in, int64_t ld_in, const void* weight, const float* cos_table,
                            const float* sin_table, void* out, int64_t ld_out, int S, int B, int H, int head_dim,
                            float eps, void* stream);

int g3_qk_rmsnorm_rope_pair_bf16(const void* in, int64_t ld_in, const void* weight_q, int H_q, const void* weight_k, int H_k,
                                 const float* cos_table, const float* sin_table, void* out, int64_t ld_out, int S, int B, int head_dim,
                                 float eps, void* stream);

int g3_gemm_qk_norm_rope_bf16(const void* A, int64_t lda, const void* W, int64_t ldw, void* C, int64_t ldc, int M, int N, int K,
                              int n_q, int n_k, const void* norm_q, const void* norm_k, const float* cos_table,
                              const float* sin_table, int B, float eps, void* vt, int64_t vt_ld, void* stream);

int g3_posemb_layernorm_modulate_bf16(void* x, int64_t ldx, const void* pe_t, const void* pe_h, const void* pe_w,
                                      const void* pos_norm, int T, int Hp, int Wp, int B, const void* shift, const void* scale,
                                      int64_t ldmod, int mod_rows, void* out, int64_t ldo, int D, float eps, void* stream);

int g3_posemb_layernorm_modulate_mxfp8(void* x, int64_t ldx, const void* pe_t, const void* pe_h, const void* pe_w, const void* pos_norm, int T,
                                       int Hp, int Wp, int B, const void* shift, const void* scale, int64_t ldmod, int mod_rows, void* q,
                                       int64_t ldq, void* scales, int64_t lds, int D, float eps, void* stream);

int g3_add_inplace_bf16(void* x, const void* y, int64_t n, void* stream);

int g3_dit_patchify_bf16(const void* const* srcs, const int* chans, const int* has_t, int n_src, void* out, int B, int T, int H,
                         int W, int patch_t, int patch_s, void* stream);
int g3_dit_unpatchify_bf16(const void* y, int64_t ldy, void* out, int B, int C_out, int T, int H, int W, int patch_t, int patch_s,
                           void* stream);
int g3_timestep_embedding_bf16(const float* timesteps, const void* norm_weight, void* t_sin, void* emb, int B, int D, void* stream);

int g3_edm_prepare_input_bf16(const void* xt, const void* gt_latent, const float* noise, const float* indicator,
                              void* new_xt, void* new_xt_scaled, int64_t n, int T, int hw, float augment_sigma,
                              float c_in_aug, float c_in_bf16, float c_in_step, void* stream);
int g3_edm_cfg_euler_step_bf16(const void* out_cond, const void* out_uncond, const void* new_xt, const void* gt_latent,
                               const float* indicator, void* xt_next, int64_t n, int T, int hw, float guidance,
                               float c_skip_bf16, float c_out_bf16, float c_skip, float c_out, float sigma,
                               float sigma_next, void* stream);

int g3_warp_project_f32(const float* points, const float* w2c, const float* K, const float* mask1, float* z, float* flow,
                        float* cam_points, float* maskz, void* group_max, int n, int h, int w, int group_size, void* stream);
int g3_warp_splat_f32(const float* image, const float* z, const float* flow, const float* maskz, const void* group_max,
                      float* accum, int n, int h, int w, int group_size, void* stream);
int g3_warp_resolve_f32(const float* accum, float* frame, float* mask, float* depth, int n, int h, int w, void* stream);

size_t g3_warp_windows_workspace_bytes(int n, int h, int w);
int g3_warp_splat_resolve_f32(const float* image, const float* z, const float* flow, const float* maskz, const void* group_max,
                              float* accum, void* workspace, float* frame, float* mask, float* depth, int n, int h, int w,
                              int group_size, void* stream);
size_t g3_render_workspace_bytes(int n, int h, int w, int group_size);
int g3_render_workspace_init(void* workspace, int n, int h, int w, int group_size, void* stream);
int g3_render_items_f32(const float* points_src, const float* image_src, const float* mask_src, const uint8_t* boundary_src,
                        const int* src_index, const float* w2c, const float* K, const float* Kinv, void* workspace, float* frame, float* mask,
                        float* depth, float* flow_out, int n, int n_src, int h, int w, int group_size, void* stream);
int g3_mesh_occlusion_f32(const float* cam_points, const uint8_t* boundary_mask, const float* K, const float* Kinv,
                          float* pts_ds, uint8_t* mask_ds, void* tmin, float* frame, float* mask, float* depth, int n, int h,
                          int w, int factor, void* stream);
int g3_unproject_points_f32(const float* depth, const float* c2w, const float* Kinv, float* points, int n, int h, int w,
                            void* stream);
int g3_reliable_depth_mask_f32(const float* depth, uint8_t* out, int n, int h, int w, int window, float ratio_thresh,
                               float eps, void* stream);
size_t g3_align_depth_workspace_bytes(int H, int W);
int g3_align_depth_f32(const float* source_depth, const float* target_depth, const uint8_t* target_mask, const float* Kinv_host,
                       const float* T_host, int non_rigid, int num_iters, float lambda_arap, float lr, float* out_depth,
                       void* workspace, size_t workspace_bytes, int H, int W, void* stream);

int g3_conv3d_cl_bf16(const void* in, int64_t ld_in, const void* w, int64_t ldw, const void* bias, const void* residual,
                      int64_t ldr, void* out, int64_t ld_out, int K, int N, int Ti, int Hi, int Wi, int To, int Ho, int Wo,
                      int kt, int kh, int kw, int st, int sh, int sw, int ot, int oh, int ow, void* stream);
int g3_conv3d_cl_gnstats_bf16(const void* in, int64_t ld_in, const void* w, int64_t ldw, const void* bias, const void* residual,
                              int64_t ldr, void* out, int64_t ld_out, int K, int N, int Ti, int Hi, int Wi, int To, int Ho, int Wo,
                              int kt, int kh, int kw, int st, int sh, int sw, int ot, int oh, int ow, void* gn_stats_f64,
                              int gn_rows_per_frame, void* stream);
int g3_groupnorm_stats_cl_bf16(const void* x, int64_t ld, void* stats_f64, int frames, int rows_per_frame, int C, void* stream);
int g3_groupnorm_apply_cl_bf16(const void* x, int64_t ld, const void* gamma, const void* beta, const void* stats_f64, void* out,
                               int64_t ldo, int frames, int rows_per_frame, int C, float eps, int swish, void* stream);
int g3_groupnorm_swish_cl_bf16(const void* x, int64_t ld, const void* gamma, const void* beta, void* stats_f64, void* out,
                               int64_t ldo, int frames, int rows_per_frame, int C, float eps, int swish, void* stream);
int g3_haar3d_patch_bf16(const void* video, void* out, int T, int H, int W, void* stream);
int g3_haar3d_unpatch_bf16(const void* coef, int64_t ld, void* video, int Tp, int Hp, int Wp, void* stream);
int g3_resample_cl_bf16(const void* in, void* out, int Ti, int Hi, int Wi, int C, int mode, void* stream);
int g3_softmax_rows_bf16(void* x, int64_t ld, int rows, int n, float scale, void* stream);
int g3_transpose2d_bf16(const void* in, int64_t ld_in, void* out, int64_t ld_out, int R, int C, void* stream);
int g3_temporal_attn_cl_bf16(const void* q, const void* k, const void* v, void* o, int T, int HW, int C, float scale,
                             void* stream);
int g3_spatial_attn_d512_bf16(const void* q, const void* k, const void* vt, int64_t ld_vt, int64_t vt_frame_stride, void* o, int frames,
                              int hw, float softmax_scale, void* stream);

#ifdef __cplusplus
}
#endif
#endif
```

Before: 0.3065.

## Use a static QK logit bound to drop online-softmax max tracking in self-attention

After q/k RMSNorm, a per-block upper bound on the attention logits is computed once from the max absolute q-norm and k-norm weights, with a small margin. A new no-max variant of the w4b attention kernel uses this bound as a fixed softmax offset. That removes the per-tile row max reduction, the running-max rescale branch and the max-tracking work in the pipelined score loop. The risk is precision loss if real logits sit far below the bound, since exponents get very small, so the bound is capped. The kernel falls back to the normal path when the bound is unusable or the launch shape does not qualify.

```diff
diff --git a/gen3c_amd/_lib.py b/gen3c_amd/_lib.py
--- a/gen3c_amd/_lib.py
+++ b/gen3c_amd/_lib.py
@@ -39,6 +39,9 @@
     "g3_flash_attn_fwd_carry_bf16": [vp, i64, i64, i64, vp, i64, i64, i64, vp, i64, i64, i64, i32, i64, i32, i32, vp, vp, vp, vp, vp, i64, i64,
                                      i64, i32, i32, i32, i32, i32, f32, i32, vp],
     "g3_flash_attn_kernel_name_ex": [i32, i32, i32, i32, i32],
+    "g3_self_attn_fwd_bounded_bf16": [vp, i64, i64, i64, vp, i64, i64, i64, vp, i64, i64, i64, i32, i64, vp, vp, vp, i64, i64, i64, i32, i32, i32,
+                                      i32, i32, f32, f32, i32, vp],
+    "g3_self_attn_kernel_name": [i32, i32, i32, i32, f32, i32],
     "g3_attn_merge_partials_bf16": [vp, vp, i32, i64, i64, i64, vp, i64, i64, i64, i32, i32, i32, i32, vp],
     "g3_transpose_v_bf16": [vp, i64, vp, i64, i32, i32, i32, i32, vp],
     "g3_layernorm_modulate_bf16": [vp, i64, vp, vp, i64, i32, vp, i64, i32, i32, f32, vp],
@@ -80,7 +83,7 @@
     "g3_edm_prepare_input_bf16": [vp, vp, vp, vp, vp, vp, i64, i32, i32, f32, f32, f32, f32, vp],
     "g3_edm_cfg_euler_step_bf16": [vp, vp, vp, vp, vp, vp, i64, i32, i32, f32, f32, f32, f32, f32, f32, f32, vp],
 }
-_RESTYPES = {"g3_last_error": C.c_char_p, "g3_flash_attn_kernel_name": C.c_char_p, "g3_gemm_kernel_name": C.c_char_p, "g3_gemm_mxfp8_kernel_name": C.c_char_p, "g3_gemm_mxfp8_mxout_kernel_name": C.c_char_p, "g3_flash_attn_kernel_name_ex": C.c_char_p, "g3_align_depth_workspace_bytes": C.c_size_t,
+_RESTYPES = {"g3_last_error": C.c_char_p, "g3_flash_attn_kernel_name": C.c_char_p, "g3_gemm_kernel_name": C.c_char_p, "g3_gemm_mxfp8_kernel_name": C.c_char_p, "g3_gemm_mxfp8_mxout_kernel_name": C.c_char_p, "g3_flash_attn_kernel_name_ex": C.c_char_p, "g3_self_attn_kernel_name": C.c_char_p, "g3_align_depth_workspace_bytes": C.c_size_t,
              "g3_warp_windows_workspace_bytes": C.c_size_t, "g3_render_workspace_bytes": C.c_size_t}
 
 
diff --git a/gen3c_amd/csrc/attention.hip b/gen3c_amd/csrc/attention.hip
--- a/gen3c_amd/csrc/attention.hip
+++ b/gen3c_amd/csrc/attention.hip
@@ -31,6 +31,7 @@
     const float* carry_lse;
     int kv_skip_begin, kv_skip_len;
     uint32_t kv_skip_vt_bytes;
+    float logit_bound_log2;
 };
 
 G3_DEVICE int k_off(int row, int chunk) { return row * HD + ((chunk ^ (row & 15)) << 3); }
@@ -890,11 +891,18 @@
 
 
 #include "attention_w4.hpp"
+#define W4B_NM 0
 #define W4B_CP 0
 #include "attention_w4b.hpp"
 #undef W4B_CP
 #define W4B_CP 1
 #include "attention_w4b.hpp"
+#undef W4B_CP
+#undef W4B_NM
+#define W4B_CP 0
+#define W4B_NM 1
+#include "attention_w4b.hpp"
+#undef W4B_NM
 #undef W4B_CP
 
 }
@@ -930,12 +938,22 @@
 
 extern "C" const char* g3_flash_attn_kernel_name(int Sq, int Skv, int B, int H) { return g3_flash_attn_kernel_name_ex(Sq, Skv, B, H, 0); }
 
+constexpr float NM_BOUND_LOG2_MAX = 60.0f;
+static float attn_bound_log2(float logit_bound) { return logit_bound * 1.4426950408889634f; }
+static bool attn_bound_usable(float bound_log2) { return bound_log2 > 0.f && bound_log2 <= NM_BOUND_LOG2_MAX; }
+
+extern "C" const char* g3_self_attn_kernel_name(int Sq, int Skv, int B, int H, float logit_bound, int variant) {
+    if (attn_resolve_variant(Sq, Skv, B, H, variant) == 11 && attn_bound_usable(attn_bound_log2(logit_bound))) return "flash_attn_fwd_w4b_nm_kernel<true>";
+    return g3_flash_attn_kernel_name_ex(Sq, Skv, B, H, variant);
+}
+
 static int flash_attn_launch(const void* q, int64_t q_row, int64_t q_batch, int64_t q_head, const void* k, int64_t k_row, int64_t k_batch,
                              int64_t k_head, const void* vt, int64_t vt_row, int64_t vt_batch, int64_t vt_head, int vt_seg_len,
                              int64_t vt_seg_stride, void* o, int64_t o_row, int64_t o_batch, int64_t o_head, int Sq, int Skv, int B, int H,
                              int head_dim, float softmax_scale, void* stream, int variant_req = 0, float* o_partial = nullptr, float* lse = nullptr, int kv_dense = 0,
                              const void* q_norm_w = nullptr, float q_norm_eps = 0.f, bool cp_form = false, const float* carry_o = nullptr,
-                             const float* carry_lse = nullptr, int kv_skip_begin = 0, int kv_skip_len = 0, uint32_t kv_skip_vt_bytes = 0) {
+                             const float* carry_lse = nullptr, int kv_skip_begin = 0, int kv_skip_len = 0, uint32_t kv_skip_vt_bytes = 0,
+                             float logit_bound = 0.f) {
     if (!q || !k || !vt || (!o && !o_partial)) return g3_set_error(G3_ERR_ARG, "g3_flash_attn_fwd_bf16: null operand");
     if ((o_partial != nullptr) != (lse != nullptr)) return g3_set_error(G3_ERR_ARG, "g3_flash_attn_fwd_ex_bf16: o_partial and lse go together");
     if (o_partial && (((uintptr_t)o_partial & 15) || ((uintptr_t)lse & 3))) return g3_set_error(G3_ERR_ARG, "g3_flash_attn_fwd_ex_bf16: misaligned o_partial / lse");
@@ -970,6 +988,7 @@
     p.q_norm_w = (const bf16_t*)q_norm_w; p.q_norm_eps = q_norm_eps;
     p.carry_o = carry_o; p.carry_lse = carry_lse;
     p.kv_skip_begin = kv_skip_begin; p.kv_skip_len = kv_skip_len; p.kv_skip_vt_bytes = kv_skip_vt_bytes;
+    p.logit_bound_log2 = attn_bound_log2(logit_bound);
     if (q_norm_w && ((uintptr_t)q_norm_w & 15)) return g3_set_error(G3_ERR_ARG, "g3_cross_attn_fwd_bf16: misaligned q_norm_weight");
     const size_t smem = (size_t)2 * (KVB * HD + HD * KVB) * sizeof(bf16_t);
     static bool attr_set[64] = {};
@@ -1010,7 +1029,7 @@
     {
       std::lock_guard<std::mutex> attr_lock(attr_mu);
       if (!attr_set[dev_id]) {
-        const void* fns[19] = {reinterpret_cast<const void*>(&flash_attn_fwd_w4b_carry_kernel<true>),
+        const void* fns[20] = {reinterpret_cast<const void*>(&flash_attn_fwd_w4b_nm_kernel<true>), reinterpret_cast<const void*>(&flash_attn_fwd_w4b_carry_kernel<true>),
                                reinterpret_cast<const void*>(&flash_attn_fwd_v3_kernel<2, 6, 8, true>), reinterpret_cast<const void*>(&flash_attn_fwd_v3_kernel<3, 6, 8, false>),
                                reinterpret_cast<const void*>(&flash_attn_fwd_w4b_kernel<false>), reinterpret_cast<const void*>(&flash_attn_fwd_w4b_kernel<true>),
                                reinterpret_cast<const void*>(&flash_attn_fwd_kernel<0>), reinterpret_cast<const void*>(&flash_attn_fwd_kernel<1>),
@@ -1020,7 +1039,7 @@
                                reinterpret_cast<const void*>(&flash_attn_fwd_v3_kernel<0, 6, 8, true, true, 4, 4>), reinterpret_cast<const void*>(&flash_attn_fwd_v3_kernel<1, 6, 8, true, true, 4, 4>),
                                reinterpret_cast<const void*>(&flash_attn_fwd_v3_kernel<0, 6, 8, false, true>), reinterpret_cast<const void*>(&flash_attn_fwd_v3_kernel<1, 6, 8, false, true>),
                                reinterpret_cast<const void*>(&flash_attn_fwd_w4_kernel<0>), reinterpret_cast<const void*>(&flash_attn_fwd_w4_kernel<1>)};
-        for (int i = 0; i < 19; ++i) {
+        for (int i = 0; i < 20; ++i) {
             hipError_t e = hipFuncSetAttribute(fns[i], hipFuncAttributeMaxDynamicSharedMemorySize, (int)smem);
             if (e != hipSuccess) return g3_set_error(G3_ERR_LAUNCH, "flash_attn: hipFuncSetAttribute: %s", hipGetErrorString(e));
         }
@@ -1035,7 +1054,9 @@
         p.grid_q = (int)grid4.x; p.n_hb = H * B; p.n_heads = H;
         p.xcd_heads = (g3_opt_attn_xcd_heads && (H * B) % 8 == 0) ? 1 : 0;
         if (p.xcd_heads) grid4 = dim3(grid4.x * H * B, 1, 1);
-        if (cp_form) hipLaunchKernelGGL(flash_attn_fwd_w4b_carry_kernel<true>, grid4, dim3(W4_THREADS), smem, st, p);
+        const bool no_max = variant == 11 && !cp_form && vt_seg_len == 0 && !p.kv_dense && attn_bound_usable(p.logit_bound_log2);
+        if (no_max) hipLaunchKernelGGL(flash_attn_fwd_w4b_nm_kernel<true>, grid4, dim3(W4_THREADS), smem, st, p);
+        else if (cp_form) hipLaunchKernelGGL(flash_attn_fwd_w4b_carry_kernel<true>, grid4, dim3(W4_THREADS), smem, st, p);
         else if (variant == 11) hipLaunchKernelGGL(flash_attn_fwd_w4b_kernel<true>, grid4, dim3(W4_THREADS), smem, st, p);
         else hipLaunchKernelGGL(flash_attn_fwd_w4b_kernel<false>, grid4, dim3(W4_THREADS), smem, st, p);
         return g3_check_launch("g3_flash_attn_fwd_bf16");
@@ -1097,6 +1118,19 @@
     if (o_partial && ((o_row & 3) || (o_batch & 3) || (o_head & 3))) return g3_set_error(G3_ERR_ARG, "g3_flash_attn_fwd_ex_bf16: o_partial strides must be multiples of 4");
     return flash_attn_launch(q, q_row, q_batch, q_head, k, k_row, k_batch, k_head, vt, vt_row, vt_batch, vt_head, vt_seg_len, vt_seg_stride, o, o_row,
                              o_batch, o_head, Sq, Skv, B, H, head_dim, softmax_scale, stream, variant, o_partial, lse);
+}
+
+extern "C" int g3_self_attn_fwd_bounded_bf16(const void* q, int64_t q_row, int64_t q_batch, int64_t q_head, const void* k, int64_t k_row,
+                                             int64_t k_batch, int64_t k_head, const void* vt, int64_t vt_row, int64_t vt_batch, int64_t vt_head,
+                                             int vt_seg_len, int64_t vt_seg_stride, void* o, float* o_partial, float* lse, int64_t o_row,
+                                             int64_t o_batch, int64_t o_head, int Sq, int Skv, int B, int H, int head_dim, float softmax_scale,
+                                             float logit_bound, int variant, void* stream) {
+    if (variant < 0 || variant > 11) return g3_set_error(G3_ERR_ARG, "g3_self_attn_fwd_bounded_bf16: variant %d out of range", variant);
+    if (o && o_partial) return g3_set_error(G3_ERR_ARG, "g3_self_attn_fwd_bounded_bf16: pass either o (bf16 result) or o_partial + lse, not both");
+    if (o_partial && ((o_row & 3) || (o_batch & 3) || (o_head & 3))) return g3_set_error(G3_ERR_ARG, "g3_self_attn_fwd_bounded_bf16: o_partial strides must be multiples of 4");
+    return flash_attn_launch(q, q_row, q_batch, q_head, k, k_row, k_batch, k_head, vt, vt_row, vt_batch, vt_head, vt_seg_len, vt_seg_stride, o, o_row,
+                             o_batch, o_head, Sq, Skv, B, H, head_dim, softmax_scale, stream, variant, o_partial, lse, 0, nullptr, 0.f, false, nullptr, nullptr, 0, 0, 0u,
+                             logit_bound);
 }
 
 extern "C" int g3_flash_attn_fwd_carry_bf16(const void* q, int64_t q_row, int64_t q_batch, int64_t q_head, const void* k, int64_t k_row,
diff --git a/gen3c_amd/csrc/attention_w4b.hpp b/gen3c_amd/csrc/attention_w4b.hpp
--- a/gen3c_amd/csrc/attention_w4b.hpp
+++ b/gen3c_amd/csrc/attention_w4b.hpp
@@ -162,7 +162,9 @@
 
 #endif
 
-#if W4B_CP
+#if W4B_NM
+#define W4B_KERNEL flash_attn_fwd_w4b_nm_kernel
+#elif W4B_CP
 #define W4B_KERNEL flash_attn_fwd_w4b_carry_kernel
 #else
 #define W4B_KERNEL flash_attn_fwd_w4b_kernel
@@ -170,6 +172,8 @@
 template <bool XB>
 __global__ __launch_bounds__(W4_THREADS, 1) void W4B_KERNEL(AttnParams p) {
     constexpr bool CP = W4B_CP;
+    constexpr bool NM = W4B_NM;
+    static_assert(!NM || (XB && !CP), "the no-max form exists for the plain XB kernel only");
     extern __shared__ __attribute__((aligned(16))) char smem_raw[];
     bf16_t* sK = reinterpret_cast<bf16_t*>(smem_raw);
     bf16_t* sV = sK + 2 * KVB * HD;
@@ -206,6 +210,11 @@
         v_skip = p.kv_skip_vt_bytes;
         asm volatile("" : "+s"(carry_o), "+s"(carry_lse), "+s"(skip_t0), "+s"(skip_nt), "+s"(v_skip));
     }
+    float bound = 0.f;
+    if constexpr (NM) {
+        bound = p.logit_bound_log2;
+        asm volatile("" : "+s"(bound));
+    }
     auto k_tile = [&](uint32_t t) -> uint32_t {
         if constexpr (CP) return t + (t >= skip_t0 ? skip_nt : 0u);
         else return t;
@@ -302,14 +311,18 @@
     __syncthreads();
 #pragma unroll
     for (int h = 0; h < 2; ++h) {
-        float ma = max3(SA[h][0][0], SA[h][0][1], SA[h][0][2]);
-        float mb2 = max3(SA[h][1][0], SA[h][1][1], SA[h][1][2]);
-#pragma unroll
-        for (int r = 3; r < 15; r += 2) {
-            ma = max3(ma, SA[h][0][r], SA[h][0][r + 1]);
-            mb2 = max3(mb2, SA[h][1][r], SA[h][1][r + 1]);
+        if constexpr (NM) {
+            m_run[h] = bound;
+        } else {
+            float ma = max3(SA[h][0][0], SA[h][0][1], SA[h][0][2]);
+            float mb2 = max3(SA[h][1][0], SA[h][1][1], SA[h][1][2]);
+#pragma unroll
+            for (int r = 3; r < 15; r += 2) {
+                ma = max3(ma, SA[h][0][r], SA[h][0][r + 1]);
+                mb2 = max3(mb2, SA[h][1][r], SA[h][1][r + 1]);
+            }
+            m_run[h] = xor32_max(max3(ma, mb2, max3(SA[h][0][15], SA[h][1][15], SA[h][1][15])));
         }
-        m_run[h] = xor32_max(max3(ma, mb2, max3(SA[h][0][15], SA[h][1][15], SA[h][1][15])));
 #pragma unroll
         for (int mb = 0; mb < 2; ++mb)
 #pragma unroll
@@ -318,6 +331,7 @@
         for (int r = 0; r < 16; ++r) negm[h][r] = -m_run[h];
         mx_cur[h] = 0.f;
     }
+    if constexpr (NM) asm volatile("" : "+v"(negm[0]), "+v"(negm[1]));
     if (XB && nt > 1) {
         constexpr int KS1 = KVB * HD * 2;
         w4b_read_head<KS1, KS1 + 32 * HD * 2, KS1, KS1 + 32 * HD * 2, KS1, KS1 + 32 * HD * 2>(kaddr[0], kaddr[1], kaddr[2]);
@@ -347,7 +361,7 @@
             using N5 = std::integral_constant<int, n0 + 5>;
             w4b_read_head<frag_off(N0{}), frag_off(N1{}), frag_off(N2{}), frag_off(N3{}), frag_off(N4{}), frag_off(N5{})>(frag_addr(N0{}), frag_addr(N2{}), frag_addr(N4{}));
         }
-        if (__any(fmaxf(mx_cur[0], mx_cur[1]) > RESCALE_THR)) {
+        if (!NM && __any(fmaxf(mx_cur[0], mx_cur[1]) > RESCALE_THR)) {
             float alpha[2], delta[2];
 #pragma unroll
             for (int h = 0; h < 2; ++h) {
@@ -443,12 +457,12 @@
                 constexpr bool unit = I < 12;
                 using U = std::integral_constant<int, unit ? 20 + I : 20>;
                 constexpr int hu = (U::value >> 2) & 1, pa = 2 * (I & 1);
-                constexpr int mxk = !has_next ? 0 : (I < 2 ? 0 : (I == 2 || I == 3 || I == 10 || I == 11) ? 1 : I < 12 ? 2 : 3);
+                constexpr int mxk = (!has_next || NM) ? 0 : (I < 2 ? 0 : (I == 2 || I == 3 || I == 10 || I == 11) ? 1 : I < 12 ? 2 : 3);
                 constexpr int mh = I < 10 ? 0 : 1;
                 constexpr int k0 = I < 2 ? 0 : I < 10 ? I - 2 : I < 12 ? I - 10 : I == 12 ? 2 : 5;
                 constexpr int k1i = mxk == 3 ? k0 + 1 : k0, k2i = mxk == 3 ? k0 + 2 : k0;
                 using H = std::integral_constant<int, mh>;
-#define W4B_SN(mb, r) (has_next ? sn(H{}, std::integral_constant<int, mb>{}, std::integral_constant<int, (r)>{}) : 0.f)
+#define W4B_SN(mb, r) ((has_next && !NM) ? sn(H{}, std::integral_constant<int, mb>{}, std::integral_constant<int, (r)>{}) : 0.f)
                 if constexpr (XB && has_next && I == 10) {
                     if (!(G3_AB_ATTN_ABLATE & 64)) asm volatile("s_waitcnt vmcnt(0)\n\ts_barrier" ::: "memory");
                 }
@@ -461,7 +475,14 @@
 #undef W4B_SN
                 if constexpr (unit) uput(U{}, k1);
             });
-            if constexpr (has_next) {
+            if constexpr (has_next && NM) {
+                using N14 = std::integral_constant<int, 16 + 14 + D>;
+                using N15 = std::integral_constant<int, 16 + 15 + D>;
+                float d0 = 0.f, d1 = 0.f;
+                uint32_t kd = 0;
+                w4b_step_pv<14, rd_off(N14{}), true, D, false, 0>(rd_addr(N14{}), pb[0][3], pb[1][3], 0.f, 0.f, kd, d0, d1, d0, d1, 0, 0, 0, 0, 0, 0, 0, 0, 0, 0, 0, 0, d0, d1);
+                w4b_step_pv<15, rd_off(N15{}), true, D, false, 0>(rd_addr(N15{}), pb[0][3], pb[1][3], 0.f, 0.f, kd, d0, d1, d0, d1, 0, 0, 0, 0, 0, 0, 0, 0, 0, 0, 0, 0, d0, d1);
+            } else if constexpr (has_next) {
                 if constexpr (XB) {
                     using N14 = std::integral_constant<int, 16 + 14 + D>;
                     using N15 = std::integral_constant<int, 16 + 15 + D>;
diff --git a/gen3c_amd/dit.py b/gen3c_amd/dit.py
--- a/gen3c_amd/dit.py
+++ b/gen3c_amd/dit.py
@@ -14,6 +14,18 @@
 
 
 _V_OPERAND_SWAP = __import__("os").environ.get("G3_V_OPERAND_SWAP", "1") != "0"
+
+
+_SELF_ATTN_LOGIT_BOUND = True
+_LOGIT_BOUND_MARGIN = 1.03
+
+
+def _qk_logit_bounds(qn_weights, kn_weights, head_dim: int = 128) -> list:
+    if not qn_weights:
+        return []
+    mq = torch.stack([w.detach().abs().max().float() for w in qn_weights])
+    mk = torch.stack([w.detach().abs().max().float() for w in kn_weights])
+    return [float(v) * head_dim / math.sqrt(head_dim) * _LOGIT_BOUND_MARGIN for v in (mq * mk).tolist()]
 
 
 def _v_by_operand_swap(S: int) -> bool:
@@ -302,6 +314,8 @@
                 w1=P[f"{mlp}.block.layer1.weight"], w2=P[f"{mlp}.block.layer2.weight"],
                 ada=[(P[f"{pre}.{j}.adaLN_modulation.1.weight"], P[f"{pre}.{j}.adaLN_modulation.2.weight"]) for j in range(3)],
             ))
+        for blk, fb in zip(blocks, _qk_logit_bounds([b["fa_qn"] for b in blocks], [b["fa_kn"] for b in blocks])):
+            blk["fa_bound"] = fb
         if self.linear_precision == "mxfp8":
             for blk in blocks:
                 blk["mx"] = {n: ops.quant_mxfp8(blk[n]) for n in MXFP8_LINEARS}
@@ -498,7 +512,10 @@
                     ops.qk_rmsnorm_rope_pair(qkv[:, :2 * D], blk["fa_qn"], nH, blk["fa_kn"], nH, cos, sin, S, B)
                     q, k = qkv[:, :D], qkv[:, D:2 * D]
                     vt = ops.transpose_v(qkv[:, 2 * D:], S, B, nH, out=self._vt_buffer(S, B, nH, dev))
-                o = ops.flash_attn(q, k, vt, S, S, B, nH)
+                if _SELF_ATTN_LOGIT_BOUND:
+                    o = ops.self_attn_bounded(q, k, vt, S, S, B, nH, blk["fa_bound"])
+                else:
+                    o = ops.flash_attn(q, k, vt, S, S, B, nH)
             self._linear(o, blk, "fa_out", out=xs, epilogue=ops.EPI_GATED_RESIDUAL, gate=gate, residual=xs)
             shift, scale, gate = self._modulation(emb, blk["ada"][1], adaln_lora, 3)
             h = self._ln(xs, shift, scale, fused)
diff --git a/gen3c_amd/ops.py b/gen3c_amd/ops.py
--- a/gen3c_amd/ops.py
+++ b/gen3c_amd/ops.py
@@ -388,8 +388,45 @@
                                              float(softmax_scale), int(variant), _stream()), "g3_flash_attn_fwd_ex_bf16")
     if timer is not None:
         timer.stop()
-        _KERNEL_TIMERS.append(("flash_attn_fwd", dict(Sq=Sq, Skv=Skv, B=B, H=H, partial=partial,
-                                                      kernel=lib.g3_flash_attn_kernel_name_ex(Sq, Skv, B, H, int(variant)).decode()), timer))
+        _record_attn_timer(timer, Sq, Skv, B, H, partial, lib.g3_flash_attn_kernel_name_ex(Sq, Skv, B, H, int(variant)).decode())
+    return (o_part, lse) if partial else out
+
+
+def _record_attn_timer(timer, Sq: int, Skv: int, B: int, H: int, partial: bool, kernel: str):
+    _KERNEL_TIMERS.append(("flash_attn_fwd", dict(Sq=Sq, Skv=Skv, B=B, H=H, partial=partial, kernel=kernel), timer))
+
+
+def self_attn_bounded(q: torch.Tensor, k: torch.Tensor, vt: torch.Tensor, Sq: int, Skv: int, B: int, H: int, logit_bound: float,
+                      out: Optional[torch.Tensor] = None, softmax_scale: Optional[float] = None, variant: int = 0, partial: bool = False):
+    qr, qw, ldq = _rowmajor2d(q, "q")
+    kr, kw, ldk = _rowmajor2d(k, "k")
+    assert qr == Sq * B and kr == Skv * B and qw == H * 128 and kw == H * 128
+    assert vt.is_contiguous() and vt.dim() == 4 and tuple(vt.shape[:3]) == (B, H, 128)
+    ldvt = vt.shape[-1]
+    o_part = lse = None
+    if partial:
+        assert out is None
+        o_part = torch.empty((Sq * B, H * 128), dtype=torch.float32, device=q.device)
+        lse = torch.empty((B, H, Sq), dtype=torch.float32, device=q.device)
+        ldo = o_part.stride(0)
+    else:
+        if out is None:
+            out = torch.empty((Sq * B, H * 128), dtype=torch.bfloat16, device=q.device)
+        ldo = out.stride(0)
+    if softmax_scale is None:
+        softmax_scale = 1.0 / math.sqrt(128)
+    lib = _lib.load()
+    timer = None
+    if _KERNEL_TIMERS is not None:
+        timer = HipTimer()
+        timer.start()
+    _lib.check(lib.g3_self_attn_fwd_bounded_bf16(_dev(q, "q"), ldq * B, ldq, 128, _dev(k, "k"), ldk * B, ldk, 128, _dev(vt, "vt"), ldvt, H * 128 * ldvt, 128 * ldvt,
+                                                 0, 0, 0 if partial else _dev(out, "out"), _dev(o_part, "o_part", torch.float32) if partial else 0,
+                                                 _dev(lse, "lse", torch.float32) if partial else 0, ldo * B, ldo, 128, Sq, Skv, B, H, 128,
+                                                 float(softmax_scale), float(logit_bound), int(variant), _stream()), "g3_self_attn_fwd_bounded_bf16")
+    if timer is not None:
+        timer.stop()
+        _record_attn_timer(timer, Sq, Skv, B, H, partial, lib.g3_self_attn_kernel_name(Sq, Skv, B, H, float(logit_bound), int(variant)).decode())
     return (o_part, lse) if partial else out
 
 
diff --git a/include/gen3c_hip.h b/include/gen3c_hip.h
--- a/include/gen3c_hip.h
+++ b/include/gen3c_hip.h
@@ -73,6 +73,12 @@
                               int64_t vt_seg_stride, void* o, float* o_partial, float* lse, int64_t o_row, int64_t o_batch, int64_t o_head,
                               int Sq, int Skv, int B, int H, int head_dim, float softmax_scale, int variant, void* stream);
 const char* g3_flash_attn_kernel_name_ex(int Sq, int Skv, int B, int H, int variant);
+
+int g3_self_attn_fwd_bounded_bf16(const void* q, int64_t q_row, int64_t q_batch, int64_t q_head, const void* k, int64_t k_row, int64_t k_batch,
+                                  int64_t k_head, const void* vt, int64_t vt_row, int64_t vt_batch, int64_t vt_head, int vt_seg_len,
+                                  int64_t vt_seg_stride, void* o, float* o_partial, float* lse, int64_t o_row, int64_t o_batch, int64_t o_head,
+                                  int Sq, int Skv, int B, int H, int head_dim, float softmax_scale, float logit_bound, int variant, void* stream);
+const char* g3_self_attn_kernel_name(int Sq, int Skv, int B, int H, float logit_bound, int variant);
 
 int g3_flash_attn_fwd_carry_bf16(const void* q, int64_t q_row, int64_t q_batch, int64_t q_head, const void* k, int64_t k_row, int64_t k_batch,
                                  int64_t k_head, const void* vt, int64_t vt_row, int64_t vt_batch, int64_t vt_head, int vt_seg_len,
```

New measurement: 0.3164 (median of 6 runs). +3.2%, better.
